# neu-vi/Superpoints_Registration

Measured on AMD Instinct MI355X. Metric: point-cloud pairs/sec (16 384 pts/cloud), higher is better.
Workload: dtype f32 (matrix products: range-scaled split-f16x2 MFMA, f32 accumulate; attention weights below 2^-5 of their row sum carried in one f16 plane); 1 GPU; synthetic 16384-pt pairs, full KPConv backbone + superpoint attn + Sinkhorn-SVD pose (3dmatch config, BASELINE configs[1]); streams_per_gpu=1, points_per_cloud=16384, generator=box, point_order=reference, upsample_indices=True, cross_step_overlap=True, streams_inside_a_forward=3: main path, pyramid searches, ResNet shortcut branches

## Files before the change

### include/spr.h

```cpp
#ifndef SPR_H_
#define SPR_H_

#include <stddef.h>
#include <stdint.h>

#ifdef __cplusplus
extern "C" {
#endif

#define SPR_VERSION 6

#define SPR_ACT_NONE 0
#define SPR_ACT_RELU 1
#define SPR_ACT_SIGMOID 2

#define SPR_ORDER_REFERENCE 0
#define SPR_ORDER_CANONICAL 1

int spr_version(void);
const char* spr_last_error(void);

size_t spr_grid_subsample_workspace_bytes(int n, int nb);
int spr_grid_subsample(const float* xyz, const int* cu, int n, int nb, float dl,
                       int max_p, int order_mode, float* out_xyz, int* out_lens,
                       int* out_total, void* ws, size_t ws_bytes, void* stream);

size_t spr_voxel_downsample_workspace_bytes(int n);
int spr_voxel_downsample(const float* xyz, int n, double voxel_size, int* out_idx,
                         int* out_count, void* ws, size_t ws_bytes, void* stream);

size_t spr_radius_neighbors_workspace_bytes(int nq, int ns, int nb);
int spr_radius_neighbors(const float* q_xyz, const int* q_cu, int nq,
                         const float* s_xyz, const int* s_cu, int ns, int nb,
                         float radius, int limit, int algo, int* out_idx,
                         int* max_count, void* ws, size_t ws_bytes, void* stream);

size_t spr_radius_table_bytes(int ns, int nb);
size_t spr_radius_table_build_workspace_bytes(int ns, int nb);
size_t spr_radius_table_query_workspace_bytes(int nq);
int spr_radius_table_slots(void);
int spr_radius_table_build(const float* s_xyz, const int* s_cu, int ns, int nb, float radius,
                           void* table, size_t table_bytes, void* ws, size_t ws_bytes, void* stream);
int spr_radius_table_query(const float* q_xyz, const int* q_cu, int nq, int self, int ns, int nb,
                           float radius, int limit, int slot, const void* table, int* out_idx,
                           int* max_count, int algo, void* ws, size_t ws_bytes, void* stream);

size_t spr_gt_overlap_workspace_bytes(int ns, int nt, int nb);
int spr_gt_overlap(const float* src_xyz, const int* src_cu, int ns, const float* tgt_xyz, const int* tgt_cu,
                   int nt, const float* pose, int nb, double radius, int* src_corr, int* tgt_corr,
                   unsigned char* src_mask, unsigned char* tgt_mask, int* corr, int* corr_count, void* ws,
                   size_t ws_bytes, void* stream);

#define SPR_AUG_NONE 0
#define SPR_AUG_SMALL 1
#define SPR_AUG_LARGE 2
int spr_philox4x32_host(const uint32_t* ctr_host, const uint32_t* key_host, uint32_t* out_host);
int spr_augment_draw(uint64_t seed, const uint64_t* pair_key_host, int nb, int mode, unsigned char* perturb_src_host,
                     unsigned char* swap_host, float* perturb_host, const uint64_t* pair_key, const int* src_cu,
                     int ns, const int* tgt_cu, int nt, float* noise, unsigned int* keys, void* stream);
size_t spr_augment_workspace_bytes(int ns, int nt, int nb, int corr_stride);
int spr_augment_pairs(const float* src_xyz, const int* src_cu, int ns, const float* tgt_xyz, const int* tgt_cu,
                      int nt, const float* pose, int nb, const unsigned char* src_mask,
                      const unsigned char* tgt_mask, const int* corr, int corr_stride, const int* corr_off,
                      const int* corr_count, const float* perturb, const unsigned char* flags, int mode, float scale,
                      int max_pts, uint64_t seed, const uint64_t* pair_key, const float* noise,
                      const unsigned int* keys, float* out_src_xyz, float* out_tgt_xyz, int* out_src_cu,
                      int* out_tgt_cu, float* out_pose, unsigned char* out_src_mask, unsigned char* out_tgt_mask,
                      int* out_src_perm, int* out_tgt_perm, int* out_corr, int* out_corr_count, int* status, void* ws,
                      size_t ws_bytes, void* stream);

size_t spr_kpconv_workspace_bytes(int nq, int ns, int cin, int cout);
size_t spr_kpconv_plan_bytes(int nq);
int spr_kpconv_plan(const int* nbr, int nq, int ns, int nbr_stride, int kmax, int rows_sorted,
                    const int* order, void* plan, size_t plan_bytes, void* stream);
size_t spr_kpconv_wplanes_bytes(int cin, int cout);
int spr_kpconv_prep_weights(const float* weights, int n_kp, int cin, int cout, const float* w_range,
                            int w_range_n, void* wplanes, size_t wplanes_bytes, void* stream);
int spr_kpconv_fwd(const float* q_xyz, int nq, const float* s_xyz, int ns, const int* nbr,
                   int nbr_stride, int kmax, int rows_sorted, const float* x, int cin,
                   const float* weights, int cout, const float* kernel_points, int n_kp,
                   float kp_extent, float* out, int impl, const float* x_range, int x_range_n,
                   const float* w_range, int w_range_n, const void* plan, const void* wplanes,
                   void* ws, size_t ws_bytes, void* stream);

size_t spr_instnorm_workspace_bytes(int max_len_host, int nb, int c);
int spr_instnorm(const float* x, const int* cu, int n, int nb, int max_len_host, int c,
                 float eps, int norm, const float* add, float slope, float* out,
                 float* out_range, int out_range_n, void* ws, size_t ws_bytes, void* stream);
int spr_instnorm_stats(const float* x, const int* cu, int n, int nb, int max_len_host, int c, float eps,
                       float* mean, float* rstd, void* ws, size_t ws_bytes, void* stream);

int spr_block_tail_tile_rows(int ka, int kb, int n_out);
size_t spr_block_tail_tiles_len(int n, int nb, int tile_rows);
int spr_block_tail_tiles(const int* cu, int n, int nb, int tile_rows, int* tiles, void* stream);
size_t spr_block_tail_workspace_bytes(int n, int nb, int kb, int n_out, int tile_rows);
int spr_block_tail(const float* xa, int ka, const float* wa, const float* xb, int kb, const float* wb,
                   const float* add, const int* cu, const int* tiles, int n, int nb, int n_out, float eps,
                   float slope, float* out, const float* xa_range, int xa_range_n, const float* wa_range,
                   int wa_range_n, const float* xb_range, int xb_range_n, const float* wb_range,
                   int wb_range_n, float* out_range, int out_range_n, const float* xa_mean,
                   const float* xa_rstd, float xa_slope, void* ws, size_t ws_bytes, void* stream);

int spr_maxpool_gather(const float* x, int ns, int c, const int* idx, int nq, int idx_stride, int k,
                       const int* order, float* out, float* out_range, int out_range_n, void* stream);
size_t spr_cell_order_workspace_bytes(int n);
int spr_cell_order(const float* xyz, const int* cu, int n, int nb, float cell, int* order, void* ws, size_t ws_bytes,
                   void* stream);

size_t spr_linear_workspace_bytes(void);
int spr_linear(const float* x, int m, int k, const float* w, int n, const float* bias,
               const float* residual, int act, float* out, const float* x_range,
               int x_range_n, const float* w_range, int w_range_n, float* out_range,
               int out_range_cap, int* out_range_n_host, void* ws, size_t ws_bytes, void* stream);
int spr_range_parts(void);
int spr_absmax(const float* x, long rows, int cols, long stride, float* parts, void* stream);
int spr_absmax_multi(const void* jobs_dev, int njobs, int parts_per_job, float* parts_out, void* stream);

int spr_set_gemm_mode(int mode);

int spr_layernorm_range_count(int m);
int spr_layernorm(const float* x, int m, int c, const float* gamma, const float* beta,
                  float eps, const float* pos, float* out_norm, float* out_pos,
                  float* range_norm, float* range_pos, void* stream);

int spr_posemb_sine(const float* xyz, int n, int d_model, float scale,
                    float temperature, float* out, void* stream);

size_t spr_attn_workspace_bytes(int t, int nseg, int nhead, int head_dim);
int spr_attn_varlen_fwd(const float* q, int q_stride, const float* k, int k_stride, const float* v,
                        int v_stride, const int* cu, const int* kv_seg, int t, int nseg, int max_len_host,
                        int nhead, int head_dim, float scale, float* out, int o_stride, float* lse,
                        int* lse_written, void* ws, size_t ws_bytes, void* stream);

size_t spr_attn_inproj_workspace_bytes(int t, int nseg, int nhead, int head_dim);
int spr_attn_inproj_prepare(const float* w_in, int d, float* out, void* stream);
int spr_attn_inproj_varlen_fwd(const float* x_qk, const float* x_v, int t, const float* w_in,
                               const float* b_in, const int* cu, const int* kv_seg, int nseg,
                               int max_len_host, int nhead, int head_dim, float scale,
                               float* out, int o_stride, const float* xqk_range,
                               int xqk_range_n, const float* xv_range, int xv_range_n,
                               float* out_range, const float* w_prep, void* ws, size_t ws_bytes, void* stream);

size_t spr_attn_probs_workspace_bytes(int t, int nhead, int head_dim);
int spr_attn_probs(const float* q, int q_stride, const float* k, int k_stride, const int* cu,
                   const int* kv_seg, int t, int nseg, int max_len_host, int nhead, int head_dim,
                   float scale, int per_head, float* out, const long long* place, int max_rows_host,
                   int max_cols_host, void* ws, size_t ws_bytes, void* stream);

#define SPR_XENC_PTRS_PER_LAYER 18
size_t spr_xenc_prepared_bytes(int n_layers, int d_ff);
size_t spr_xenc_plan_bytes(void);
int spr_xenc_prepare(const void* const* layer_ptrs_host, const float* eps_host, int n_layers,
                     int d_model, int nhead, int d_ff, const float* final_g, const float* final_b,
                     float final_eps, float pos_bound, void* prepared, size_t prepared_bytes,
                     void* plan_host, size_t plan_bytes, void* stream);
size_t spr_xenc_workspace_bytes(int t, int nseg);
int spr_xenc_forward(const void* plan_host, const float* x, const float* pos, const int* cu,
                     const int* kv_self, const int* kv_cross, int t, int nseg, int max_len_host,
                     float* out, void* ws, size_t ws_bytes, void* stream);

size_t spr_attn_bwd_workspace_bytes(int t, int nseg, int nhead);
size_t spr_attn_bwd_min_workspace_bytes(int t, int nhead);
int spr_attn_varlen_bwd(const float* q, int q_stride, const float* k, int k_stride, const float* v,
                        int v_stride, const float* out, int o_stride, const float* dout, int do_stride,
                        const float* lse, const int* cu, const int* kv_seg, const int* q_seg, int t, int nseg,
                        int max_len_host, int nhead, int head_dim, float scale, float* dq, float* dk,
                        float* dv, void* ws, size_t ws_bytes, void* stream);

int spr_set_attn_mode(int mode);

size_t spr_match_workspace_bytes(const int* cu_host, int npairs);
int spr_match_dualsoftmax(const float* feat, int d, const int* cu,
                          const int* cu_host, int npairs, float* match_val,
                          float* match_val2, int* match_ind, void* ws, size_t ws_bytes,
                          void* stream);

int spr_pose_residuals(const float* pose, const float* a, const float* b, const int* pair_cu,
                       int npairs, int total_host, float* res, void* stream);
int spr_pose_scores(const float* poses, int nh, const float* a, const float* b, int n,
                    float* score, void* stream);

int spr_weighted_procrustes(const float* a, const float* b, const float* w,
                            const int* pair_cu, int npairs, float* out_pose,
                            void* stream);

size_t spr_sinkhorn_workspace_bytes(const int* cu_host, int npairs);
int spr_sinkhorn_correspondences(const float* feat, int d, const float* xyz,
                                 const int* cu, const int* cu_host, int npairs,
                                 const float* alpha, const float* beta, int n_iters,
                                 int slack, float* out_w, float* out_that,
                                 void* ws, size_t ws_bytes, void* stream);

int spr_match_sinkhorn(const float* feat, int d, const float* xyz, const int* cu, const int* cu_host,
                       int npairs, const float* alpha, const float* beta, int n_iters, float* match_val,
                       float* match_val2, int* match_ind, float* out_w, float* out_that, void* ws,
                       size_t ws_bytes, void* stream);

int spr_gather_rows(const float* x, int n_src, int c, const int* idx, int n,
                    float* out, void* stream);

size_t spr_loss_workspace_bytes(int n_max, int m_max, int d);
int spr_overlap_pool(const float* ov_prev, int ns_prev, const int* pool,
                     int pool_stride, int w, int nq, float* out, void* stream);
int spr_bce_logits_mean(const float* x, const float* y, int n, float* out,
                        void* ws, size_t ws_bytes, void* stream);
int spr_infonce_pair(const float* anchor_feat, int n, const float* positive_feat,
                     int m, int d, const float* anchor_xyz, const float* pose_gt,
                     const float* positive_xyz, const float* W, float r_p,
                     float r_n, float* out, void* ws, size_t ws_bytes,
                     void* stream);
int spr_transform_l1_pair(const float* pose_gt, const float* pose_pred,
                          const float* xyz, int n, float* out, void* ws,
                          size_t ws_bytes, void* stream);
int spr_sum_scaled(const float* values, int n, float scale, float* out,
                   void* stream);

int spr_bgemm(const float* A, const float* B, float* C, const void* desc_dev, int nbatch,
              int max_m, int max_n, long sa_i, long sa_k, long sb_k, long sb_j, long sc_i,
              long sc_j, float alpha, float beta, void* stream);
size_t spr_tn_product_split_workspace_bytes(void);
int spr_tn_product_split(const float* L, const float* R, long rows, int nl, int nr, int chunk,
                         const float* l_range, int l_range_n, const float* r_range, int r_range_n,
                         float* parts, void* ws, size_t ws_bytes, void* stream);
size_t spr_tn_product_f64_workspace_bytes(long rows, int nl, int nr);
int spr_tn_product_f64(const float* L, const float* R, long rows, int nl, int nr, float* out,
                       void* ws, size_t ws_bytes, void* stream);
int spr_reduce_parts(const float* parts, int nparts, long n, float scale, float* out,
                     int accumulate, void* stream);
int spr_act_bwd(const float* y, const float* dy, int act, long n, float* out, void* stream);
size_t spr_colsum_workspace_bytes(int n);
int spr_colsum(const float* x, long m, int n, float* out, void* ws, size_t ws_bytes, void* stream);
size_t spr_layernorm_bwd_workspace_bytes(int c);
int spr_layernorm_bwd(const float* x, int m, int c, const float* gamma, float eps,
                      const float* dy_norm, const float* dy_pos, float* dx, float* dgamma,
                      float* dbeta, void* ws, size_t ws_bytes, void* stream);
size_t spr_instnorm_bwd_workspace_bytes(int max_len_host, int nb, int c);
int spr_instnorm_bwd(const float* x, const float* out, const float* dout, const int* cu, int n,
                     int nb, int max_len_host, int c, float eps, int norm, float slope,
                     float* dx, float* dadd, void* ws, size_t ws_bytes, void* stream);
size_t spr_scatter_workspace_bytes(long rows, int c);
int spr_maxpool_bwd(const float* x, int ns, int c, const int* idx, int nq, int idx_stride, int k,
                    const float* dy, float* dx, void* ws, size_t ws_bytes, void* stream);
int spr_scatter_rows_add(const float* dy, const int* idx, int n, int c, int n_src, float* dx,
                         void* ws, size_t ws_bytes, void* stream);
size_t spr_kpconv_weighted_features_workspace_bytes(int ns);
int spr_kpconv_weighted_features(const float* q_xyz, int nq, const float* s_xyz, int ns,
                                 const int* nbr, int nbr_stride, int kmax, const float* x, int cin,
                                 const float* kernel_points, int n_kp, float kp_extent,
                                 float* wf, float* cnt, void* ws, size_t ws_bytes, void* stream);
int spr_kpconv_bwd_dx(const float* q_xyz, int nq, const float* s_xyz, int ns, const int* nbr,
                      int nbr_stride, int kmax, int cin, const float* kernel_points, int n_kp,
                      float kp_extent, const float* dwf, const float* dwf_range, int dwf_range_n, float* dx,
                      void* ws, size_t ws_bytes, void* stream);
int spr_softmax_rows(float* mat, const void* desc_dev, int nbatch, int max_m, void* stream);
int spr_softmax_bwd_rows(const float* p, float* dp, const void* desc_dev, int nbatch, int max_m,
                         void* stream);

int spr_bce_logits_mean_bwd(const float* x, const float* y, int n, const float* gout, float* dx,
                            void* stream);
int spr_infonce_pair_dlogits(const float* anchor_feat, int n, const float* positive_feat, int m,
                             int d, const float* anchor_xyz, const float* pose_gt,
                             const float* positive_xyz, const float* W, float r_p, float r_n,
                             float* dlogits, float* row_mask, float* wsym_out, float* t_out,
                             void* ws, size_t ws_bytes, void* stream);
int spr_wsym_bwd(const float* dwsym, int d, float* dW, void* stream);
int spr_transform_l1_pair_bwd(const float* pose_gt, const float* pose_pred, const float* xyz, int n,
                              const float* gout, float* dpose_pred, void* stream);
int spr_weighted_procrustes_bwd(const float* a, const float* b, const float* w,
                                const int* pair_cu, int npairs, const float* dpose, float* da,
                                float* db, float* dw, void* stream);
size_t spr_sinkhorn_bwd_workspace_bytes(const int* cu_host, int npairs, int n_iters);
int spr_sinkhorn_bwd(const float* feat, int d, const float* xyz, const int* cu,
                     const int* cu_host, int npairs, const float* alpha, const float* beta,
                     int n_iters, const float* dw, const float* dthat, float* dfeat,
                     float* dalpha, float* dbeta, void* ws, size_t ws_bytes, void* stream);

size_t spr_circle_loss_workspace_bytes(int nbatch, int max_n, int max_m);
int spr_circle_loss(const float* src_feat, const float* tgt_feat, int d, const float* src_xyz,
                    const float* pose_gt, const float* tgt_xyz, const int* cu_src, const int* cu_tgt,
                    int nbatch, int max_n, int max_m, float r_p, float r_n, float* out, void* ws,
                    size_t ws_bytes, void* stream);
int spr_circle_loss_bwd(const float* src_feat, const float* tgt_feat, int d, const float* src_xyz,
                        const float* pose_gt, const float* tgt_xyz, const int* cu_src, const int* cu_tgt,
                        int nbatch, int max_n, int max_m, float r_p, float r_n, const float* gout, float* G,
                        float* d_src, float* d_tgt, void* ws, size_t ws_bytes, void* stream);

int spr_prof_enable(int on);
int spr_prof_read(int max_records, int* codes_host, int* nqs_host, float* ms_host);

int spr_selftest(int* status_host);

#ifdef __cplusplus
}
#endif
#endif
```

### superpoints_registration_amd/_lib.py

```python
import ctypes
import os
import subprocess

_HERE = os.path.dirname(os.path.abspath(__file__))
LIB_PATH = os.environ.get("SPR_HIP_LIB") or os.path.join(_HERE, "libspr_hip.so")

_vp = ctypes.c_void_p
_i = ctypes.c_int
_f = ctypes.c_float
_sz = ctypes.c_size_t
_l = ctypes.c_long
_u64 = ctypes.c_uint64

SIGNATURES = {
    "spr_version": (_i, []),
    "spr_last_error": (ctypes.c_char_p, []),
    "spr_grid_subsample_workspace_bytes": (_sz, [_i, _i]),
    "spr_grid_subsample": (_i, [_vp, _vp, _i, _i, _f, _i, _i, _vp, _vp, _vp, _vp, _sz, _vp]),
    "spr_voxel_downsample_workspace_bytes": (_sz, [_i]),
    "spr_voxel_downsample": (_i, [_vp, _i, ctypes.c_double, _vp, _vp, _vp, _sz, _vp]),
    "spr_radius_neighbors_workspace_bytes": (_sz, [_i, _i, _i]),
    "spr_radius_neighbors": (_i, [_vp, _vp, _i, _vp, _vp, _i, _i, _f, _i, _i, _vp, _vp, _vp, _sz, _vp]),
    "spr_radius_table_bytes": (_sz, [_i, _i]),
    "spr_radius_table_build_workspace_bytes": (_sz, [_i, _i]),
    "spr_radius_table_query_workspace_bytes": (_sz, [_i]),
    "spr_radius_table_slots": (_i, []),
    "spr_radius_table_build": (_i, [_vp, _vp, _i, _i, _f, _vp, _sz, _vp, _sz, _vp]),
    "spr_radius_table_query": (_i, [_vp, _vp, _i, _i, _i, _i, _f, _i, _i, _vp, _vp, _vp, _i, _vp, _sz, _vp]),
    "spr_gt_overlap_workspace_bytes": (_sz, [_i, _i, _i]),
    "spr_gt_overlap": (_i, [_vp, _vp, _i, _vp, _vp, _i, _vp, _i, ctypes.c_double, _vp, _vp, _vp, _vp, _vp, _vp, _vp,
                            _sz, _vp]),
    "spr_philox4x32_host": (_i, [_vp, _vp, _vp]),
    "spr_augment_draw": (_i, [_u64, _vp, _i, _i, _vp, _vp, _vp, _vp, _vp, _i, _vp, _i, _vp, _vp, _vp]),
    "spr_augment_workspace_bytes": (_sz, [_i, _i, _i, _i]),
    "spr_augment_pairs": (_i, [_vp, _vp, _i, _vp, _vp, _i, _vp, _i, _vp, _vp, _vp, _i, _vp, _vp, _vp, _vp, _i, _f, _i,
                               _u64, _vp, _vp, _vp, _vp, _vp, _vp, _vp, _vp, _vp, _vp, _vp, _vp, _vp, _vp, _vp, _vp,
                               _sz, _vp]),
    "spr_kpconv_workspace_bytes": (_sz, [_i, _i, _i, _i]),
    "spr_kpconv_fwd": (_i, [_vp, _i, _vp, _i, _vp, _i, _i, _i, _vp, _i, _vp, _i, _vp, _i, _f, _vp, _i, _vp, _i, _vp,
                            _i, _vp, _vp, _vp, _sz, _vp]),
    "spr_instnorm_workspace_bytes": (_sz, [_i, _i, _i]),
    "spr_instnorm": (_i, [_vp, _vp, _i, _i, _i, _i, _f, _i, _vp, _f, _vp, _vp, _i, _vp, _sz, _vp]),
    "spr_maxpool_gather": (_i, [_vp, _i, _i, _vp, _i, _i, _i, _vp, _vp, _vp, _i, _vp]),
    "spr_linear_workspace_bytes": (_sz, []),
    "spr_linear": (_i, [_vp, _i, _i, _vp, _i, _vp, _vp, _i, _vp, _vp, _i, _vp, _i, _vp, _i, _vp, _vp, _sz, _vp]),
    "spr_range_parts": (_i, []),
    "spr_absmax_multi": (_i, [_vp, _i, _i, _vp, _vp]),
    "spr_absmax": (_i, [_vp, _l, _i, _l, _vp, _vp]),
    "spr_kpconv_plan_bytes": (_sz, [_i]),
    "spr_kpconv_plan": (_i, [_vp, _i, _i, _i, _i, _i, _vp, _vp, _sz, _vp]),
    "spr_kpconv_wplanes_bytes": (_sz, [_i, _i]),
    "spr_kpconv_prep_weights": (_i, [_vp, _i, _i, _i, _vp, _i, _vp, _sz, _vp]),
    "spr_block_tail_tile_rows": (_i, [_i, _i, _i]),
    "spr_block_tail_tiles_len": (_sz, [_i, _i, _i]),
    "spr_block_tail_tiles": (_i, [_vp, _i, _i, _i, _vp, _vp]),
    "spr_block_tail_workspace_bytes": (_sz, [_i, _i, _i, _i, _i]),
    "spr_block_tail": (_i, [_vp, _i, _vp, _vp, _i, _vp, _vp, _vp, _vp, _i, _i, _i, _f, _f, _vp, _vp, _i, _vp, _i,
                            _vp, _i, _vp, _i, _vp, _i, _vp, _vp, _f, _vp, _sz, _vp]),
    "spr_instnorm_stats": (_i, [_vp, _vp, _i, _i, _i, _i, _f, _vp, _vp, _vp, _sz, _vp]),
    "spr_cell_order_workspace_bytes": (_sz, [_i]),
    "spr_cell_order": (_i, [_vp, _vp, _i, _i, _f, _vp, _vp, _sz, _vp]),
    "spr_layernorm_range_count": (_i, [_i]),
    "spr_attn_inproj_prepare": (_i, [_vp, _i, _vp, _vp]),
    "spr_set_gemm_mode": (_i, [_i]),
    "spr_layernorm": (_i, [_vp, _i, _i, _vp, _vp, _f, _vp, _vp, _vp, _vp, _vp, _vp]),
    "spr_posemb_sine": (_i, [_vp, _i, _i, _f, _f, _vp, _vp]),
    "spr_attn_workspace_bytes": (_sz, [_i, _i, _i, _i]),
    "spr_attn_varlen_fwd": (_i, [_vp, _i, _vp, _i, _vp, _i, _vp, _vp, _i, _i, _i, _i, _i, _f, _vp, _i, _vp, _vp, _vp,
                                 _sz, _vp]),
    "spr_attn_probs_workspace_bytes": (_sz, [_i, _i, _i]),
    "spr_attn_probs": (_i, [_vp, _i, _vp, _i, _vp, _vp, _i, _i, _i, _i, _i, _f, _i, _vp, _vp, _i, _i, _vp, _sz,
                            _vp]),
    "spr_attn_bwd_workspace_bytes": (_sz, [_i, _i, _i]),
    "spr_attn_bwd_min_workspace_bytes": (_sz, [_i, _i]),
    "spr_attn_varlen_bwd": (_i, [_vp, _i, _vp, _i, _vp, _i, _vp, _i, _vp, _i, _vp, _vp, _vp, _vp, _i, _i, _i, _i, _i,
                                 _f, _vp, _vp, _vp, _vp, _sz, _vp]),
    "spr_attn_inproj_workspace_bytes": (_sz, [_i, _i, _i, _i]),
    "spr_attn_inproj_varlen_fwd": (_i, [_vp, _vp, _i, _vp, _vp, _vp, _vp, _i, _i, _i, _i, _f, _vp, _i, _vp, _i, _vp,
                                        _i, _vp, _vp, _vp, _sz, _vp]),
    "spr_set_attn_mode": (_i, [_i]),
    "spr_xenc_prepared_bytes": (_sz, [_i, _i]),
    "spr_xenc_plan_bytes": (_sz, []),
    "spr_xenc_prepare": (_i, [_vp, _vp, _i, _i, _i, _i, _vp, _vp, _f, _f, _vp, _sz, _vp, _sz, _vp]),
    "spr_xenc_workspace_bytes": (_sz, [_i, _i]),
    "spr_xenc_forward": (_i, [_vp, _vp, _vp, _vp, _vp, _vp, _i, _i, _i, _vp, _vp, _sz, _vp]),
    "spr_match_workspace_bytes": (_sz, [_vp, _i]),
    "spr_match_dualsoftmax": (_i, [_vp, _i, _vp, _vp, _i, _vp, _vp, _vp, _vp, _sz, _vp]),
    "spr_pose_residuals": (_i, [_vp, _vp, _vp, _vp, _i, _i, _vp, _vp]),
    "spr_pose_scores": (_i, [_vp, _i, _vp, _vp, _i, _vp, _vp]),
    "spr_weighted_procrustes": (_i, [_vp, _vp, _vp, _vp, _i, _vp, _vp]),
    "spr_sinkhorn_workspace_bytes": (_sz, [_vp, _i]),
    "spr_match_sinkhorn": (_i, [_vp, _i, _vp, _vp, _vp, _i, _vp, _vp, _i, _vp, _vp, _vp, _vp, _vp, _vp, _sz, _vp]),
    "spr_sinkhorn_correspondences": (_i, [_vp, _i, _vp, _vp, _vp, _i, _vp, _vp, _i, _i, _vp, _vp, _vp,
                                          _sz, _vp]),
    "spr_loss_workspace_bytes": (_sz, [_i, _i, _i]),
    "spr_overlap_pool": (_i, [_vp, _i, _vp, _i, _i, _i, _vp, _vp]),
    "spr_bce_logits_mean": (_i, [_vp, _vp, _i, _vp, _vp, _sz, _vp]),
    "spr_infonce_pair": (_i, [_vp, _i, _vp, _i, _i, _vp, _vp, _vp, _vp, _f, _f, _vp, _vp, _sz, _vp]),
    "spr_transform_l1_pair": (_i, [_vp, _vp, _vp, _i, _vp, _vp, _sz, _vp]),
    "spr_sum_scaled": (_i, [_vp, _i, _f, _vp, _vp]),
    "spr_gather_rows": (_i, [_vp, _i, _i, _vp, _i, _vp, _vp]),
    "spr_bgemm": (_i, [_vp, _vp, _vp, _vp, _i, _i, _i, _l, _l, _l, _l, _l, _l, _f, _f, _vp]),
    "spr_tn_product_split_workspace_bytes": (_sz, []),
    "spr_tn_product_split": (_i, [_vp, _vp, _l, _i, _i, _i, _vp, _i, _vp, _i, _vp, _vp, _sz, _vp]),
    "spr_tn_product_f64_workspace_bytes": (_sz, [_l, _i, _i]),
    "spr_tn_product_f64": (_i, [_vp, _vp, _l, _i, _i, _vp, _vp, _sz, _vp]),
    "spr_reduce_parts": (_i, [_vp, _i, _l, _f, _vp, _i, _vp]),
    "spr_act_bwd": (_i, [_vp, _vp, _i, _l, _vp, _vp]),
    "spr_colsum_workspace_bytes": (_sz, [_i]),
    "spr_colsum": (_i, [_vp, _l, _i, _vp, _vp, _sz, _vp]),
    "spr_layernorm_bwd_workspace_bytes": (_sz, [_i]),
    "spr_layernorm_bwd": (_i, [_vp, _i, _i, _vp, _f, _vp, _vp, _vp, _vp, _vp, _vp, _sz, _vp]),
    "spr_instnorm_bwd_workspace_bytes": (_sz, [_i, _i, _i]),
    "spr_instnorm_bwd": (_i, [_vp, _vp, _vp, _vp, _i, _i, _i, _i, _f, _i, _f, _vp, _vp, _vp, _sz, _vp]),
    "spr_scatter_workspace_bytes": (_sz, [_l, _i]),
    "spr_maxpool_bwd": (_i, [_vp, _i, _i, _vp, _i, _i, _i, _vp, _vp, _vp, _sz, _vp]),
    "spr_scatter_rows_add": (_i, [_vp, _vp, _i, _i, _i, _vp, _vp, _sz, _vp]),
    "spr_kpconv_weighted_features_workspace_bytes": (_sz, [_i]),
    "spr_kpconv_weighted_features": (_i, [_vp, _i, _vp, _i, _vp, _i, _i, _vp, _i, _vp, _i, _f, _vp, _vp, _vp, _sz,
                                          _vp]),
    "spr_kpconv_bwd_dx": (_i, [_vp, _i, _vp, _i, _vp, _i, _i, _i, _vp, _i, _f, _vp, _vp, _i, _vp, _vp, _sz, _vp]),
    "spr_softmax_rows": (_i, [_vp, _vp, _i, _i, _vp]),
    "spr_softmax_bwd_rows": (_i, [_vp, _vp, _vp, _i, _i, _vp]),
    "spr_bce_logits_mean_bwd": (_i, [_vp, _vp, _i, _vp, _vp, _vp]),
    "spr_infonce_pair_dlogits": (_i, [_vp, _i, _vp, _i, _i, _vp, _vp, _vp, _vp, _f, _f, _vp, _vp, _vp, _vp, _vp, _sz,
                                      _vp]),
    "spr_wsym_bwd": (_i, [_vp, _i, _vp, _vp]),
    "spr_transform_l1_pair_bwd": (_i, [_vp, _vp, _vp, _i, _vp, _vp, _vp]),
    "spr_weighted_procrustes_bwd": (_i, [_vp, _vp, _vp, _vp, _i, _vp, _vp, _vp, _vp, _vp]),
    "spr_sinkhorn_bwd_workspace_bytes": (_sz, [_vp, _i, _i]),
    "spr_sinkhorn_bwd": (_i, [_vp, _i, _vp, _vp, _vp, _i, _vp, _vp, _i, _vp, _vp, _vp, _vp, _vp, _vp, _sz, _vp]),
    "spr_circle_loss_workspace_bytes": (_sz, [_i, _i, _i]),
    "spr_circle_loss": (_i, [_vp, _vp, _i, _vp, _vp, _vp, _vp, _vp, _i, _i, _i, _f, _f, _vp, _vp, _sz, _vp]),
    "spr_circle_loss_bwd": (_i, [_vp, _vp, _i, _vp, _vp, _vp, _vp, _vp, _i, _i, _i, _f, _f, _vp, _vp, _vp, _vp, _vp,
                                 _sz, _vp]),
    "spr_selftest": (_i, [_vp]),
    "spr_prof_enable": (_i, [_i]),
    "spr_prof_read": (_i, [_i, _vp, _vp, _vp]),
}

_lib = None


def build(force: bool = False) -> str:
    if force:
        subprocess.check_call(["make", "-s", "-C", os.path.join(_HERE, "csrc"), "clean"])
    subprocess.check_call(["make", "-s", "-j8", "-C", os.path.join(_HERE, "csrc")])
    return LIB_PATH


def lib():
    global _lib
    if _lib is None:
        if not os.path.exists(LIB_PATH):
            raise RuntimeError(
                f"{LIB_PATH} is missing: build it with "
                "`python -c 'import __graft_entry__ as g; g.build()'` "
                "(there is no fallback path)")
        l = ctypes.CDLL(LIB_PATH)
        for name, (res, args) in SIGNATURES.items():
            fn = getattr(l, name)
            fn.restype = res
            fn.argtypes = args
        _lib = l
    return _lib


def check(rc: int, what: str) -> None:
    if rc != 0:
        msg = lib().spr_last_error()
        raise RuntimeError(f"{what}: {msg.decode() if msg else 'error'} (status {rc})")
```

### superpoints_registration_amd/csrc/grid_subsample.hip

```cpp
#include <cstring>
#include <rocprim/device/device_radix_sort.hpp>
#include <rocprim/device/device_scan.hpp>

#include <mutex>
#include <unordered_map>
#include <vector>

#include "spr_common.h"

namespace spr {
namespace {

constexpr int kKeyBits = 40;
constexpr unsigned long long kKeyMask = (1ull << kKeyBits) - 1;
constexpr int kMaxSched = 40;

struct CloudInfo {
  float org[3];
  unsigned int nx, ny;
};

struct SchedArg {
  unsigned int v[kMaxSched];
};

struct Schedule {
  std::vector<unsigned int> buckets;
};
const Schedule& host_schedule() {
  static Schedule s;
  static std::once_flag once;
  std::call_once(once, [] {
    std::unordered_map<size_t, char> m;
    size_t bc = m.bucket_count();
    s.buckets.push_back((unsigned int)bc);
    const size_t kMax = (size_t)1 << 22;
    for (size_t i = 0; i < kMax; ++i) {
      m.emplace(i, 0);
      if (m.bucket_count() != bc) {
        bc = m.bucket_count();
        s.buckets.push_back((unsigned int)bc);
      }
    }
  });
  return s;
}

__global__ __launch_bounds__(256) void k_bbox(const float* __restrict__ xyz,
                                              const int* __restrict__ cu,
                                              float dl, CloudInfo* info) {
  const int c = blockIdx.x;
  const int beg = cu[c], end = cu[c + 1];
  __shared__ float smn[3][256], smx[3][256];
  float mn[3], mx[3];
  if (end > beg) {
    for (int d = 0; d < 3; ++d) mn[d] = mx[d] = xyz[3 * (size_t)beg + d];
  } else {
    for (int d = 0; d < 3; ++d) mn[d] = mx[d] = 0.f;
  }
  for (int i = beg + threadIdx.x; i < end; i += blockDim.x) {
    for (int d = 0; d < 3; ++d) {
      float v = xyz[3 * (size_t)i + d];
      if (v < mn[d]) mn[d] = v;
      if (v > mx[d]) mx[d] = v;
    }
  }
  for (int d = 0; d < 3; ++d) {
    smn[d][threadIdx.x] = mn[d];
    smx[d][threadIdx.x] = mx[d];
  }
  __syncthreads();
  for (int s = 128; s > 0; s >>= 1) {
    if (threadIdx.x < s) {
      for (int d = 0; d < 3; ++d) {
        float a = smn[d][threadIdx.x + s];
        if (a < smn[d][threadIdx.x]) smn[d][threadIdx.x] = a;
        float b = smx[d][threadIdx.x + s];
        if (b > smx[d][threadIdx.x]) smx[d][threadIdx.x] = b;
      }
    }
    __syncthreads();
  }
  if (threadIdx.x == 0) {
    const float inv = __fdiv_rn(1.0f, dl);
    CloudInfo ci;
    for (int d = 0; d < 3; ++d)
      ci.org[d] = __fmul_rn(floorf(__fmul_rn(smn[d][0], inv)), dl);
    ci.nx = (unsigned int)floorf(__fdiv_rn(__fsub_rn(smx[0][0], ci.org[0]), dl)) + 1u;
    ci.ny = (unsigned int)floorf(__fdiv_rn(__fsub_rn(smx[1][0], ci.org[1]), dl)) + 1u;
    info[c] = ci;
  }
}

__global__ void k_keys(const float* __restrict__ xyz, const int* __restrict__ cu,
                       int n, int nb, float dl, const CloudInfo* __restrict__ info,
                       unsigned long long* keys, int* vals, int* err) {
  const int i = blockIdx.x * blockDim.x + threadIdx.x;
  if (i >= n) return;
  const int c = find_segment(cu, nb, i);
  const CloudInfo ci = info[c];
  const unsigned long long ix =
      (unsigned long long)floorf(__fdiv_rn(__fsub_rn(xyz[3 * (size_t)i + 0], ci.org[0]), dl));
  const unsigned long long iy =
      (unsigned long long)floorf(__fdiv_rn(__fsub_rn(xyz[3 * (size_t)i + 1], ci.org[1]), dl));
  const unsigned long long iz =
      (unsigned long long)floorf(__fdiv_rn(__fsub_rn(xyz[3 * (size_t)i + 2], ci.org[2]), dl));
  const unsigned long long key =
      ix + (unsigned long long)ci.nx * iy + (unsigned long long)ci.nx * ci.ny * iz;
  if (key > kKeyMask) atomicOr(err, 1);
  keys[i] = ((unsigned long long)c << kKeyBits) | (key & kKeyMask);
  vals[i] = i;
}

__global__ void k_flags(const unsigned long long* __restrict__ keys, int n, int* flags) {
  const int i = blockIdx.x * blockDim.x + threadIdx.x;
  if (i >= n) return;
  flags[i] = (i == 0 || keys[i] != keys[i - 1]) ? 1 : 0;
}

__global__ void k_segstart(const int* __restrict__ flags, const int* __restrict__ vid,
                           int n, int* vstart, int* nvox) {
  const int i = blockIdx.x * blockDim.x + threadIdx.x;
  if (i >= n) return;
  if (flags[i]) vstart[vid[i]] = i;
  if (i == n - 1) *nvox = vid[i] + flags[i];
}

__global__ void k_bary(const float* __restrict__ xyz,
                       const unsigned long long* __restrict__ keys,
                       const int* __restrict__ vals, const int* __restrict__ vstart,
                       const int* __restrict__ nvox_p, int n, float* bary,
                       unsigned long long* vkey, int* vfirst) {
  const int v = blockIdx.x * blockDim.x + threadIdx.x;
  const int nvox = *nvox_p;
  if (v >= nvox) return;
  const int beg = vstart[v];
  const int end = (v + 1 < nvox) ? vstart[v + 1] : n;
  float sx = 0.f, sy = 0.f, sz = 0.f;
  for (int j = beg; j < end; ++j) {
    const size_t p = (size_t)vals[j];
    sx = __fadd_rn(sx, xyz[3 * p + 0]);
    sy = __fadd_rn(sy, xyz[3 * p + 1]);
    sz = __fadd_rn(sz, xyz[3 * p + 2]);
  }
  const float a = (float)(1.0 / (double)(end - beg));
  bary[3 * (size_t)v + 0] = __fmul_rn(sx, a);
  bary[3 * (size_t)v + 1] = __fmul_rn(sy, a);
  bary[3 * (size_t)v + 2] = __fmul_rn(sz, a);
  const unsigned long long k = keys[beg];
  vkey[v] = k;
  vfirst[v] = vals[beg];
}

__global__ void k_cloud_lb(const unsigned long long* __restrict__ vkey,
                           const int* __restrict__ nvox_p, int nb, int* vcu) {
  const int c = blockIdx.x * blockDim.x + threadIdx.x;
  if (c > nb) return;
  const int nvox = *nvox_p;
  int lo = 0, hi = nvox;
  while (lo < hi) {
    const int mid = (lo + hi) >> 1;
    if ((int)(vkey[mid] >> kKeyBits) < c)
      lo = mid + 1;
    else
      hi = mid;
  }
  vcu[c] = lo;
}

__global__ void k_cloud_offsets(const int* __restrict__ vcu, int nb, int max_p, int* out_cu,
                                int* out_lens, int* out_total) {
  if (threadIdx.x != 0 || blockIdx.x != 0) return;
  int b = 0;
  for (int c = 0; c < nb; ++c) {
    out_cu[c] = b;
    const int m = vcu[c + 1] - vcu[c];
    const int keep = (max_p > 0 && m > max_p) ? max_p : m;
    out_lens[c] = keep;
    b += keep;
  }
  out_cu[nb] = b;
  *out_total = b;
}

__global__ void k_emit_canonical(const float* __restrict__ bary,
                                 const unsigned long long* __restrict__ vkey,
                                 const int* __restrict__ nvox_p,
                                 const int* __restrict__ vcu,
                                 const int* __restrict__ out_cu,
                                 const int* __restrict__ out_lens, float* out) {
  const int v = blockIdx.x * blockDim.x + threadIdx.x;
  if (v >= *nvox_p) return;
  const int c = (int)(vkey[v] >> kKeyBits);
  const int r = v - vcu[c];
  if (r >= out_lens[c]) return;
  const size_t o = (size_t)(out_cu[c] + r);
  out[3 * o + 0] = bary[3 * (size_t)v + 0];
  out[3 * o + 1] = bary[3 * (size_t)v + 1];
  out[3 * o + 2] = bary[3 * (size_t)v + 2];
}

__global__ void k_mark_first(const int* __restrict__ vfirst, const int* __restrict__ nvox_p, int* __restrict__ mark,
                             int* __restrict__ who) {
  const int v = blockIdx.x * blockDim.x + threadIdx.x;
  if (v >= *nvox_p) return;
  const int f = vfirst[v];
  mark[f] = 1;
  who[f] = v;
}
__global__ void k_compact_first(const int* __restrict__ mark, const int* __restrict__ pos, const int* __restrict__ who,
                                int n, int* __restrict__ ins) {
  const int i = blockIdx.x * blockDim.x + threadIdx.x;
  if (i >= n || !mark[i]) return;
  ins[pos[i]] = who[i];
}

__device__ void block_inclusive_scan(int* data, int m, int* lds ) {
  const int t = threadIdx.x, T = blockDim.x;
  const int per = (m + T - 1) / T;
  const int beg = min(t * per, m), end = min(beg + per, m);
  int s = 0;
  for (int i = beg; i < end; ++i) s += data[i];
  lds[t] = s;
  __syncthreads();
  for (int o = 1; o < T; o <<= 1) {
    int v = (t >= o) ? lds[t - o] : 0;
    __syncthreads();
    lds[t] += v;
    __syncthreads();
  }
  int run = lds[t] - s;
  for (int i = beg; i < end; ++i) {
    run += data[i];
    data[i] = run;
  }
  __syncthreads();
}

__device__ __forceinline__ int fast_mod(unsigned long long k, unsigned int nbk, double inv) {
  const unsigned long long q = (unsigned long long)((double)k * inv);
  long long r = (long long)k - (long long)(q * (unsigned long long)nbk);
  if (r < 0) r += nbk;
  else if (r >= (long long)nbk) r -= nbk;
  return (int)r;
}

constexpr int kUmapLdsInts = 31744;

__global__ __launch_bounds__(1024) void k_umap_order(
    const unsigned long long* __restrict__ vkey, const int* __restrict__ ins,
    const int* __restrict__ vcu, const int* __restrict__ cu, int nsched, SchedArg sched,
    int* listA, int* listB, int* tfirst, int* tcnt, int* thead, int* nxt,
    int* scan, int* bucket, const float* __restrict__ bary, const int* __restrict__ out_cu,
    const int* __restrict__ out_lens, float* out) {
  __shared__ int lds[1024];
  extern __shared__ int lds_tab[];
  const int c = blockIdx.x;
  const int base = vcu[c];
  const int m = vcu[c + 1] - base;
  if (m <= 0) return;
  int* la = listA + base;
  int* lb = listB + base;
  int* nx = nxt + base;
  int* sc = scan + base;
  int* bk = bucket + base;
  const size_t toff = 3 * (size_t)cu[c] + 16 * (size_t)c;
  const int t = threadIdx.x, T = blockDim.x;

  int done = 0;
  int e = 0;
  int* cur = la;
  int* nxtl = lb;
  while (done < m) {
    e += 1;
    if (e >= nsched) break;
    const int nbk = (int)sched.v[e];
    const int upto = min(m, nbk);
    const int len = upto;
    const double inv = 1.0 / (double)nbk;
    auto epoch = [&](int* tf, int* tc, int* th) {
      for (int b = t; b < nbk; b += T) {
        tf[b] = 0x7fffffff;
        tc[b] = 0;
        th[b] = -1;
      }
      for (int p = done + t; p < upto; p += T) cur[p] = p;
      __syncthreads();
      for (int p = t; p < len; p += T) {
        const int el = cur[p];
        const int b = fast_mod(vkey[ins[base + el]] & kKeyMask, (unsigned int)nbk, inv);
        bk[p] = b;
        atomicMin(&tf[b], p);
        atomicAdd(&tc[b], 1);
        nx[p] = atomicExch(&th[b], p);
      }
      __syncthreads();
      for (int p = t; p < len; p += T) {
        const int b = bk[p];
        sc[p] = (tf[b] == p) ? tc[b] : 0;
      }
      __syncthreads();
      block_inclusive_scan(sc, len, lds);
      const int total = len;
      for (int p = t; p < len; p += T) {
        const int b = bk[p];
        int greater = 0;
        for (int q = th[b]; q != -1; q = nx[q]) greater += (q > p) ? 1 : 0;
        const int pos = (total - sc[tf[b]]) + greater;
        nxtl[pos] = cur[p];
      }
      __syncthreads();
    };
    if (3 * nbk <= kUmapLdsInts) epoch(lds_tab, lds_tab + nbk, lds_tab + 2 * nbk);
    else epoch(tfirst + toff, tcnt + toff, thead + toff);
    int* tmp = cur;
    cur = nxtl;
    nxtl = tmp;
    done = upto;
  }
  const int keep = out_lens[c];
  const size_t ob = (size_t)out_cu[c];
  for (int p = t; p < keep; p += T) {
    const size_t v = (size_t)ins[base + cur[p]];
    out[3 * (ob + p) + 0] = bary[3 * v + 0];
    out[3 * (ob + p) + 1] = bary[3 * v + 1];
    out[3 * (ob + p) + 2] = bary[3 * v + 2];
  }
}

__global__ void k_check_err(const int* err, int* out_total) {
  if (*err) *out_total = -1;
}

size_t sort_temp_bytes(int n) {
  size_t bytes = 0;
  rocprim::radix_sort_pairs(nullptr, bytes, (unsigned long long*)nullptr,
                            (unsigned long long*)nullptr, (int*)nullptr, (int*)nullptr,
                            (unsigned int)(n > 0 ? n : 1));
  size_t sb = 0;
  rocprim::exclusive_scan(nullptr, sb, (int*)nullptr, (int*)nullptr, 0, (size_t)(n > 0 ? n : 1),
                          rocprim::plus<int>());
  return align_up(bytes > sb ? bytes : sb, 256) + 256;
}

}
}

using namespace spr;

extern "C" size_t spr_grid_subsample_workspace_bytes(int n, int nb) {
  const size_t N = (size_t)(n > 0 ? n : 1), B = (size_t)(nb > 0 ? nb : 1);
  size_t b = 0;
  b += align_up(sizeof(CloudInfo) * B, 256);
  b += 3 * align_up(8 * N, 256);
  b += 10 * align_up(4 * N, 256);
  b += 2 * align_up(4 * N, 256);
  b += align_up(12 * N, 256);
  b += 3 * align_up(4 * (3 * N + 16 * B + 64), 256);
  b += 4 * align_up(4 * (B + 1), 256);
  b += 1024;
  b += sort_temp_bytes(n);
  return b;
}

extern "C" int spr_grid_subsample(const float* xyz, const int* cu, int n, int nb,
                                  float dl, int max_p, int order_mode,
                                  float* out_xyz, int* out_lens, int* out_total,
                                  void* ws, size_t ws_bytes, void* stream_) {
  hipStream_t stream = (hipStream_t)stream_;
  SPR_REQUIRE(n >= 0 && nb >= 1, "grid_subsample: bad sizes n=%d nb=%d", n, nb);
  SPR_REQUIRE(dl > 0.f, "grid_subsample: sampleDl must be > 0");
  SPR_REQUIRE(nb < (1 << 23), "grid_subsample: too many clouds");
  SPR_REQUIRE(n > 0, "grid_subsample: empty input");
  SPR_REQUIRE(ws_bytes >= spr_grid_subsample_workspace_bytes(n, nb),
              "grid_subsample: workspace too small");
  Workspace w(ws, ws_bytes);
  const size_t N = (size_t)n;
  CloudInfo* info = w.take<CloudInfo>(nb);
  unsigned long long* keys = w.take<unsigned long long>(N);
  unsigned long long* keys2 = w.take<unsigned long long>(N);
  unsigned long long* vkey = w.take<unsigned long long>(N);
  int* vals = w.take<int>(N);
  int* vals2 = w.take<int>(N);
  int* flags = w.take<int>(N);
  int* vid = w.take<int>(N);
  int* vstart = w.take<int>(N);
  int* vfirst = w.take<int>(N);
  int* sval = w.take<int>(N);
  int* sval2 = w.take<int>(N);
  int* listA = w.take<int>(N);
  int* listB = w.take<int>(N);
  int* nxt = w.take<int>(N);
  int* scan = w.take<int>(N);
  float* bary = w.take<float>(3 * N);
  const size_t tsz = 3 * N + 16 * (size_t)nb + 64;
  int* tfirst = w.take<int>(tsz);
  int* tcnt = w.take<int>(tsz);
  int* thead = w.take<int>(tsz);
  int* cloud_cnt = w.take<int>(nb + 1);
  int* vcu = w.take<int>(nb + 1);
  int* out_cu = w.take<int>(nb + 1);
  int* scalars = w.take<int>(64);
  size_t temp_bytes = sort_temp_bytes(n);
  void* temp = w.take<char>(temp_bytes);
  SPR_REQUIRE(temp != nullptr, "grid_subsample: workspace carve failed");
  int* nvox = scalars;
  int* err = scalars + 1;

  SPR_HIP_CHECK(hipMemsetAsync(scalars, 0, 64 * sizeof(int), stream));
  SPR_HIP_CHECK(hipMemsetAsync(cloud_cnt, 0, (nb + 1) * sizeof(int), stream));

  const int TB = 256;
  hipLaunchKernelGGL(k_bbox, dim3(nb), dim3(256), 0, stream, xyz, cu, dl, info);
  hipLaunchKernelGGL(k_keys, dim3(cdiv(n, TB)), dim3(TB), 0, stream, xyz, cu, n, nb, dl,
                     info, keys, vals, err);
  SPR_LAUNCH_CHECK();
  size_t tb = temp_bytes;
  int key_bits = kKeyBits + 1;
  while (key_bits < 64 && (1ull << (key_bits - kKeyBits)) < (unsigned long long)nb) ++key_bits;
  SPR_HIP_CHECK(rocprim::radix_sort_pairs(temp, tb, keys, keys2, vals, vals2,
                                          (unsigned int)n, 0, key_bits, stream));
  hipLaunchKernelGGL(k_flags, dim3(cdiv(n, TB)), dim3(TB), 0, stream, keys2, n, flags);
  tb = temp_bytes;
  SPR_HIP_CHECK(rocprim::exclusive_scan(temp, tb, flags, vid, 0, (size_t)n,
                                        rocprim::plus<int>(), stream));
  hipLaunchKernelGGL(k_segstart, dim3(cdiv(n, TB)), dim3(TB), 0, stream, flags, vid, n,
                     vstart, nvox);
  hipLaunchKernelGGL(k_bary, dim3(cdiv(n, TB)), dim3(TB), 0, stream, xyz, keys2, vals2,
                     vstart, nvox, n, bary, vkey, vfirst);
  hipLaunchKernelGGL(k_cloud_lb, dim3(cdiv(nb + 1, 256)), dim3(256), 0, stream, vkey, nvox, nb, vcu);
  hipLaunchKernelGGL(k_cloud_offsets, dim3(1), dim3(64), 0, stream, vcu, nb, max_p, out_cu,
                     out_lens, out_total);
  SPR_LAUNCH_CHECK();
  if (order_mode == SPR_ORDER_CANONICAL) {
    hipLaunchKernelGGL(k_emit_canonical, dim3(cdiv(n, TB)), dim3(TB), 0, stream, bary,
                       vkey, nvox, vcu, out_cu, out_lens, out_xyz);
  } else {
    const Schedule& s = host_schedule();
    SchedArg sched;
    for (int i = 0; i < kMaxSched; ++i)
      sched.v[i] = i < (int)s.buckets.size() ? s.buckets[i] : 0xffffffffu;
    const int nsched = (int)(s.buckets.size() < (size_t)kMaxSched ? s.buckets.size() : kMaxSched);
    SPR_HIP_CHECK(hipMemsetAsync(flags, 0, N * sizeof(int), stream));
    hipLaunchKernelGGL(k_mark_first, dim3(cdiv(n, TB)), dim3(TB), 0, stream, vfirst, nvox, flags, vid);
    tb = temp_bytes;
    SPR_HIP_CHECK(rocprim::exclusive_scan(temp, tb, flags, vstart, 0, (size_t)n, rocprim::plus<int>(), stream));
    hipLaunchKernelGGL(k_compact_first, dim3(cdiv(n, TB)), dim3(TB), 0, stream, flags, vstart, vid, n, sval2);
    const int umap_lds = kUmapLdsInts * (int)sizeof(int);
    if (int rc = ensure_dyn_lds((const void*)k_umap_order, umap_lds)) return rc;
    hipLaunchKernelGGL(k_umap_order, dim3(nb), dim3(1024), umap_lds, stream, vkey, sval2, vcu, cu,
                       nsched, sched, listA, listB, tfirst, tcnt, thead, nxt, scan, sval, bary, out_cu,
                       out_lens, out_xyz);
  }
  hipLaunchKernelGGL(k_check_err, dim3(1), dim3(1), 0, stream, err, out_total);
  SPR_LAUNCH_CHECK();
  return 0;
}

namespace spr {
namespace {
__device__ __forceinline__ unsigned int spread10(unsigned int v) {
  v &= 0x3ffu;
  v = (v | (v << 16)) & 0x030000ffu;
  v = (v | (v << 8)) & 0x0300f00fu;
  v = (v | (v << 4)) & 0x030c30c3u;
  v = (v | (v << 2)) & 0x09249249u;
  return v;
}
__global__ void k_order_keys(const float* __restrict__ xyz, const int* __restrict__ cu, int n, int nb, float inv_cell,
                             unsigned long long* __restrict__ keys, int* __restrict__ vals) {
  const int i = blockIdx.x * blockDim.x + threadIdx.x;
  if (i >= n) return;
  int lo = 0, hi = nb;
  while (hi - lo > 1) {
    const int mid = (lo + hi) >> 1;
    if (cu[mid] <= i) lo = mid; else hi = mid;
  }
  const int o = cu[lo];
  unsigned int c[3];
#pragma unroll
  for (int a = 0; a < 3; ++a) {
    const float d = (xyz[3 * (size_t)i + a] - xyz[3 * (size_t)o + a]) * inv_cell;
    const int q = (int)floorf(fminf(fmaxf(d, -512.f), 511.f)) + 512;
    c[a] = (unsigned int)q;
  }
  const unsigned int m = spread10(c[0]) | (spread10(c[1]) << 1) | (spread10(c[2]) << 2);
  keys[i] = ((unsigned long long)lo << 30) | m;
  vals[i] = i;
}
}
}

extern "C" size_t spr_cell_order_workspace_bytes(int n) {
  const size_t N = (size_t)(n > 0 ? n : 1);
  return 2 * align_up(8 * N, 256) + align_up(4 * N, 256) + sort_temp_bytes(n) + 256;
}

extern "C" int spr_cell_order(const float* xyz, const int* cu, int n, int nb, float cell, int* order, void* ws,
                              size_t ws_bytes, void* stream_) {
  hipStream_t stream = (hipStream_t)stream_;
  SPR_REQUIRE(n >= 1 && nb >= 1 && nb < (1 << 30) && cell > 0.f, "cell_order: bad arguments");
  SPR_REQUIRE(ws_bytes >= spr_cell_order_workspace_bytes(n), "cell_order: workspace too small");
  Workspace w(ws, ws_bytes);
  unsigned long long* keys = w.take<unsigned long long>(n);
  unsigned long long* keys2 = w.take<unsigned long long>(n);
  int* vals = w.take<int>(n);
  size_t tb = sort_temp_bytes(n);
  void* temp = w.take<char>(tb);
  SPR_REQUIRE(temp != nullptr, "cell_order: workspace carve failed");
  hipLaunchKernelGGL(k_order_keys, dim3(cdiv(n, 256)), dim3(256), 0, stream, xyz, cu, n, nb, 1.0f / cell, keys, vals);
  SPR_LAUNCH_CHECK();
  int bits = 31;
  while (bits < 60 && (1ull << (bits - 30)) < (unsigned long long)nb) ++bits;
  SPR_HIP_CHECK(rocprim::radix_sort_pairs(temp, tb, keys, keys2, vals, order, (unsigned int)n, 0, bits, stream));
  return 0;
}

namespace spr {
namespace {
__global__ void k_vox_keys(const float* __restrict__ xyz, int n, double voxel, unsigned long long* keys,
                           int* vals, int* err) {
  const int i = blockIdx.x * blockDim.x + threadIdx.x;
  if (i >= n) return;
  unsigned long long k = 0;
#pragma unroll
  for (int d = 0; d < 3; ++d) {
    const double q = (double)xyz[3 * (size_t)i + d] / voxel;
    const long long c = (long long)q;
    if (c < -(1ll << 20) || c >= (1ll << 20)) atomicExch(err, 1);
    k = (k << 21) | (unsigned long long)((c + (1ll << 20)) & 0x1fffff);
  }
  keys[i] = k;
  vals[i] = i;
}
__global__ void k_vox_heads(const unsigned long long* __restrict__ keys, const int* __restrict__ vals, int n,
                            unsigned int* out) {
  const int i = blockIdx.x * blockDim.x + threadIdx.x;
  if (i >= n) return;
  const bool head = i == 0 || keys[i] != keys[i - 1];
  out[i] = head ? (unsigned int)vals[i] : 0xffffffffu;
}
__global__ void k_vox_count(const unsigned int* __restrict__ sorted, int n, int* out_idx, int* count,
                            const int* err) {
  const int i = blockIdx.x * blockDim.x + threadIdx.x;
  if (i >= n) return;
  const bool ok = sorted[i] != 0xffffffffu;
  out_idx[i] = ok ? (int)sorted[i] : -1;
  if (ok && (i + 1 == n || sorted[i + 1] == 0xffffffffu)) count[0] = err[0] ? -1 : i + 1;
}
size_t vox_temp_bytes(int n) {
  size_t a = 0, b = 0;
  rocprim::radix_sort_pairs(nullptr, a, (unsigned long long*)nullptr, (unsigned long long*)nullptr, (int*)nullptr,
                            (int*)nullptr, (unsigned int)(n > 0 ? n : 1), 0, 63);
  rocprim::radix_sort_keys(nullptr, b, (unsigned int*)nullptr, (unsigned int*)nullptr, (unsigned int)(n > 0 ? n : 1), 0,
                           32);
  return align_up(a > b ? a : b, 256);
}
}
}

extern "C" size_t spr_voxel_downsample_workspace_bytes(int n) {
  const size_t N = (size_t)(n > 0 ? n : 1);
  return 2 * align_up(8 * N, 256) + 4 * align_up(4 * N, 256) + 256 + spr::vox_temp_bytes(n);
}

extern "C" int spr_voxel_downsample(const float* xyz, int n, double voxel_size, int* out_idx, int* out_count, void* ws,
                                    size_t ws_bytes, void* stream_) {
  hipStream_t stream = (hipStream_t)stream_;
  SPR_REQUIRE(n >= 1 && voxel_size > 0.0 && xyz && out_idx && out_count, "voxel_downsample: bad arguments");
  SPR_REQUIRE(ws && ws_bytes >= spr_voxel_downsample_workspace_bytes(n), "voxel_downsample: workspace too small");
  Workspace w(ws, ws_bytes);
  unsigned long long* keys = w.take<unsigned long long>(n);
  unsigned long long* keys2 = w.take<unsigned long long>(n);
  int* vals = w.take<int>(n);
  int* vals2 = w.take<int>(n);
  unsigned int* sel = w.take<unsigned int>(n);
  unsigned int* sel2 = w.take<unsigned int>(n);
  int* err = w.take<int>(1);
  const size_t temp_bytes = vox_temp_bytes(n);
  void* temp = w.take<char>(temp_bytes);
  SPR_REQUIRE(temp != nullptr, "voxel_downsample: workspace carve failed");
  SPR_HIP_CHECK(hipMemsetAsync(err, 0, sizeof(int), stream));
  SPR_HIP_CHECK(hipMemsetAsync(out_count, 0, sizeof(int), stream));
  const int TBk = 256;
  hipLaunchKernelGGL(k_vox_keys, dim3(cdiv(n, TBk)), dim3(TBk), 0, stream, xyz, n, voxel_size, keys, vals, err);
  size_t tb = temp_bytes;
  SPR_HIP_CHECK(rocprim::radix_sort_pairs(temp, tb, keys, keys2, vals, vals2, (unsigned int)n, 0, 63, stream));
  hipLaunchKernelGGL(k_vox_heads, dim3(cdiv(n, TBk)), dim3(TBk), 0, stream, keys2, vals2, n, sel);
  tb = temp_bytes;
  SPR_HIP_CHECK(rocprim::radix_sort_keys(temp, tb, sel, sel2, (unsigned int)n, 0, 32, stream));
  hipLaunchKernelGGL(k_vox_count, dim3(cdiv(n, TBk)), dim3(TBk), 0, stream, sel2, n, out_idx, out_count, err);
  SPR_LAUNCH_CHECK();
  return 0;
}
```

### superpoints_registration_amd/csrc/radius_neighbors.hip

```cpp
#include <cstring>
#include <rocprim/device/device_radix_sort.hpp>
#include <rocprim/device/device_scan.hpp>

#include "spr_common.h"
#include <type_traits>

namespace spr {
namespace {

struct NbrCloud {
  float mn[3];
  int pad;
};

constexpr int kMaxCell = 8191;

__global__ __launch_bounds__(256) void k_min(const float* __restrict__ xyz,
                                             const int* __restrict__ cu, NbrCloud* info) {
  const int c = blockIdx.x;
  const int beg = cu[c], end = cu[c + 1];
  __shared__ float smn[3][256];
  float mn[3] = {3.0e38f, 3.0e38f, 3.0e38f};
  for (int i = beg + threadIdx.x; i < end; i += blockDim.x)
    for (int d = 0; d < 3; ++d) mn[d] = fminf(mn[d], xyz[3 * (size_t)i + d]);
  for (int d = 0; d < 3; ++d) smn[d][threadIdx.x] = mn[d];
  __syncthreads();
  for (int s = 128; s > 0; s >>= 1) {
    if (threadIdx.x < s)
      for (int d = 0; d < 3; ++d)
        smn[d][threadIdx.x] = fminf(smn[d][threadIdx.x], smn[d][threadIdx.x + s]);
    __syncthreads();
  }
  if (threadIdx.x == 0) {
    NbrCloud ci;
    for (int d = 0; d < 3; ++d) ci.mn[d] = (end > beg) ? smn[d][0] : 0.f;
    ci.pad = 0;
    info[c] = ci;
  }
}

__device__ __forceinline__ int cell_coord(float p, float mn, float inv_cell) {
  float v = (p - mn) * inv_cell;
  v = fminf(fmaxf(v, -4.0f), 20000.0f);
  return (int)floorf(v);
}

__device__ __forceinline__ unsigned long long pack_key(int c, int cz, int cy, int cx) {
  return ((unsigned long long)c << 48) | ((unsigned long long)cz << 32) |
         ((unsigned long long)cy << 16) | (unsigned long long)cx;
}

__global__ void k_cellkeys(const float* __restrict__ xyz, const int* __restrict__ cu, int n,
                           int nb, float inv_cell, const NbrCloud* __restrict__ info,
                           unsigned long long* keys, int* vals, int* err) {
  const int i = blockIdx.x * blockDim.x + threadIdx.x;
  if (i >= n) return;
  const int c = find_segment(cu, nb, i);
  const NbrCloud ci = info[c];
  const int cx = cell_coord(xyz[3 * (size_t)i + 0], ci.mn[0], inv_cell);
  const int cy = cell_coord(xyz[3 * (size_t)i + 1], ci.mn[1], inv_cell);
  const int cz = cell_coord(xyz[3 * (size_t)i + 2], ci.mn[2], inv_cell);
  if (cx > kMaxCell || cy > kMaxCell || cz > kMaxCell || cx < 0 || cy < 0 || cz < 0)
    atomicOr(err, 1);
  keys[i] = pack_key(c, cz & 0xffff, cy & 0xffff, cx & 0xffff);
  vals[i] = i;
}

__global__ void k_gather_sorted(const float* __restrict__ xyz, const int* __restrict__ vals,
                                int n, float4* rec) {
  const int i = blockIdx.x * blockDim.x + threadIdx.x;
  if (i >= n) return;
  const int j = vals[i];
  rec[i] = make_float4(xyz[3 * (size_t)j + 0], xyz[3 * (size_t)j + 1], xyz[3 * (size_t)j + 2],
                       __int_as_float(j));
}

__device__ __forceinline__ bool nbr_less(float d2a, int ia, float d2b, int ib) {
  return (d2a < d2b) || (d2a == d2b && ia < ib);
}

template <int BLOCK>
__global__ __launch_bounds__(BLOCK) void k_query(
    const float* __restrict__ q_xyz, const int* __restrict__ q_cu, int nq,
    const int* __restrict__ s_cu, int ns, int nb, const NbrCloud* __restrict__ info,
    const unsigned long long* __restrict__ skeys, const float4* __restrict__ rec, float r2,
    float inv_cell, int limit, int* __restrict__ out, int* max_count) {
  extern __shared__ __align__(16) unsigned char smem[];
  float* l_d2 = (float*)smem;
  int* l_id = (int*)(smem + sizeof(float) * (size_t)limit * BLOCK);
  const int t = threadIdx.x;
  const int i = blockIdx.x * BLOCK + t;
  int total = 0;
  if (i < nq) {
    const int c = find_segment(q_cu, nb, i);
    const NbrCloud ci = info[c];
    const float qx = q_xyz[3 * (size_t)i + 0], qy = q_xyz[3 * (size_t)i + 1],
                qz = q_xyz[3 * (size_t)i + 2];
    const int cx = cell_coord(qx, ci.mn[0], inv_cell);
    const int cy = cell_coord(qy, ci.mn[1], inv_cell);
    const int cz = cell_coord(qz, ci.mn[2], inv_cell);
    const int sbeg = s_cu[c], send = s_cu[c + 1];
    int kept = 0;
    const int xlo = max(cx - 1, 0), xhi = min(cx + 1, kMaxCell);
    if (xhi >= 0 && xlo <= kMaxCell && send > sbeg) {
      for (int dz = -1; dz <= 1; ++dz) {
        const int z = cz + dz;
        if (z < 0 || z > kMaxCell) continue;
        for (int dy = -1; dy <= 1; ++dy) {
          const int y = cy + dy;
          if (y < 0 || y > kMaxCell) continue;
          const unsigned long long klo = pack_key(c, z, y, xlo);
          const unsigned long long khi = pack_key(c, z, y, xhi);
          int lo = sbeg, hi = send;
          while (lo < hi) {
            const int mid = (lo + hi) >> 1;
            if (skeys[mid] < klo)
              lo = mid + 1;
            else
              hi = mid;
          }
          for (int j = lo; j < send; ++j) {
            if (skeys[j] > khi) break;
            const float4 s = rec[j];
            const float dx = __fsub_rn(qx, s.x), dy2 = __fsub_rn(qy, s.y),
                        dzz = __fsub_rn(qz, s.z);
            float d2 = __fmul_rn(dx, dx);
            d2 = __fadd_rn(d2, __fmul_rn(dy2, dy2));
            d2 = __fadd_rn(d2, __fmul_rn(dzz, dzz));
            if (d2 < r2) {
              total++;
              const int sid = __float_as_int(s.w);
              int pos;
              if (kept < limit) {
                pos = kept++;
              } else {
                const int last = limit - 1;
                if (!nbr_less(d2, sid, l_d2[last * BLOCK + t], l_id[last * BLOCK + t]))
                  continue;
                pos = last;
              }
              while (pos > 0 &&
                     nbr_less(d2, sid, l_d2[(pos - 1) * BLOCK + t], l_id[(pos - 1) * BLOCK + t])) {
                l_d2[pos * BLOCK + t] = l_d2[(pos - 1) * BLOCK + t];
                l_id[pos * BLOCK + t] = l_id[(pos - 1) * BLOCK + t];
                --pos;
              }
              l_d2[pos * BLOCK + t] = d2;
              l_id[pos * BLOCK + t] = sid;
            }
          }
        }
      }
    }
    int* row = out + (size_t)i * limit;
    for (int k = 0; k < limit; ++k) row[k] = (k < kept) ? l_id[k * BLOCK + t] : ns;
  }
  int m = total;
#pragma unroll
  for (int o = 32; o > 0; o >>= 1) m = max(m, __shfl_xor(m, o, 64));
  if ((t & 63) == 0 && m > 0) atomicMax(max_count, m);
}


struct GridCloud {
  float mn[3];
  int dim[3];
  long long off;
};

__global__ __launch_bounds__(256) void k_grid_dims(const float* __restrict__ xyz,
                                                   const int* __restrict__ cu, float inv_cell,
                                                   GridCloud* info, int* err) {
  const int c = blockIdx.x;
  const int beg = cu[c], end = cu[c + 1];
  __shared__ float smn[3][256], smx[3][256];
  float mn[3] = {3.0e38f, 3.0e38f, 3.0e38f}, mx[3] = {-3.0e38f, -3.0e38f, -3.0e38f};
  for (int i = beg + threadIdx.x; i < end; i += blockDim.x)
    for (int d = 0; d < 3; ++d) {
      const float v = xyz[3 * (size_t)i + d];
      mn[d] = fminf(mn[d], v);
      mx[d] = fmaxf(mx[d], v);
    }
  for (int d = 0; d < 3; ++d) {
    smn[d][threadIdx.x] = mn[d];
    smx[d][threadIdx.x] = mx[d];
  }
  __syncthreads();
  for (int s = 128; s > 0; s >>= 1) {
    if (threadIdx.x < s)
      for (int d = 0; d < 3; ++d) {
        smn[d][threadIdx.x] = fminf(smn[d][threadIdx.x], smn[d][threadIdx.x + s]);
        smx[d][threadIdx.x] = fmaxf(smx[d][threadIdx.x], smx[d][threadIdx.x + s]);
      }
    __syncthreads();
  }
  if (threadIdx.x == 0) {
    GridCloud g;
    for (int d = 0; d < 3; ++d) {
      g.mn[d] = (end > beg) ? smn[d][0] : 0.f;
      int n = 1;
      if (end > beg) {
        n = cell_coord(smx[d][0], g.mn[d], inv_cell) + 1;
        if (n < 1) n = 1;
        if (n > kMaxCell + 1) {
          atomicOr(err, 1);
          n = 1;
        }
      }
      g.dim[d] = n;
    }
    g.off = 0;
    info[c] = g;
  }
}

constexpr int kTableSlots = 8;
constexpr int kHdrErr = 0, kHdrCells = 1, kHdrSlot0 = 8;
__global__ void k_grid_offsets(GridCloud* info, int nb, long long cap, int* hdr) {
  if (threadIdx.x != 0 || blockIdx.x != 0) return;
  int* err = hdr + kHdrErr;
  for (int k = 0; k < kTableSlots; ++k) hdr[kHdrSlot0 + k] = 0;
  long long off = 0;
  for (int c = 0; c < nb; ++c) {
    info[c].off = off;
    off += (long long)info[c].dim[0] * info[c].dim[1] * info[c].dim[2];
    if (off > cap) {
      atomicOr(err, 2);
      off = 0;
    }
  }
  hdr[kHdrCells] = (int)off;
}

constexpr int kScanBlock = 4096;
__global__ __launch_bounds__(256) void k_table_zero(const int* __restrict__ hdr, int* __restrict__ count) {
  const long base = (long)blockIdx.x * kScanBlock;
  if (base > (long)hdr[kHdrCells]) return;
  int4* p = reinterpret_cast<int4*>(count + base) + threadIdx.x;
#pragma unroll
  for (int u = 0; u < 4; ++u) p[u * 256] = make_int4(0, 0, 0, 0);
}

__device__ __forceinline__ int block_sum_256(int v, int* sh ) {
#pragma unroll
  for (int o = 32; o > 0; o >>= 1) v += __shfl_xor(v, o, 64);
  if ((threadIdx.x & 63) == 0) sh[threadIdx.x >> 6] = v;
  __syncthreads();
  const int r = sh[0] + sh[1] + sh[2] + sh[3];
  __syncthreads();
  return r;
}

__global__ __launch_bounds__(256) void k_table_bsum(const int* __restrict__ hdr, const int* __restrict__ count,
                                                    int* __restrict__ bsum) {
  __shared__ int sh[4];
  const long base = (long)blockIdx.x * kScanBlock;
  if (base > (long)hdr[kHdrCells]) return;
  const int4* p = reinterpret_cast<const int4*>(count + base) + threadIdx.x;
  int v = 0;
#pragma unroll
  for (int u = 0; u < 4; ++u) {
    const int4 q = p[u * 256];
    v += q.x + q.y + q.z + q.w;
  }
  v = block_sum_256(v, sh);
  if (threadIdx.x == 0) bsum[blockIdx.x] = v;
}

__global__ __launch_bounds__(256) void k_table_scan(const int* __restrict__ hdr, int* __restrict__ count,
                                                    const int* __restrict__ bsum) {
  __shared__ int sh[4];
  __shared__ int wsum[4];
  const long base = (long)blockIdx.x * kScanBlock;
  if (base > (long)hdr[kHdrCells]) return;
  int off = 0;
  for (int b = threadIdx.x; b < (int)blockIdx.x; b += 256) off += bsum[b];
  off = block_sum_256(off, sh);
  int4* p = reinterpret_cast<int4*>(count + base) + 4 * threadIdx.x;
  int4 q[4];
#pragma unroll
  for (int u = 0; u < 4; ++u) q[u] = p[u];
  int mine = 0;
#pragma unroll
  for (int u = 0; u < 4; ++u) mine += q[u].x + q[u].y + q[u].z + q[u].w;
  int incl = mine;
  const int lane = threadIdx.x & 63;
#pragma unroll
  for (int o = 1; o < 64; o <<= 1) {
    const int v = __shfl_up(incl, o, 64);
    if (lane >= o) incl += v;
  }
  if (lane == 63) wsum[threadIdx.x >> 6] = incl;
  __syncthreads();
  int run = off + incl - mine;
  for (int w = 0; w < (int)(threadIdx.x >> 6); ++w) run += wsum[w];
#pragma unroll
  for (int u = 0; u < 4; ++u) {
    int4 o4;
    o4.x = run; run += q[u].x;
    o4.y = run; run += q[u].y;
    o4.z = run; run += q[u].z;
    o4.w = run; run += q[u].w;
    p[u] = o4;
  }
}

__device__ __forceinline__ long long grid_cell(const GridCloud& g, int cx, int cy, int cz) {
  return g.off + ((long long)cz * g.dim[1] + cy) * g.dim[0] + cx;
}

__global__ void k_cell_count(const float* __restrict__ xyz, const int* __restrict__ cu, int n, int nb,
                             float inv_cell, const GridCloud* __restrict__ info,
                             const int* __restrict__ err, int* count, int* cell_of, int* rank) {
  const int i = blockIdx.x * blockDim.x + threadIdx.x;
  if (i >= n || *err) return;
  const int c = find_segment(cu, nb, i);
  const GridCloud g = info[c];
  int cx = cell_coord(xyz[3 * (size_t)i + 0], g.mn[0], inv_cell);
  int cy = cell_coord(xyz[3 * (size_t)i + 1], g.mn[1], inv_cell);
  int cz = cell_coord(xyz[3 * (size_t)i + 2], g.mn[2], inv_cell);
  cx = min(max(cx, 0), g.dim[0] - 1);
  cy = min(max(cy, 0), g.dim[1] - 1);
  cz = min(max(cz, 0), g.dim[2] - 1);
  const long long L = grid_cell(g, cx, cy, cz);
  cell_of[i] = (int)L;
  rank[i] = atomicAdd(&count[L], 1);
}

__global__ void k_cell_scatter(const float* __restrict__ xyz, int n, const int* __restrict__ err,
                               const int* __restrict__ cell_of, const int* __restrict__ start,
                               const int* __restrict__ rank, float4* rec) {
  const int i = blockIdx.x * blockDim.x + threadIdx.x;
  if (i >= n || *err) return;
  const int L = cell_of[i];
  const int pos = start[L] + rank[i];
  rec[pos] = make_float4(xyz[3 * (size_t)i + 0], xyz[3 * (size_t)i + 1], xyz[3 * (size_t)i + 2],
                         __int_as_float(i));
}

struct Runs9 {
  int2 r0, r1, r2, r3, r4, r5, r6, r7, r8;
};
__device__ __forceinline__ int2 pick9(int k, const Runs9& a) {
  int2 v = a.r0;
  v = (k == 1) ? a.r1 : v;
  v = (k == 2) ? a.r2 : v;
  v = (k == 3) ? a.r3 : v;
  v = (k == 4) ? a.r4 : v;
  v = (k == 5) ? a.r5 : v;
  v = (k == 6) ? a.r6 : v;
  v = (k == 7) ? a.r7 : v;
  v = (k == 8) ? a.r8 : v;
  return v;
}

__device__ __forceinline__ unsigned long long nbr_key(float d2, int id) {
  return ((unsigned long long)__float_as_uint(d2) << 32) | (unsigned)id;
}

static inline int nbr_row_cap(int limit) { return limit * 2 < 128 ? limit * 2 : 128; }

__global__ __launch_bounds__(256) void k_scan_table(
    const float* __restrict__ q_xyz, const int* __restrict__ q_cu, int nq, int nb,
    const GridCloud* __restrict__ info, const int* __restrict__ start,
    const float4* __restrict__ rec, const int* __restrict__ err, float r2, float inv_cell,
    int cap, int limit, int self, unsigned long long* __restrict__ tmp_key, int* __restrict__ kept_out,
    int* __restrict__ qid_out, int* max_count) {
  constexpr int kBins = 16;
  __shared__ unsigned short l_hist[kBins * 256];
  const int t = blockIdx.x * blockDim.x + threadIdx.x;
  if (*err) return;
  int total = 0;
  if (t < nq) {
    const int c = find_segment(q_cu, nb, t);
    const GridCloud g = info[c];
    int i = t;
    float qx, qy, qz;
    if (self) {
      const float4 me = rec[t];
      i = __float_as_int(me.w);
      qx = me.x, qy = me.y, qz = me.z;
    } else {
      qx = q_xyz[3 * (size_t)t + 0], qy = q_xyz[3 * (size_t)t + 1], qz = q_xyz[3 * (size_t)t + 2];
    }
    const int cx = cell_coord(qx, g.mn[0], inv_cell);
    const int cy = cell_coord(qy, g.mn[1], inv_cell);
    const int cz = cell_coord(qz, g.mn[2], inv_cell);
    const int xlo = max(cx - 1, 0), xhi = min(cx + 1, g.dim[0] - 1);
    auto run_of = [&](int k) -> int2 {
      const int z = cz + k / 3 - 1, y = cy + k % 3 - 1;
      const bool in = xlo <= xhi && z >= 0 && z < g.dim[2] && y >= 0 && y < g.dim[1];
      const long long L0 = in ? grid_cell(g, xlo, y, z) : 0;
      const long long L1 = in ? grid_cell(g, xhi, y, z) + 1 : 0;
      const int b = start[L0];
      return make_int2(b, in ? start[L1] : b);
    };
    Runs9 runs;
    runs.r0 = run_of(0); runs.r1 = run_of(1); runs.r2 = run_of(2);
    runs.r3 = run_of(3); runs.r4 = run_of(4); runs.r5 = run_of(5);
    runs.r6 = run_of(6); runs.r7 = run_of(7); runs.r8 = run_of(8);
    unsigned long long* const row = tmp_key + t;
    const size_t rs = (size_t)nq;
    int kept = 0;
    unsigned long long worst = 0;
    int w_pos = 0;
    const float bin_scale = (float)kBins / r2;
    unsigned short* my_hist = l_hist + threadIdx.x;
#pragma unroll
    for (int b = 0; b < kBins; ++b) my_hist[b * 256] = 0;
    int cut_bin = kBins;
    bool second = false;
    auto consider = [&](const float4 s) {
      const float dx = __fsub_rn(qx, s.x), dy = __fsub_rn(qy, s.y), dz = __fsub_rn(qz, s.z);
      float d2 = __fmul_rn(dx, dx);
      d2 = __fadd_rn(d2, __fmul_rn(dy, dy));
      d2 = __fadd_rn(d2, __fmul_rn(dz, dz));
      if (!(d2 < r2)) return;
      const int bin = min((int)(d2 * bin_scale), kBins - 1);
      if (!second) {
        total++;
        const unsigned short h = my_hist[bin * 256];
        my_hist[bin * 256] = h == 65535 ? h : (unsigned short)(h + 1);
        if (kept < cap) row[rs * kept++] = nbr_key(d2, __float_as_int(s.w));
        return;
      }
      if (bin > cut_bin) return;
      const unsigned long long key = nbr_key(d2, __float_as_int(s.w));
      if (kept < cap) {
        row[rs * kept] = key;
        if (kept == 0 || key > worst) {
          worst = key;
          w_pos = kept;
        }
        ++kept;
        return;
      }
      if (!(key < worst)) return;
      row[rs * w_pos] = key;
      __threadfence_block();
      worst = key;
      for (int k = 0; k < cap; ++k) {
        const unsigned long long rk = row[rs * k];
        if (rk > worst) {
          worst = rk;
          w_pos = k;
        }
      }
    };
    auto scan = [&]() {
      int k = 0, j = runs.r0.x, e = runs.r0.y;
      while (k < 9) {
        float4 s8[8];
        bool v8[8];
#pragma unroll
        for (int u = 0; u < 8; ++u) {
          while (k < 9 && j >= e) {
            ++k;
            const int2 r = pick9(k, runs);
            j = r.x;
            e = r.y;
          }
          v8[u] = k < 9;
          s8[u] = rec[v8[u] ? j : 0];
          j += v8[u] ? 1 : 0;
        }
#pragma unroll
        for (int u = 0; u < 8; ++u)
          if (v8[u]) consider(s8[u]);
      }
    };
    scan();
    if (total > cap) {
      int cum = 0;
      cut_bin = kBins - 1;
      for (int b = 0; b < kBins; ++b) {
        cum += my_hist[b * 256];
        if (cum >= limit) {
          cut_bin = b;
          break;
        }
      }
      second = true;
      kept = 0;
      scan();
    }
    kept_out[t] = kept;
    qid_out[t] = i;
  }
  int m = total;
#pragma unroll
  for (int o = 32; o > 0; o >>= 1) m = max(m, __shfl_xor(m, o, 64));
  if ((threadIdx.x & 63) == 0 && m > 0) atomicMax(max_count, m);
}

template <int BLOCK>
__global__ __launch_bounds__(BLOCK) void k_sort_rows(const unsigned long long* __restrict__ tmp_key,
                                                     const int* __restrict__ kept_in,
                                                     const int* __restrict__ qid_in,
                                                     const int* __restrict__ err, int nq, int ns,
                                                     int limit, int lslots, int* __restrict__ out) {
  extern __shared__ __align__(16) unsigned char smem[];
  unsigned long long* l_key = (unsigned long long*)smem;
  const int t = threadIdx.x;
  const int i = blockIdx.x * BLOCK + t;
  if (*err || i >= nq) return;
  const int kept = kept_in[i];
  const unsigned long long* src = tmp_key + i;
  const size_t rs = (size_t)nq;
  const int staged = min(kept, lslots);
  for (int k = 0; k < staged; ++k) l_key[k * BLOCK + t] = src[rs * k];
  auto key_at = [&](int k) { return k < lslots ? l_key[k * BLOCK + t] : src[rs * k]; };
  int* row = out + (size_t)qid_in[i] * limit;
  constexpr unsigned long long kInf = ~0ull;
  for (int a = 0; a < kept; a += 4) {
    const unsigned long long k0 = key_at(a);
    const unsigned long long k1 = a + 1 < kept ? key_at(a + 1) : kInf;
    const unsigned long long k2 = a + 2 < kept ? key_at(a + 2) : kInf;
    const unsigned long long k3 = a + 3 < kept ? key_at(a + 3) : kInf;
    int r0 = 0, r1 = 0, r2 = 0, r3 = 0;
    for (int b = 0; b < staged; ++b) {
      const unsigned long long kb = l_key[b * BLOCK + t];
      r0 += kb < k0 ? 1 : 0;
      r1 += kb < k1 ? 1 : 0;
      r2 += kb < k2 ? 1 : 0;
      r3 += kb < k3 ? 1 : 0;
    }
    for (int b = staged; b < kept; ++b) {
      const unsigned long long kb = src[rs * b];
      r0 += kb < k0 ? 1 : 0;
      r1 += kb < k1 ? 1 : 0;
      r2 += kb < k2 ? 1 : 0;
      r3 += kb < k3 ? 1 : 0;
    }
    if (r0 < limit) row[r0] = (int)(unsigned)k0;
    if (a + 1 < kept && r1 < limit) row[r1] = (int)(unsigned)k1;
    if (a + 2 < kept && r2 < limit) row[r2] = (int)(unsigned)k2;
    if (a + 3 < kept && r3 < limit) row[r3] = (int)(unsigned)k3;
  }
  for (int k = kept; k < limit; ++k) row[k] = ns;
}

constexpr int kKnnChunk = 16;

__device__ __forceinline__ unsigned long long readlane_u64(unsigned long long v, int l) {
  const unsigned lo = __builtin_amdgcn_readlane((int)(unsigned)v, l);
  const unsigned hi = __builtin_amdgcn_readlane((int)(unsigned)(v >> 32), l);
  return ((unsigned long long)hi << 32) | lo;
}

template <bool BIG>
__global__ __launch_bounds__(256) void k_knn_wave(
    const float* __restrict__ q_xyz, const int* __restrict__ q_cu, int nq, int nb,
    const GridCloud* __restrict__ info, const int* __restrict__ start, const float4* __restrict__ rec,
    const int* __restrict__ err, float r2, float inv_cell, int limit, int self, int ns, int* __restrict__ out,
    int* max_count, int* q_ctr) {
  __shared__ unsigned long long s_key[4][128];
  const int lane = threadIdx.x & 63, wave = threadIdx.x >> 6;
  if (*err) return;
  unsigned long long* sk = s_key[wave];
  constexpr unsigned long long kNone = ~0ull;
  int cl_lo = 0, cl_hi = 0;
  GridCloud g = info[0];
  int wave_max = 0;
  for (;;) {
    int c0 = 0;
    if (lane == 0) c0 = atomicAdd(q_ctr, kKnnChunk);
    c0 = __builtin_amdgcn_readfirstlane(c0);
    if (c0 >= nq) break;
    const int c1 = min(c0 + kKnnChunk, nq);
    for (int t = c0; t < c1; ++t) {
      if (t < cl_lo || t >= cl_hi) {
        const int c = find_segment(q_cu, nb, t);
        cl_lo = q_cu[c];
        cl_hi = q_cu[c + 1];
        g = info[c];
      }
      int qi = t;
      float qx, qy, qz;
      if (self) {
        const float4 me = rec[t];
        qi = __float_as_int(me.w);
        qx = me.x, qy = me.y, qz = me.z;
      } else {
        qx = q_xyz[3 * (size_t)t + 0], qy = q_xyz[3 * (size_t)t + 1], qz = q_xyz[3 * (size_t)t + 2];
      }
      const int cx = cell_coord(qx, g.mn[0], inv_cell);
      const int cy = cell_coord(qy, g.mn[1], inv_cell);
      const int cz = cell_coord(qz, g.mn[2], inv_cell);
      const int xlo = max(cx - 1, 0), xhi = min(cx + 1, g.dim[0] - 1);
      int rb = 0, re = 0;
      if (lane < 9) {
        const int z = cz + lane / 3 - 1, y = cy + lane % 3 - 1;
        const bool in = xlo <= xhi && z >= 0 && z < g.dim[2] && y >= 0 && y < g.dim[1];
        if (in) {
          rb = start[grid_cell(g, xlo, y, z)];
          re = start[grid_cell(g, xhi, y, z) + 1];
        }
      }
      const int len = re - rb;
      int pre = len;
#pragma unroll
      for (int o = 1; o < 16; o <<= 1) {
        const int v = __shfl_up(pre, o, 64);
        if (lane >= o) pre += v;
      }
      const int n_c = __builtin_amdgcn_readlane(pre, 8);
      const int ex = pre - len;
      int roff[9], rdel[9];
#pragma unroll
      for (int k = 0; k < 9; ++k) {
        roff[k] = __builtin_amdgcn_readlane(ex, k);
        rdel[k] = __builtin_amdgcn_readlane(rb, k) - roff[k];
      }
      unsigned long long lk0 = kNone, lk1 = kNone;
      int cnt = 0, total = 0;
      auto fetch = [&](int base) __attribute__((always_inline)) -> float4 {
        const int ci = base + lane;
        int d = rdel[0];
#pragma unroll
        for (int k = 1; k < 9; ++k) d = ci >= roff[k] ? rdel[k] : d;
        return rec[ci < n_c ? ci + d : 0];
      };
      float4 sp_next = make_float4(0.f, 0.f, 0.f, 0.f);
      if (n_c > 0) sp_next = fetch(0);
      for (int base = 0; base < n_c; base += 64) {
        const int ci = base + lane;
        const bool valid = ci < n_c;
        const float4 sp = sp_next;
        if (base + 64 < n_c) sp_next = fetch(base + 64);
        const float dx = __fsub_rn(qx, sp.x), dy = __fsub_rn(qy, sp.y), dz = __fsub_rn(qz, sp.z);
        float d2 = __fmul_rn(dx, dx);
        d2 = __fadd_rn(d2, __fmul_rn(dy, dy));
        d2 = __fadd_rn(d2, __fmul_rn(dz, dz));
        bool in = valid && d2 < r2;
        const unsigned long long key = nbr_key(d2, __float_as_int(sp.w));
        unsigned long long m = __builtin_amdgcn_ballot_w64(in);
        total += __popcll(m);
        if (cnt == limit) {
          const unsigned long long worst = (!BIG || limit <= 64) ? readlane_u64(lk0, limit - 1) : readlane_u64(lk1, limit - 65);
          in = in && key < worst;
          m = __builtin_amdgcn_ballot_w64(in);
        }
        if (m == 0) continue;
        int sh0 = 0, sh1 = 0, myrank = 0;
        for (unsigned long long mm = m; mm != 0; mm &= mm - 1) {
          const int jl = __builtin_ctzll(mm);
          const unsigned long long kj = readlane_u64(key, jl);
          int nl = __popcll(__builtin_amdgcn_ballot_w64(lk0 < kj));
          sh0 += kj < lk0 ? 1 : 0;
          if (BIG) {
            nl += __popcll(__builtin_amdgcn_ballot_w64(lk1 < kj));
            sh1 += kj < lk1 ? 1 : 0;
          }
          nl += __popcll(__builtin_amdgcn_ballot_w64(in && key < kj));
          if (lane == jl) myrank = nl;
        }
        if (lk0 != kNone && lane + sh0 < limit) sk[lane + sh0] = lk0;
        if (BIG && lk1 != kNone && 64 + lane + sh1 < limit) sk[64 + lane + sh1] = lk1;
        if (in && myrank < limit) sk[myrank] = key;
        cnt = min(cnt + (int)__popcll(m), limit);
        asm volatile("s_waitcnt lgkmcnt(0)" ::: "memory");
        lk0 = lane < cnt ? sk[lane] : kNone;
        if (BIG) lk1 = 64 + lane < cnt ? sk[64 + lane] : kNone;
        asm volatile("s_waitcnt lgkmcnt(0)" ::: "memory");
      }
      int* row = out + (size_t)qi * limit;
      if (lane < limit) row[lane] = lane < cnt ? (int)(unsigned)lk0 : ns;
      if (BIG && 64 + lane < limit) row[64 + lane] = 64 + lane < cnt ? (int)(unsigned)lk1 : ns;
      wave_max = max(wave_max, total);
    }
  }
  if (lane == 0 && wave_max > 0 && wave_max > *reinterpret_cast<volatile int*>(max_count)) atomicMax(max_count, wave_max);
}

template <int B, int E, class F>
__device__ __forceinline__ void static_for(F&& f) {
  if constexpr (B < E) {
    f(std::integral_constant<int, B>{});
    static_for<B + 1, E>(f);
  }
}

template <int N>
__global__ __launch_bounds__(256) void k_sort_rows_reg(const unsigned long long* __restrict__ tmp_key,
                                                       const int* __restrict__ kept_in, const int* __restrict__ qid_in,
                                                       const int* __restrict__ err, int nq, int ns, int limit,
                                                       int* __restrict__ out) {
  static_assert(N % 8 == 0, "rows in chunks of eight");
  const int i = blockIdx.x * 256 + threadIdx.x;
  if (*err) return;
  const bool act = i < nq;
  const int kept = act ? min(kept_in[i], N) : 0;
  int kmax = kept;
#pragma unroll
  for (int o = 32; o > 0; o >>= 1) kmax = max(kmax, __shfl_xor(kmax, o, 64));
  kmax = __builtin_amdgcn_readfirstlane(kmax);
  const unsigned long long* src = tmp_key + (act ? i : 0);
  const size_t rs = (size_t)nq;
  unsigned long long key[N];
  static_for<0, N>([&](auto kc) { key[decltype(kc)::value] = ~0ull; });
  static_for<0, N / 8>([&](auto cc) {
    constexpr int k0 = 8 * decltype(cc)::value;
    if (k0 < kmax) {
      static_for<k0, k0 + 8>([&](auto kc) {
        constexpr int k = decltype(kc)::value;
        if (k < kept) key[k] = src[rs * k];
      });
    }
  });
  int* row = out + (size_t)(act ? qid_in[i] : 0) * limit;
  static_for<0, N>([&](auto ac) {
    constexpr int a = decltype(ac)::value;
    if (a < kmax) {
      int r = 0;
      static_for<0, N / 8>([&](auto cc) {
        constexpr int b0 = 8 * decltype(cc)::value;
        if (b0 < kmax) {
          static_for<b0, b0 + 8>([&](auto bc) { r += key[decltype(bc)::value] < key[a] ? 1 : 0; });
        }
      });
      if (a < kept && r < limit) row[r] = (int)(unsigned)key[a];
    }
  });
  if (act)
    for (int k = kept; k < limit; ++k) row[k] = ns;
}

__global__ void k_nbr_err2(const int* hdr, int slot, int* max_count) {
  const int err = hdr[kHdrErr];
  if (err & 1) *max_count = -1;
  else if (err & 2) *max_count = -2;
  else *max_count = hdr[kHdrSlot0 + slot];
}

size_t table_cap_cells(int ns) { return (size_t)64 * (size_t)(ns > 0 ? ns : 1) + ((size_t)1 << 20); }

size_t table_cells_alloc(int ns) { return align_up(table_cap_cells(ns) + 1, kScanBlock); }
struct TableView {
  int* hdr;
  GridCloud* ginfo;
  int* start;
  float4* rec;
};
size_t table_bytes(int ns, int nb) {
  return align_up(64 * sizeof(int), 256) + align_up(sizeof(GridCloud) * (size_t)(nb > 0 ? nb : 1), 256) +
         align_up(4 * table_cells_alloc(ns), 256) + align_up(16 * (size_t)(ns > 0 ? ns : 1), 256);
}
TableView table_view(void* blob, int ns, int nb) {
  Workspace w(blob, table_bytes(ns, nb));
  TableView t;
  t.hdr = w.take<int>(64);
  t.ginfo = w.take<GridCloud>(nb > 0 ? nb : 1);
  t.start = w.take<int>(table_cells_alloc(ns));
  t.rec = w.take<float4>(ns > 0 ? ns : 1);
  return t;
}
size_t table_build_ws_bytes(int ns) {
  return 2 * align_up(4 * (size_t)(ns > 0 ? ns : 1), 256) + align_up(4 * (table_cells_alloc(ns) / kScanBlock), 256);
}
size_t table_query_ws_bytes(int nq) {
  const size_t Q = (size_t)(nq > 0 ? nq : 1);
  return align_up(8 * Q * 128, 256) + 2 * align_up(4 * Q, 256);
}

int table_build(const float* s_xyz, const int* s_cu, int ns, int nb, float radius, void* blob, void* ws,
                size_t ws_bytes, hipStream_t stream) {
  const TableView t = table_view(blob, ns, nb);
  Workspace w(ws, ws_bytes);
  int* cell_of = w.take<int>((size_t)ns);
  int* rank = w.take<int>((size_t)ns);
  const int nblk = (int)(table_cells_alloc(ns) / kScanBlock);
  int* bsum = w.take<int>((size_t)nblk);
  SPR_REQUIRE(bsum != nullptr, "radius table: workspace carve failed");
  const float inv_cell = 1.0f / (radius * (1.0f + 1.0f / 256.0f));
  const int TB = 256;
  SPR_HIP_CHECK(hipMemsetAsync(t.hdr, 0, 8 * sizeof(int), stream));
  hipLaunchKernelGGL(k_grid_dims, dim3(nb), dim3(256), 0, stream, s_xyz, s_cu, inv_cell, t.ginfo, t.hdr + kHdrErr);
  hipLaunchKernelGGL(k_grid_offsets, dim3(1), dim3(64), 0, stream, t.ginfo, nb, (long long)table_cap_cells(ns), t.hdr);
  hipLaunchKernelGGL(k_table_zero, dim3(nblk), dim3(256), 0, stream, t.hdr, t.start);
  hipLaunchKernelGGL(k_cell_count, dim3(cdiv(ns, TB)), dim3(TB), 0, stream, s_xyz, s_cu, ns, nb, inv_cell, t.ginfo,
                     t.hdr + kHdrErr, t.start, cell_of, rank);
  hipLaunchKernelGGL(k_table_bsum, dim3(nblk), dim3(256), 0, stream, t.hdr, t.start, bsum);
  hipLaunchKernelGGL(k_table_scan, dim3(nblk), dim3(256), 0, stream, t.hdr, t.start, bsum);
  hipLaunchKernelGGL(k_cell_scatter, dim3(cdiv(ns, TB)), dim3(TB), 0, stream, s_xyz, ns, t.hdr + kHdrErr, cell_of,
                     t.start, rank, t.rec);
  SPR_LAUNCH_CHECK();
  return 0;
}

int table_query(const float* q_xyz, const int* q_cu, int nq, int self, int ns, int nb, float radius, int limit,
                int slot, const void* blob, int* out_idx, int* max_count, void* ws, size_t ws_bytes,
                hipStream_t stream, int algo = -1) {
  const TableView t = table_view(const_cast<void*>(blob), ns, nb);
  Workspace w(ws, ws_bytes);
  constexpr int kRegRows = 64;
  const bool use_reg = limit <= kRegRows;
  const int rcap = use_reg ? min(nbr_row_cap(limit), kRegRows) : nbr_row_cap(limit);
  unsigned long long* tmp_key = w.take<unsigned long long>((size_t)nq * rcap);
  int* kept = w.take<int>((size_t)nq);
  int* qid = w.take<int>((size_t)nq);
  SPR_REQUIRE(qid != nullptr, "radius query: workspace carve failed");
  const float r2 = radius * radius;
  const float inv_cell = 1.0f / (radius * (1.0f + 1.0f / 256.0f));
  if (algo == 1) {
    SPR_HIP_CHECK(hipMemsetAsync(qid, 0, sizeof(int), stream));
    const int nblk = min(cdiv(nq, 4 * kKnnChunk), 8 * device_cu_count());
    if (limit <= 64)
      hipLaunchKernelGGL(k_knn_wave<false>, dim3(nblk), dim3(256), 0, stream, q_xyz, q_cu, nq, nb, t.ginfo, t.start, t.rec,
                         t.hdr + kHdrErr, r2, inv_cell, limit, self, ns, out_idx, t.hdr + kHdrSlot0 + slot, qid);
    else
      hipLaunchKernelGGL(k_knn_wave<true>, dim3(nblk), dim3(256), 0, stream, q_xyz, q_cu, nq, nb, t.ginfo, t.start, t.rec,
                         t.hdr + kHdrErr, r2, inv_cell, limit, self, ns, out_idx, t.hdr + kHdrSlot0 + slot, qid);
    hipLaunchKernelGGL(k_nbr_err2, dim3(1), dim3(1), 0, stream, t.hdr, slot, max_count);
    SPR_LAUNCH_CHECK();
    return 0;
  }
  hipLaunchKernelGGL(k_scan_table, dim3(cdiv(nq, 256)), dim3(256), 0, stream, q_xyz, q_cu, nq, nb, t.ginfo, t.start,
                     t.rec, t.hdr + kHdrErr, r2, inv_cell, rcap, limit, self, tmp_key, kept, qid, t.hdr + kHdrSlot0 + slot);
  if (use_reg) {
    hipLaunchKernelGGL(k_sort_rows_reg<kRegRows>, dim3(cdiv(nq, 256)), dim3(256), 0, stream, tmp_key, kept, qid,
                       t.hdr + kHdrErr, nq, ns, limit, out_idx);
    hipLaunchKernelGGL(k_nbr_err2, dim3(1), dim3(1), 0, stream, t.hdr, slot, max_count);
    SPR_LAUNCH_CHECK();
    return 0;
  }
  constexpr int BLOCK = 64;
  hipLaunchKernelGGL(k_sort_rows<BLOCK>, dim3(cdiv(nq, BLOCK)), dim3(BLOCK), (size_t)rcap * 8 * BLOCK, stream, tmp_key,
                     kept, qid, t.hdr + kHdrErr, nq, ns, limit, rcap, out_idx);
  hipLaunchKernelGGL(k_nbr_err2, dim3(1), dim3(1), 0, stream, t.hdr, slot, max_count);
  SPR_LAUNCH_CHECK();
  return 0;
}

__global__ void k_nbr_err(const int* err, int* max_count) {
  if (*err) *max_count = -1;
}

size_t nbr_sort_temp_bytes(int n) {
  size_t bytes = 0;
  rocprim::radix_sort_pairs(nullptr, bytes, (unsigned long long*)nullptr,
                            (unsigned long long*)nullptr, (int*)nullptr, (int*)nullptr,
                            (unsigned int)(n > 0 ? n : 1));
  return align_up(bytes, 256) + 256;
}

}
}

using namespace spr;

extern "C" size_t spr_radius_neighbors_workspace_bytes(int nq, int ns, int nb) {
  const size_t N = (size_t)(ns > 0 ? ns : 1), B = (size_t)(nb > 0 ? nb : 1);
  size_t b = 0;
  b += align_up(sizeof(NbrCloud) * B, 256);
  b += 2 * align_up(8 * N, 256);
  b += 2 * align_up(4 * N, 256);
  b += align_up(16 * N, 256);
  b += 256;
  b += nbr_sort_temp_bytes(ns);
  b += table_bytes(ns, nb) + table_build_ws_bytes(ns) + table_query_ws_bytes(nq);
  return b;
}

extern "C" int spr_radius_neighbors(const float* q_xyz, const int* q_cu, int nq,
                                    const float* s_xyz, const int* s_cu, int ns, int nb,
                                    float radius, int limit, int algo, int* out_idx,
                                    int* max_count, void* ws, size_t ws_bytes, void* stream_) {
  hipStream_t stream = (hipStream_t)stream_;
  SPR_REQUIRE(nq > 0 && ns > 0 && nb >= 1, "radius_neighbors: empty input (nq=%d ns=%d)", nq, ns);
  SPR_REQUIRE(nb < 65536, "radius_neighbors: at most 65535 clouds per call");
  SPR_REQUIRE(radius > 0.f, "radius_neighbors: radius must be > 0");
  SPR_REQUIRE(limit >= 1 && limit <= 128, "radius_neighbors: limit must be in [1,128], got %d", limit);
  SPR_REQUIRE(ws_bytes >= spr_radius_neighbors_workspace_bytes(nq, ns, nb),
              "radius_neighbors: workspace too small");
  Workspace w(ws, ws_bytes);
  const size_t N = (size_t)ns;
  NbrCloud* info = w.take<NbrCloud>(nb);
  unsigned long long* keys = w.take<unsigned long long>(N);
  unsigned long long* keys2 = w.take<unsigned long long>(N);
  int* vals = w.take<int>(N);
  int* vals2 = w.take<int>(N);
  float4* rec = w.take<float4>(N);
  int* err = w.take<int>(16);
  size_t temp_bytes = nbr_sort_temp_bytes(ns);
  void* temp = w.take<char>(temp_bytes);
  SPR_REQUIRE(temp != nullptr, "radius_neighbors: workspace carve failed");

  const int TB = 256;
  if (algo == 0) {
    void* blob = w.take<char>(table_bytes(ns, nb));
    const size_t bws = table_build_ws_bytes(ns), qws = table_query_ws_bytes(nq);
    void* build_ws = w.take<char>(bws);
    void* query_ws = w.take<char>(qws);
    SPR_REQUIRE(query_ws != nullptr, "radius_neighbors: workspace carve failed (table)");
    if (int rc = table_build(s_xyz, s_cu, ns, nb, radius, blob, build_ws, bws, stream)) return rc;
    return table_query(q_xyz, q_cu, nq, (q_xyz == s_xyz && q_cu == s_cu && nq == ns) ? 1 : 0, ns, nb, radius, limit, 0,
                       blob, out_idx, max_count, query_ws, qws, stream);
  }
  const float r2 = radius * radius;
  const float inv_cell = 1.0f / (radius * (1.0f + 1.0f / 256.0f));
  SPR_HIP_CHECK(hipMemsetAsync(err, 0, 16 * sizeof(int), stream));
  SPR_HIP_CHECK(hipMemsetAsync(max_count, 0, sizeof(int), stream));
  hipLaunchKernelGGL(k_min, dim3(nb), dim3(256), 0, stream, s_xyz, s_cu, info);
  hipLaunchKernelGGL(k_cellkeys, dim3(cdiv(ns, TB)), dim3(TB), 0, stream, s_xyz, s_cu, ns, nb,
                     inv_cell, info, keys, vals, err);
  SPR_LAUNCH_CHECK();
  size_t tb = temp_bytes;
  SPR_HIP_CHECK(rocprim::radix_sort_pairs(temp, tb, keys, keys2, vals, vals2,
                                          (unsigned int)ns, 0, 64, stream));
  hipLaunchKernelGGL(k_gather_sorted, dim3(cdiv(ns, TB)), dim3(TB), 0, stream, s_xyz, vals2, ns,
                     rec);
  if (limit <= 64) {
    constexpr int BLOCK = 128;
    const size_t lds = (size_t)limit * BLOCK * 8;
    hipLaunchKernelGGL(k_query<BLOCK>, dim3(cdiv(nq, BLOCK)), dim3(BLOCK), lds, stream, q_xyz,
                       q_cu, nq, s_cu, ns, nb, info, keys2, rec, r2, inv_cell, limit, out_idx,
                       max_count);
  } else {
    constexpr int BLOCK = 64;
    const size_t lds = (size_t)limit * BLOCK * 8;
    hipLaunchKernelGGL(k_query<BLOCK>, dim3(cdiv(nq, BLOCK)), dim3(BLOCK), lds, stream, q_xyz,
                       q_cu, nq, s_cu, ns, nb, info, keys2, rec, r2, inv_cell, limit, out_idx,
                       max_count);
  }
  hipLaunchKernelGGL(k_nbr_err, dim3(1), dim3(1), 0, stream, err, max_count);
  SPR_LAUNCH_CHECK();
  return 0;
}

extern "C" size_t spr_radius_table_bytes(int ns, int nb) { return table_bytes(ns, nb); }
extern "C" size_t spr_radius_table_build_workspace_bytes(int ns, int nb) { (void)nb; return table_build_ws_bytes(ns); }
extern "C" size_t spr_radius_table_query_workspace_bytes(int nq) { return table_query_ws_bytes(nq); }
extern "C" int spr_radius_table_slots(void) { return kTableSlots; }

extern "C" int spr_radius_table_build(const float* s_xyz, const int* s_cu, int ns, int nb, float radius, void* table,
                                      size_t table_bytes_, void* ws, size_t ws_bytes, void* stream_) {
  SPR_REQUIRE(s_xyz && s_cu && table && ns > 0 && nb >= 1 && nb < 65536, "radius_table_build: bad arguments");
  SPR_REQUIRE(radius > 0.f, "radius_table_build: radius must be > 0");
  SPR_REQUIRE(table_bytes_ >= table_bytes(ns, nb) && ((uintptr_t)table & 255) == 0, "radius_table_build: table too small or misaligned");
  SPR_REQUIRE(ws != nullptr && ws_bytes >= table_build_ws_bytes(ns), "radius_table_build: workspace too small");
  return table_build(s_xyz, s_cu, ns, nb, radius, table, ws, ws_bytes, (hipStream_t)stream_);
}

extern "C" int spr_radius_table_query(const float* q_xyz, const int* q_cu, int nq, int self, int ns, int nb,
                                      float radius, int limit, int slot, const void* table, int* out_idx,
                                      int* max_count, int algo, void* ws, size_t ws_bytes, void* stream_) {
  SPR_REQUIRE(q_xyz && q_cu && table && out_idx && max_count && nq > 0 && ns > 0 && nb >= 1, "radius_table_query: bad arguments");
  SPR_REQUIRE(limit >= 1 && limit <= 128, "radius_table_query: limit must be in [1,128], got %d", limit);
  SPR_REQUIRE(slot >= 0 && slot < kTableSlots, "radius_table_query: slot out of range");
  SPR_REQUIRE(!self || nq == ns, "radius_table_query: a self search has nq == ns");
  SPR_REQUIRE(algo >= -1 && algo <= 1,
              "radius_table_query: algo must be 0 (thread per query), 1 (wave per query) or -1 (the library's choice)");
  SPR_REQUIRE(ws != nullptr && ws_bytes >= table_query_ws_bytes(nq), "radius_table_query: workspace too small");
  return table_query(q_xyz, q_cu, nq, self ? 1 : 0, ns, nb, radius, limit, slot, table, out_idx, max_count, ws, ws_bytes,
                     (hipStream_t)stream_, algo);
}
```

### superpoints_registration_amd/csrc/spr_common.h

```cpp
#pragma once
#include <hip/hip_runtime.h>

#include <cstdarg>
#include <cstdio>
#include <cstdint>
#include <cstring>

#include "../../include/spr.h"

namespace spr {

constexpr int kWave = 64;

void set_error(const char* fmt, ...);

#define SPR_HIP_CHECK(expr)                                                   \
  do {                                                                        \
    hipError_t _e = (expr);                                                   \
    if (_e != hipSuccess) {                                                   \
      ::spr::set_error("%s failed: %s (%s:%d)", #expr, hipGetErrorString(_e), \
                       __FILE__, __LINE__);                                   \
      return 1;                                                               \
    }                                                                         \
  } while (0)

#define SPR_LAUNCH_CHECK()                                                  \
  do {                                                                      \
    hipError_t _e = hipGetLastError();                                      \
    if (_e != hipSuccess) {                                                 \
      ::spr::set_error("kernel launch failed: %s (%s:%d)",                  \
                       hipGetErrorString(_e), __FILE__, __LINE__);          \
      return 1;                                                             \
    }                                                                       \
  } while (0)

#define SPR_REQUIRE(cond, ...)        \
  do {                                \
    if (!(cond)) {                    \
      ::spr::set_error(__VA_ARGS__);  \
      return 2;                       \
    }                                 \
  } while (0)

static inline size_t align_up(size_t x, size_t a) { return (x + a - 1) / a * a; }
static inline int cdiv(long a, long b) { return (int)((a + b - 1) / b); }

struct Workspace {
  char* base;
  size_t size;
  size_t off;
  Workspace(void* p, size_t n) : base((char*)p), size(n), off(0) {}
  template <typename T>
  T* take(size_t count) {
    size_t bytes = align_up(count * sizeof(T), 256);
    if (off + bytes > size) return nullptr;
    T* r = (T*)(base + off);
    off += bytes;
    return r;
  }
};

bool prof_enabled();
void prof_push(hipEvent_t beg, hipEvent_t end, int code, int n);
struct ProfScope {
  hipStream_t stream;
  bool on;
  hipEvent_t beg, end;
  int code, n;
  ProfScope(hipStream_t s, int code_, int n_) : stream(s), on(prof_enabled()), code(code_), n(n_) {
    if (!on) return;
    if (hipEventCreate(&beg) != hipSuccess || hipEventCreate(&end) != hipSuccess) {
      on = false;
      return;
    }
    (void)hipEventRecord(beg, stream);
  }
  ~ProfScope() {
    if (!on) return;
    (void)hipEventRecord(end, stream);
    prof_push(beg, end, code, n);
  }
};

int ensure_dyn_lds(const void* kernel, int bytes);
int device_cu_count();

int launch_absmax(const float* x, long rows, int cols, long stride, float* parts, hipStream_t stream);
int launch_absmax2(const float* x0, long rows0, int cols0, long stride0, float* parts0, const float* x1,
                   long rows1, int cols1, long stride1, float* parts1, hipStream_t stream);

#ifdef __HIPCC__
typedef float f32x4 __attribute__((ext_vector_type(4)));
typedef float f32x16 __attribute__((ext_vector_type(16)));

__device__ __forceinline__ int find_segment(const int* __restrict__ cu, int nseg,
                                            int i) {
  int lo = 0, hi = nseg;
  while (hi - lo > 1) {
    int mid = (lo + hi) >> 1;
    if (cu[mid] <= i)
      lo = mid;
    else
      hi = mid;
  }
  return lo;
}

__device__ __forceinline__ int xcd_swizzle(int b, int nwg) {
  const int q = nwg >> 3, r = nwg & 7;
  const int xcd = b & 7, idx = b >> 3;
  const int base = (xcd < r) ? xcd * (q + 1) : r * (q + 1) + (xcd - r) * q;
  return base + idx;
}

typedef _Float16 spr_h16x2 __attribute__((ext_vector_type(2)));
__device__ __forceinline__ void split_pk(float a, float b, unsigned int& hi_u, unsigned int& lo_u) {
  const spr_h16x2 hi = {(_Float16)a, (_Float16)b};
  hi_u = __builtin_bit_cast(unsigned int, hi);
  asm("v_fma_mixlo_f16 %0, %1, -1.0, %2 op_sel_hi:[1,0,0]\n\t"
      "v_fma_mixhi_f16 %0, %1, -1.0, %3 op_sel:[1,0,0] op_sel_hi:[1,0,0]"
      : "=&v"(lo_u)
      : "v"(hi_u), "v"(a), "v"(b));
}

__device__ __forceinline__ void split_pk_s(float a, float b, float s, unsigned int& hi_u,
                                           unsigned int& lo_u) {
  asm("v_fma_mixlo_f16 %0, %1, %3, 0 op_sel_hi:[0,0,0]\n\t"
      "v_fma_mixhi_f16 %0, %2, %3, 0 op_sel_hi:[0,0,0]"
      : "=&v"(hi_u)
      : "v"(a), "v"(b), "v"(s));
  asm("v_fma_mixlo_f16 %0, %2, %4, -%1 op_sel_hi:[0,0,1]\n\t"
      "v_fma_mixhi_f16 %0, %3, %4, -%1 op_sel:[0,0,1] op_sel_hi:[0,0,1]"
      : "=&v"(lo_u)
      : "v"(hi_u), "v"(a), "v"(b), "v"(s));
}

__device__ __forceinline__ void split_pk_s_hi(float a, float b, float s, unsigned int& hi_u) {
  asm("v_fma_mixlo_f16 %0, %1, %3, 0 op_sel_hi:[0,0,0]\n\t"
      "v_fma_mixhi_f16 %0, %2, %3, 0 op_sel_hi:[0,0,0]"
      : "=&v"(hi_u)
      : "v"(a), "v"(b), "v"(s));
}
__device__ __forceinline__ void split_pk_s_lo(float a, float b, float s, unsigned int hi_u, unsigned int& lo_u) {
  asm("v_fma_mixlo_f16 %0, %2, %4, -%1 op_sel_hi:[0,0,1]\n\t"
      "v_fma_mixhi_f16 %0, %3, %4, -%1 op_sel:[0,0,1] op_sel_hi:[0,0,1]"
      : "=&v"(lo_u)
      : "v"(hi_u), "v"(a), "v"(b), "v"(s));
}

__host__ __device__ __forceinline__ int pow2_exp_for(float amax) {
  if (!(amax > 0.f) || !(amax < 3.0e38f)) return 0;
  unsigned int u;
#ifdef __HIP_DEVICE_COMPILE__
  u = __float_as_uint(amax);
#else
  memcpy(&u, &amax, 4);
#endif
  const int e = (int)((u >> 23) & 0xff) - 127;
  int k = 14 - e;
  if (k > 60) k = 60;
  if (k < -60) k = -60;
  return k;
}
__host__ __device__ __forceinline__ float pow2f(int k) {
  const unsigned int u = (unsigned int)(127 + k) << 23;
  float f;
#ifdef __HIP_DEVICE_COMPILE__
  f = __uint_as_float(u);
#else
  memcpy(&f, &u, 4);
#endif
  return f;
}

constexpr int kAmaxParts = 512;
constexpr int kRangeSlots = 64;
__device__ __forceinline__ float block_absmax(const float* __restrict__ parts, float* sh, int n = kAmaxParts) {
  float m = 0.f;
  for (int i = threadIdx.x; i < n; i += blockDim.x) m = fmaxf(m, parts[i]);
#pragma unroll
  for (int o = 32; o > 0; o >>= 1) m = fmaxf(m, __shfl_xor(m, o, 64));
  if ((threadIdx.x & 63) == 0) sh[threadIdx.x >> 6] = m;
  __syncthreads();
  if (threadIdx.x == 0) {
    float t = sh[0];
    for (int w = 1; w < (int)(blockDim.x >> 6); ++w) t = fmaxf(t, sh[w]);
    sh[16] = t;
  }
  __syncthreads();
  return sh[16];
}

__device__ __forceinline__ float wave_sum(float v) {
#pragma unroll
  for (int o = 32; o > 0; o >>= 1) v += __shfl_xor(v, o, 64);
  return v;
}
__device__ __forceinline__ double wave_sum_d(double v) {
#pragma unroll
  for (int o = 32; o > 0; o >>= 1) v += __shfl_xor(v, o, 64);
  return v;
}
__device__ __forceinline__ float wave_max(float v) {
#pragma unroll
  for (int o = 32; o > 0; o >>= 1) v = fmaxf(v, __shfl_xor(v, o, 64));
  return v;
}
#endif

}
```

### superpoints_registration_amd/hip_shim.py

```python
import ctypes
import os

import numpy as np
import torch

_LIB = os.environ.get("SPR_HIP_LIB") or os.path.join(os.path.dirname(os.path.abspath(__file__)), "libspr_hip.so")
_L = None


def _lib():
    global _L
    if _L is None:
        L = ctypes.CDLL(_LIB)
        L.spr_grid_subsample_workspace_bytes.restype = ctypes.c_size_t
        L.spr_radius_neighbors_workspace_bytes.restype = ctypes.c_size_t
        L.spr_last_error.restype = ctypes.c_char_p
        _L = L
    return _L


def _p(t):
    return ctypes.c_void_p(t.data_ptr())


def _cu(lens, dev):
    cu = np.zeros(len(lens) + 1, np.int32)
    cu[1:] = np.cumsum(np.asarray(lens, dtype=np.int64))
    return torch.from_numpy(cu).to(dev)


def _stream(dev):
    return ctypes.c_void_p(torch.cuda.current_stream(dev).cuda_stream)


def _raise(L):
    msg = L.spr_last_error()
    raise RuntimeError(msg.decode() if msg else "Error")


class cpp_subsampling:

    @staticmethod
    def subsample_batch(points, batches, sampleDl=0.1, max_p=0, verbose=0):
        L = _lib()
        dev = torch.device("cuda")
        x = torch.as_tensor(np.ascontiguousarray(points, dtype=np.float32)).to(dev)
        n, nb = int(x.shape[0]), len(batches)
        if n < 1 or nb < 1 or int(np.sum(batches)) != n:
            raise RuntimeError("Error converting input to numpy arrays of the right type")
        ws = torch.empty(L.spr_grid_subsample_workspace_bytes(n, nb), dtype=torch.uint8, device=dev)
        out = torch.empty((n, 3), dtype=torch.float32, device=dev)
        lens = torch.empty(nb, dtype=torch.int32, device=dev)
        tot = torch.empty(1, dtype=torch.int32, device=dev)
        cu = _cu(batches, dev)
        rc = L.spr_grid_subsample(_p(x), _p(cu), n, nb, ctypes.c_float(sampleDl), int(max_p), 0,
                                  _p(out), _p(lens), _p(tot), _p(ws), ctypes.c_size_t(ws.numel()), _stream(dev))
        if rc:
            _raise(L)
        m = int(tot.item())
        if m < 0:
            raise RuntimeError("voxel grid too large for 40-bit keys")
        return out[:m].cpu().numpy(), lens.cpu().numpy()


class cpp_neighbors:

    @staticmethod
    def batch_query(queries, supports, q_batches, s_batches, radius=0.1, limit=128):
        L = _lib()
        dev = torch.device("cuda")
        q = torch.as_tensor(np.ascontiguousarray(queries, dtype=np.float32)).to(dev)
        s = torch.as_tensor(np.ascontiguousarray(supports, dtype=np.float32)).to(dev)
        nq, ns, nb = int(q.shape[0]), int(s.shape[0]), len(q_batches)
        if nq < 1 or ns < 1 or nb < 1 or len(s_batches) != nb:
            raise RuntimeError("Error")
        ws = torch.empty(L.spr_radius_neighbors_workspace_bytes(nq, ns, nb), dtype=torch.uint8, device=dev)
        out = torch.empty((nq, limit), dtype=torch.int32, device=dev)
        mc = torch.empty(1, dtype=torch.int32, device=dev)
        m = -2
        q_cu, s_cu = _cu(q_batches, dev), _cu(s_batches, dev)
        for algo in (0, 1):
            rc = L.spr_radius_neighbors(_p(q), _p(q_cu), nq, _p(s), _p(s_cu), ns, nb,
                                        ctypes.c_float(radius), int(limit), algo, _p(out), _p(mc), _p(ws),
                                        ctypes.c_size_t(ws.numel()), _stream(dev))
            if rc:
                _raise(L)
            m = int(mc.item())
            if m != -2:
                break
        if m < 1:
            raise RuntimeError("Error")
        return out[:, :min(m, limit)].cpu().numpy()
```

### superpoints_registration_amd/kpconv.py

```python
from dataclasses import dataclass
from typing import List

import torch
import torch.nn as nn

from . import ops
from .kpconv_blocks import block_decider

_DOWN = ('pool', 'strided')
_STOP = ('global', 'upsample')


@dataclass
class BlockPlan:
    name: str
    level: int
    radius: float
    in_dim: int
    out_dim: int
    down: bool


@dataclass
class LevelPlan:
    radius: float
    has_conv: bool
    down: bool
    limit: int


def plan_pyramid(cfg):
    r = cfg.first_subsampling_dl * cfg.conv_radius
    in_dim, out_dim, level = cfg.in_feats_dim, cfg.first_feats_dim, 0
    blocks: List[BlockPlan] = []
    members: List[List[BlockPlan]] = [[]]
    for name in cfg.architecture:
        if any(s in name for s in _STOP):
            break
        down = any(s in name for s in _DOWN)
        bp = BlockPlan(name, level, r, in_dim, out_dim, down)
        blocks.append(bp)
        members[-1].append(bp)
        in_dim = out_dim // 2 if 'simple' in name else out_dim
        if down:
            level += 1
            r *= 2
            out_dim *= 2
            members.append([])
    if not members[-1]:
        members.pop()
    levels = []
    for l, mem in enumerate(members):
        levels.append(LevelPlan(radius=mem[0].radius,
                                has_conv=any(not b.down for b in mem),
                                down=mem[-1].down,
                                limit=int(cfg.neighborhood_limits[l])))
    return blocks, levels, in_dim


class KPFEncoder(nn.Module):

    def __init__(self, config, d_bottle, increase_channel_when_downsample=True):
        super().__init__()
        if not increase_channel_when_downsample:
            raise NotImplementedError("constant-width pyramids are not used by RegTR")
        blocks, _, final_dim = plan_pyramid(config)
        self._plans = blocks
        self.encoder_blocks = nn.ModuleList(
            block_decider(b.name, b.radius, b.in_dim, b.out_dim, b.level, config) for b in blocks)
        self.encoder_skips = [i for i, b in enumerate(blocks) if b.down]
        self.encoder_skip_dims = [b.in_dim for b in blocks if b.down]
        self.encoder_skips.append(len(blocks) - 1)
        self.encoder_skip_dims.append(final_dim)

    def forward(self, x, batch):
        skip_x = []
        for i, block in enumerate(self.encoder_blocks):
            if i in self.encoder_skips:
                skip_x.append(x)
            x = block(x, batch)
        return x, skip_x

    def forward_streamed(self, x, stream):
        plans = self._plans
        skip_x, i, meta = [], 0, None
        for meta, kind, level in stream:
            while i < len(self.encoder_blocks):
                bp = plans[i]
                ready = bp.level < level or (bp.level == level and (kind == 'down' or not bp.down))
                if not ready:
                    break
                if i in self.encoder_skips:
                    skip_x.append(x)
                x = self.encoder_blocks[i](x, meta)
                i += 1
        assert i == len(self.encoder_blocks), "pyramid ended before the encoder"
        return x, skip_x, meta


def batch_grid_subsampling_kpconv(points, batches_len, features=None, labels=None, sampleDl=0.1,
                                  max_p=0, verbose=0, random_grid_orient=True,
                                  order=ops.ORDER_REFERENCE):
    if features is not None or labels is not None:
        raise NotImplementedError('subsampling with features / labels is not on the RegTR path')
    return ops.grid_subsample(points, ops.lengths_to_cu(batches_len, points.device), sampleDl,
                              max_p=max_p, order=order)


def batch_neighbors_kpconv(queries, supports, q_batches, s_batches, radius, max_neighbors):
    limit = int(max_neighbors) if max_neighbors > 0 else 128
    idx, _ = ops.radius_neighbors(queries, supports,
                                  ops.lengths_to_cu(q_batches, queries.device),
                                  ops.lengths_to_cu(s_batches, queries.device),
                                  radius, limit, exact_width=True)
    return idx


batch_grid_subsampling_kpconv_gpu = batch_grid_subsampling_kpconv
batch_neighbors_kpconv_gpu = batch_neighbors_kpconv


class _IndexList(list):

    def __init__(self, dtype):
        super().__init__()
        self._dtype = dtype

    def _conv(self, i):
        t = list.__getitem__(self, i)
        if t.dtype != self._dtype:
            t = t.to(self._dtype)
            list.__setitem__(self, i, t)
        return t

    def __getitem__(self, i):
        if isinstance(i, slice):
            return [self._conv(j) for j in range(*i.indices(len(self)))]
        return self._conv(i if i >= 0 else len(self) + i)

    def __iter__(self):
        return (self._conv(i) for i in range(len(self)))


class Preprocessor(nn.Module):

    def __init__(self, cfg, compute_upsamples=True, order=ops.ORDER_REFERENCE,
                 index_dtype=torch.int64):
        super().__init__()
        self.cfg = cfg
        self.compute_upsamples = compute_upsamples
        self.order = order
        self.index_dtype = index_dtype
        self._row_counts = {}

    def forward(self, pts: List[torch.Tensor]):
        meta = None
        for meta, _, _ in self.stream(pts):
            pass
        return meta

    def stream(self, pts: List[torch.Tensor]):
        cfg = self.cfg
        _, levels, _ = plan_pyramid(cfg)
        device = pts[0].device
        points = torch.cat(pts, dim=0).to(torch.float32).contiguous()
        lens_host = [int(p.shape[0]) for p in pts]

        meta = {k: [] for k in ('points', 'stack_lengths')}
        meta.update({k: _IndexList(self.index_dtype) for k in ('neighbors', 'pools', 'upsamples')})
        meta.update(_cu={}, _i32={}, _lens_host=[], _rows_sorted=True, pool_order=[])
        placeholder = torch.zeros((0, 1), dtype=self.index_dtype, device=device)

        def publish(key, level, idx):
            if idx is None:
                meta[key].append(placeholder)
                return
            meta['_i32'][(key, level)] = idx
            meta[key].append(idx)
            if key != 'upsamples':
                ops.kpconv_plan_prefetch(idx, plan_ns[0])

        plan_ns = [0]

        def open_level(l, points, lens_host, cu):
            meta['points'].append(points)
            meta['stack_lengths'].append(torch.tensor(lens_host, dtype=torch.int32, device=device))
            meta['_cu'][l] = cu
            meta['_lens_host'].append(lens_host)

        table = [None]

        def search(key, queries, q_cu, supports, s_cu, radius, limit):
            if table[0] is None or not table[0].matches(supports, s_cu, radius):
                table[0] = ops.RadiusTable(supports, s_cu, radius)
            prev = self._row_counts.get(key)
            idx, m = table[0].query(queries, q_cu, limit, dense=None if prev is None else prev > 1.5 * limit)
            self._row_counts[key] = m
            return idx

        cu = ops.lengths_to_cu(lens_host, device)
        open_level(0, points, lens_host, cu)
        for l, lv in enumerate(levels):
            conv = pool = up = None
            plan_ns[0] = points.shape[0]
            if lv.has_conv:
                conv = search((l, 'conv'), points, cu, points, cu, lv.radius, lv.limit)
            publish('neighbors', l, conv)
            yield meta, 'conv', l
            if lv.down:
                dl = 2 * lv.radius / cfg.conv_radius
                sub_points, sub_lens = ops.grid_subsample(points, cu, dl, order=self.order)
                sub_lens_host = sub_lens.tolist()
                sub_cu = ops.lengths_to_cu(sub_lens_host, device)
                pool = search((l, 'pool'), sub_points, sub_cu, points, cu, lv.radius, lv.limit)
                meta['pool_order'].append(ops.cell_order(sub_points, sub_cu, dl))
                if self.compute_upsamples:
                    up = search((l, 'up'), points, cu, sub_points, sub_cu, 2 * lv.radius, lv.limit)
            if not lv.down:
                meta['pool_order'].append(None)
            publish('pools', l, pool)
            publish('upsamples', l, up)
            if lv.down:
                points, lens_host, cu = sub_points, sub_lens_host, sub_cu
                open_level(l + 1, points, lens_host, cu)
            yield meta, 'down', l


PreprocessorGPU = Preprocessor
```

### superpoints_registration_amd/ops.py

```python
import ctypes
import math
import threading
from typing import Optional, Sequence, Tuple

import numpy as np
import torch

from . import _lib

ACT_NONE, ACT_RELU, ACT_SIGMOID = 0, 1, 2
ORDER_REFERENCE, ORDER_CANONICAL = 0, 1


def _stream(t: torch.Tensor):
    return ctypes.c_void_p(torch.cuda.current_stream(t.device).cuda_stream)


def _ptr(t: Optional[torch.Tensor]):
    return None if t is None else ctypes.c_void_p(t.data_ptr())


def _dev(t: torch.Tensor, name: str, dtype=None) -> torch.Tensor:
    if not isinstance(t, torch.Tensor) or not t.is_cuda:
        raise RuntimeError(f"{name} must be a tensor on the MI355X device (got "
                           f"{t.device if isinstance(t, torch.Tensor) else type(t)}); "
                           "the HIP path has no CPU fallback")
    if dtype is not None and t.dtype != dtype:
        t = t.to(dtype)
    return t.contiguous()


_ws_cache = {}


_range_epoch = [0]


def invalidate_ranges() -> None:
    _range_epoch[0] += 1


def _set_range(t: torch.Tensor, parts: torch.Tensor, n: int, guard=None) -> None:
    if n > 0:
        t._spr_range = (parts, int(n), t._version, t.data_ptr(), _range_epoch[0], guard)


def _get_range(t):
    r = getattr(t, '_spr_range', None)
    if r is None or r[2] != t._version or r[3] != t.data_ptr() or r[4] != _range_epoch[0]:
        return None, 0
    if r[5] is not None:
        r[5].acquire()
    return r[0], r[1]

_RANGE_CAP = 4096
_STREAM_SLOTS = 512
_zero_pool = {}


def _zero_slots(n: int, device) -> torch.Tensor:
    key = (device, torch.cuda.current_stream(device).cuda_stream)
    pool = _zero_pool.get(key)
    if pool is None or pool[1] + n > pool[0].numel():
        pool = [torch.zeros(1 << 18, dtype=torch.float32, device=device), 0]
        _zero_pool[key] = pool
    out = pool[0][pool[1]:pool[1] + n]
    pool[1] += n
    return out


class _StreamGuard:

    def __init__(self, buf: torch.Tensor):
        self.stream = torch.cuda.current_stream(buf.device)
        self.event = torch.cuda.Event()
        self.event.record(self.stream)
        self.buf = buf
        self.seen = {self.stream.cuda_stream}

    def acquire(self):
        cur = torch.cuda.current_stream(self.buf.device)
        if cur.cuda_stream not in self.seen:
            cur.wait_event(self.event)
            self.buf.record_stream(cur)
            self.seen.add(cur.cuda_stream)


def _static_range(w: torch.Tensor):
    r, n = _get_range(w)
    if r is not None:
        return r, n
    L = _lib.lib()
    n = L.spr_range_parts()
    flat = w.reshape(-1, w.shape[-1])
    parts = torch.empty((n,), dtype=torch.float32, device=w.device)
    _lib.check(L.spr_absmax(_ptr(flat), flat.shape[0], flat.shape[1], flat.shape[1], _ptr(parts), _stream(w)),
               "spr_absmax")
    _set_range(w, parts, n, _StreamGuard(parts))
    return parts, n


_PRIME_PARTS = 16


def prime_weight_ranges(params) -> int:
    todo = [p for p in params if isinstance(p, torch.Tensor) and p.is_cuda and p.dtype == torch.float32
            and p.dim() >= 2 and p.is_contiguous() and p.numel() > 0 and _get_range(p)[0] is None]
    if not todo:
        return 0
    dev = todo[0].device
    todo = [p for p in todo if p.device == dev]
    rec = np.zeros((len(todo), 2), dtype=np.int64)
    for i, p in enumerate(todo):
        rec[i, 0] = p.data_ptr()
        rec[i, 1] = p.numel()
    jobs = torch.from_numpy(rec).to(dev)
    parts = torch.empty((len(todo), _PRIME_PARTS), dtype=torch.float32, device=dev)
    _lib.check(_lib.lib().spr_absmax_multi(_ptr(jobs), len(todo), _PRIME_PARTS, _ptr(parts), _stream(parts)),
               "spr_absmax_multi")
    guard = _StreamGuard(parts)
    for i, p in enumerate(todo):
        _set_range(p, parts[i], _PRIME_PARTS, guard)
    return len(todo)


def weight_transposed(w: torch.Tensor) -> torch.Tensor:
    c = getattr(w, '_spr_wt', None)
    if c is not None and c[1] == w._version and c[2] == w.data_ptr() and c[3] == _range_epoch[0]:
        c[4].acquire()
        return c[0]
    wt = w.detach().t().contiguous()
    r, n = _static_range(w)
    if r is not None:
        rw = getattr(w, '_spr_range', None)
        _set_range(wt, r, n, rw[5] if rw is not None else None)
    w._spr_wt = (wt, w._version, w.data_ptr(), _range_epoch[0], _StreamGuard(wt))
    return wt


def ensure_range(t: torch.Tensor) -> torch.Tensor:
    if t.dim() != 2 or not t.is_contiguous() or _get_range(t)[0] is not None:
        return t
    L = _lib.lib()
    n = L.spr_range_parts()
    parts = torch.empty((n,), dtype=torch.float32, device=t.device)
    _lib.check(L.spr_absmax(_ptr(t), t.shape[0], t.shape[1], t.shape[1], _ptr(parts), _stream(t)), "spr_absmax")
    _set_range(t, parts, n)
    return t


def _workspace(nbytes: int, device) -> torch.Tensor:
    key = (device, torch.cuda.current_stream(device).cuda_stream)
    buf = _ws_cache.get(key)
    if buf is None or buf.numel() < nbytes:
        buf = torch.empty(max(int(nbytes), 1 << 20), dtype=torch.uint8, device=device)
        _ws_cache[key] = buf
    return buf


def lengths_to_cu(lengths, device) -> torch.Tensor:
    if isinstance(lengths, torch.Tensor):
        l = lengths.to(device=device, dtype=torch.int32)
        cu = torch.zeros(l.numel() + 1, dtype=torch.int32, device=device)
        cu[1:] = torch.cumsum(l, 0)
        return cu
    arr = np.zeros(len(lengths) + 1, dtype=np.int32)
    arr[1:] = np.cumsum(np.asarray(lengths, dtype=np.int64))
    return torch.from_numpy(arr).to(device)


def selftest() -> None:
    st = ctypes.c_int(-1)
    _lib.check(_lib.lib().spr_selftest(ctypes.byref(st)), "spr_selftest")


def grid_subsample(points: torch.Tensor, cu: torch.Tensor, dl: float, max_p: int = 0,
                   order: int = ORDER_REFERENCE) -> Tuple[torch.Tensor, torch.Tensor]:
    points = _dev(points, "points", torch.float32)
    cu = _dev(cu, "cu", torch.int32)
    n, nb = points.shape[0], cu.numel() - 1
    L = _lib.lib()
    ws = _workspace(L.spr_grid_subsample_workspace_bytes(n, nb), points.device)
    out = torch.empty((max(n, 1), 3), dtype=torch.float32, device=points.device)
    out_lens = torch.empty((nb,), dtype=torch.int32, device=points.device)
    total = torch.empty((1,), dtype=torch.int32, device=points.device)
    _lib.check(L.spr_grid_subsample(_ptr(points), _ptr(cu), n, nb, float(dl), int(max_p), int(order),
                                    _ptr(out), _ptr(out_lens), _ptr(total), _ptr(ws), ws.numel(),
                                    _stream(points)), "spr_grid_subsample")
    m = int(total.item())
    if m < 0:
        raise RuntimeError("spr_grid_subsample: voxel grid too large for 40-bit keys")
    return out[:m], out_lens


def voxel_downsample(points: torch.Tensor, voxel_size: float) -> torch.Tensor:
    points = _dev(points, "points", torch.float32)
    n = points.shape[0]
    L = _lib.lib()
    ws = _workspace(L.spr_voxel_downsample_workspace_bytes(n), points.device)
    idx = torch.empty((n,), dtype=torch.int32, device=points.device)
    cnt = torch.empty((1,), dtype=torch.int32, device=points.device)
    _lib.check(L.spr_voxel_downsample(_ptr(points), n, float(voxel_size), _ptr(idx), _ptr(cnt), _ptr(ws), ws.numel(),
                                      _stream(points)), "spr_voxel_downsample")
    m = int(cnt.item())
    if m < 0:
        raise RuntimeError("spr_voxel_downsample: coordinates exceed 2^20 voxels")
    return points[idx[:m].long()]


def radius_neighbors(queries: torch.Tensor, supports: torch.Tensor, q_cu: torch.Tensor,
                     s_cu: torch.Tensor, radius: float, limit: int,
                     exact_width: bool = True, algo: int = 0) -> Tuple[torch.Tensor, int]:
    queries = _dev(queries, "queries", torch.float32)
    supports = _dev(supports, "supports", torch.float32)
    q_cu = _dev(q_cu, "q_cu", torch.int32)
    s_cu = _dev(s_cu, "s_cu", torch.int32)
    nq, ns, nb = queries.shape[0], supports.shape[0], q_cu.numel() - 1
    L = _lib.lib()
    ws = _workspace(L.spr_radius_neighbors_workspace_bytes(nq, ns, nb), queries.device)
    out = torch.empty((nq, limit), dtype=torch.int32, device=queries.device)
    mc = torch.empty((1,), dtype=torch.int32, device=queries.device)
    _lib.check(L.spr_radius_neighbors(_ptr(queries), _ptr(q_cu), nq, _ptr(supports), _ptr(s_cu), ns,
                                      nb, float(radius), int(limit), int(algo), _ptr(out), _ptr(mc),
                                      _ptr(ws), ws.numel(), _stream(queries)), "spr_radius_neighbors")
    if not exact_width:
        return out, -1
    m = int(mc.item())
    if m == -2 and algo == 0:
        return radius_neighbors(queries, supports, q_cu, s_cu, radius, limit, exact_width, algo=1)
    if m < 0:
        raise RuntimeError("spr_radius_neighbors: cloud extent / radius exceeds 8191 cells per axis")
    if m < 1:
        raise RuntimeError("Error")
    return out[:, :min(m, limit)], m


def gt_overlap(src_xyz: torch.Tensor, src_cu: torch.Tensor, tgt_xyz: torch.Tensor, tgt_cu: torch.Tensor,
               pose: torch.Tensor, radius: float):
    src_xyz = _dev(src_xyz, "src_xyz", torch.float32)
    tgt_xyz = _dev(tgt_xyz, "tgt_xyz", torch.float32)
    src_cu = _dev(src_cu, "src_cu", torch.int32)
    tgt_cu = _dev(tgt_cu, "tgt_cu", torch.int32)
    pose = _dev(pose, "pose", torch.float32)
    ns, nt, nb = src_xyz.shape[0], tgt_xyz.shape[0], src_cu.numel() - 1
    if tgt_cu.numel() - 1 != nb or tuple(pose.shape) != (nb, 3, 4):
        raise ValueError(f"gt_overlap: {nb} source clouds, {tgt_cu.numel() - 1} target clouds, pose {tuple(pose.shape)}")
    dev = src_xyz.device
    L = _lib.lib()
    ws = _workspace(L.spr_gt_overlap_workspace_bytes(ns, nt, nb), dev)
    src_corr = torch.empty((ns,), dtype=torch.int32, device=dev)
    tgt_corr = torch.empty((nt,), dtype=torch.int32, device=dev)
    src_mask = torch.empty((ns,), dtype=torch.uint8, device=dev)
    tgt_mask = torch.empty((nt,), dtype=torch.uint8, device=dev)
    corr = torch.empty((2, ns), dtype=torch.int32, device=dev)
    count = torch.zeros((max(nb, 1),), dtype=torch.int32, device=dev)
    _lib.check(L.spr_gt_overlap(_ptr(src_xyz), _ptr(src_cu), ns, _ptr(tgt_xyz), _ptr(tgt_cu), nt, _ptr(pose), nb,
                                float(radius), _ptr(src_corr), _ptr(tgt_corr), _ptr(src_mask), _ptr(tgt_mask),
                                _ptr(corr), _ptr(count), _ptr(ws), ws.numel(), _stream(src_xyz)), "spr_gt_overlap")
    counts = count[:nb].tolist()
    if any(c < 0 for c in counts):
        raise RuntimeError("spr_gt_overlap: non-finite coordinates or pose")
    return src_corr, tgt_corr, src_mask.view(torch.bool), tgt_mask.view(torch.bool), corr, counts


AUG_MODES = {'none': 0, 'small': 1, 'large': 2}


def philox4x32(counter, key) -> np.ndarray:
    c = np.ascontiguousarray(counter, dtype=np.uint32).reshape(4)
    k = np.ascontiguousarray(key, dtype=np.uint32).reshape(2)
    out = np.zeros(4, dtype=np.uint32)
    _lib.check(_lib.lib().spr_philox4x32_host(c.ctypes.data, k.ctypes.data, out.ctypes.data), "spr_philox4x32_host")
    return out


def augment_draw(seed: int, pair_keys, mode: str, src_cu: Optional[torch.Tensor] = None,
                 tgt_cu: Optional[torch.Tensor] = None, ns: int = 0, nt: int = 0):
    pk = np.ascontiguousarray(pair_keys, dtype=np.uint64).reshape(-1)
    nb = pk.size
    psrc = np.zeros(nb, dtype=np.uint8)
    swap = np.zeros(nb, dtype=np.uint8)
    perturb = np.zeros((nb, 3, 4), dtype=np.float32)
    L = _lib.lib()
    if src_cu is None:
        _lib.check(L.spr_augment_draw(int(seed), pk.ctypes.data, nb, AUG_MODES[mode], psrc.ctypes.data, swap.ctypes.data,
                                      perturb.ctypes.data, None, None, 0, None, 0, None, None, None), "spr_augment_draw")
        return psrc.astype(bool), swap.astype(bool), perturb
    src_cu = _dev(src_cu, "src_cu", torch.int32)
    tgt_cu = _dev(tgt_cu, "tgt_cu", torch.int32)
    if src_cu.numel() - 1 != nb or tgt_cu.numel() - 1 != nb:
        raise ValueError(f"augment_draw: {nb} pair keys, cu arrays of {src_cu.numel() - 1} / {tgt_cu.numel() - 1} clouds")
    dev = src_cu.device
    pk_dev = torch.from_numpy(pk.view(np.int64)).to(dev)
    noise = torch.empty((ns + nt, 3), dtype=torch.float32, device=dev)
    keys = torch.empty((ns + nt,), dtype=torch.int32, device=dev)
    _lib.check(L.spr_augment_draw(int(seed), pk.ctypes.data, nb, AUG_MODES[mode], psrc.ctypes.data, swap.ctypes.data,
                                  perturb.ctypes.data, _ptr(pk_dev), _ptr(src_cu), int(ns), _ptr(tgt_cu), int(nt),
                                  _ptr(noise), _ptr(keys), _stream(src_cu)), "spr_augment_draw")
    return psrc.astype(bool), swap.astype(bool), perturb, noise, keys


def augment_pairs(src_xyz: torch.Tensor, src_cu: torch.Tensor, tgt_xyz: torch.Tensor, tgt_cu: torch.Tensor,
                  pose: torch.Tensor, perturb_src, swap, perturb, mode: str, scale: float, max_pts: int = 30000,
                  seed: int = 0, pair_keys=None, src_mask: Optional[torch.Tensor] = None,
                  tgt_mask: Optional[torch.Tensor] = None, corr: Optional[torch.Tensor] = None, corr_off=None,
                  corr_count=None, noise: Optional[torch.Tensor] = None, keys: Optional[torch.Tensor] = None,
                  out_lens=None) -> dict:
    src_xyz = _dev(src_xyz, "src_xyz", torch.float32)
    tgt_xyz = _dev(tgt_xyz, "tgt_xyz", torch.float32)
    src_cu = _dev(src_cu, "src_cu", torch.int32)
    tgt_cu = _dev(tgt_cu, "tgt_cu", torch.int32)
    pose = _dev(pose, "pose", torch.float32)
    dev = src_xyz.device
    ns, nt, nb = src_xyz.shape[0], tgt_xyz.shape[0], src_cu.numel() - 1
    if tgt_cu.numel() - 1 != nb or tuple(pose.shape) != (nb, 3, 4):
        raise ValueError(f"augment_pairs: {nb} source clouds, {tgt_cu.numel() - 1} target clouds, pose {tuple(pose.shape)}")
    flags_h = (np.asarray(perturb_src, dtype=bool).reshape(-1).astype(np.uint8)
               | (np.asarray(swap, dtype=bool).reshape(-1).astype(np.uint8) << 1))
    if flags_h.size != nb:
        raise ValueError(f"augment_pairs: {flags_h.size} decisions for {nb} pairs")
    flags = torch.from_numpy(flags_h).to(dev)
    if isinstance(perturb, torch.Tensor):
        perturb_d = perturb.to(device=dev, dtype=torch.float32).contiguous()
    else:
        perturb_d = torch.from_numpy(np.ascontiguousarray(perturb, dtype=np.float32)).to(dev)
    if tuple(perturb_d.shape) != (nb, 3, 4):
        raise ValueError(f"augment_pairs: perturb {tuple(perturb_d.shape)} for {nb} pairs")
    pk_dev = None
    if pair_keys is not None:
        pk = np.ascontiguousarray(pair_keys, dtype=np.uint64).reshape(-1)
        if pk.size != nb:
            raise ValueError(f"augment_pairs: {pk.size} pair keys for {nb} pairs")
        pk_dev = torch.from_numpy(pk.view(np.int64)).to(dev)
    elif noise is None or keys is None:
        raise ValueError("augment_pairs: pair_keys are needed when noise or keys are generated inline")
    if (src_mask is None) != (tgt_mask is None):
        raise ValueError("augment_pairs: masks come for both clouds or for neither")
    if src_mask is not None:
        src_mask = _dev(src_mask, "src_mask").to(torch.uint8).contiguous()
        tgt_mask = _dev(tgt_mask, "tgt_mask").to(torch.uint8).contiguous()
        if src_mask.numel() != ns or tgt_mask.numel() != nt:
            raise ValueError("augment_pairs: mask length differs from the cloud's")
    if noise is not None:
        noise = _dev(noise, "noise", torch.float32)
        if tuple(noise.shape) != (ns + nt, 3):
            raise ValueError(f"augment_pairs: noise {tuple(noise.shape)}, expected {(ns + nt, 3)}")
    if keys is not None:
        keys = _dev(keys, "keys", torch.int32)
        if keys.numel() != ns + nt:
            raise ValueError(f"augment_pairs: {keys.numel()} keys for {ns + nt} points")
    stride = 0
    off_d = cnt_d = out_corr = out_cnt = None
    if corr is not None:
        corr = _dev(corr, "corr", torch.int32)
        stride = int(corr.shape[1])
        off_d = torch.from_numpy(np.ascontiguousarray(corr_off, dtype=np.int32).reshape(-1)).to(dev) \
            if not isinstance(corr_off, torch.Tensor) else _dev(corr_off, "corr_off", torch.int32)
        cnt_d = torch.from_numpy(np.ascontiguousarray(corr_count, dtype=np.int32).reshape(-1)).to(dev) \
            if not isinstance(corr_count, torch.Tensor) else _dev(corr_count, "corr_count", torch.int32)
        if off_d.numel() != nb or cnt_d.numel() != nb:
            raise ValueError("augment_pairs: corr_off / corr_count need one entry per pair")
        out_corr = torch.empty((2, stride), dtype=torch.int32, device=dev)
        out_cnt = torch.zeros((nb,), dtype=torch.int32, device=dev)
    if out_lens is not None:
        n_os, n_ot = int(sum(out_lens[0])), int(sum(out_lens[1]))
    else:
        n_os = n_ot = ns + nt
    L = _lib.lib()
    ws = _workspace(L.spr_augment_workspace_bytes(ns, nt, nb, stride), dev)
    o_src = torch.empty((n_os, 3), dtype=torch.float32, device=dev)
    o_tgt = torch.empty((n_ot, 3), dtype=torch.float32, device=dev)
    o_scu = torch.empty((nb + 1,), dtype=torch.int32, device=dev)
    o_tcu = torch.empty((nb + 1,), dtype=torch.int32, device=dev)
    o_pose = torch.empty((nb, 3, 4), dtype=torch.float32, device=dev)
    o_sperm = torch.empty((n_os,), dtype=torch.int32, device=dev)
    o_tperm = torch.empty((n_ot,), dtype=torch.int32, device=dev)
    o_smask = torch.empty((n_os,), dtype=torch.uint8, device=dev) if src_mask is not None else None
    o_tmask = torch.empty((n_ot,), dtype=torch.uint8, device=dev) if src_mask is not None else None
    status = torch.zeros((max(nb, 1),), dtype=torch.int32, device=dev)
    _lib.check(L.spr_augment_pairs(
        _ptr(src_xyz), _ptr(src_cu), ns, _ptr(tgt_xyz), _ptr(tgt_cu), nt, _ptr(pose), nb, _ptr(src_mask), _ptr(tgt_mask),
        _ptr(corr), stride, _ptr(off_d), _ptr(cnt_d), _ptr(perturb_d), _ptr(flags), AUG_MODES[mode], float(scale),
        int(max_pts), int(seed), _ptr(pk_dev), _ptr(noise), _ptr(keys), _ptr(o_src), _ptr(o_tgt), _ptr(o_scu),
        _ptr(o_tcu), _ptr(o_pose), _ptr(o_smask), _ptr(o_tmask), _ptr(o_sperm), _ptr(o_tperm), _ptr(out_corr),
        _ptr(out_cnt), _ptr(status), _ptr(ws), ws.numel(), _stream(src_xyz)), "spr_augment_pairs")
    out = {'src_xyz': o_src, 'tgt_xyz': o_tgt, 'src_cu': o_scu, 'tgt_cu': o_tcu, 'pose': o_pose, 'src_perm': o_sperm,
           'tgt_perm': o_tperm, 'status': status[:nb]}
    if src_mask is not None:
        out['src_mask'], out['tgt_mask'] = o_smask.view(torch.bool), o_tmask.view(torch.bool)
    if corr is not None:
        out['corr'], out['corr_count'] = out_corr, out_cnt
    return out


class RadiusTable:

    def __init__(self, supports: torch.Tensor, s_cu: torch.Tensor, radius: float):
        self.supports = _dev(supports, "supports", torch.float32)
        self.s_cu = _dev(s_cu, "s_cu", torch.int32)
        self.radius = float(radius)
        self.ns, self.nb = self.supports.shape[0], self.s_cu.numel() - 1
        L = _lib.lib()
        self.blob = torch.empty((L.spr_radius_table_bytes(self.ns, self.nb),), dtype=torch.uint8, device=supports.device)
        ws = _workspace(L.spr_radius_table_build_workspace_bytes(self.ns, self.nb), supports.device)
        _lib.check(L.spr_radius_table_build(_ptr(self.supports), _ptr(self.s_cu), self.ns, self.nb, self.radius,
                                            _ptr(self.blob), self.blob.numel(), _ptr(ws), ws.numel(),
                                            _stream(self.supports)), "spr_radius_table_build")
        self._slot = 0
        self._slots = L.spr_radius_table_slots()
        self._versions = (self.supports._version, self.s_cu._version)

    def matches(self, supports: torch.Tensor, s_cu: torch.Tensor, radius: float) -> bool:
        return (supports.data_ptr() == self.supports.data_ptr() and supports.shape[0] == self.ns
                and s_cu.data_ptr() == self.s_cu.data_ptr() and float(radius) == self.radius
                and (self.supports._version, self.s_cu._version) == self._versions
                and supports._version == self.supports._version and s_cu._version == self.s_cu._version
                and self._slot < self._slots)

    def query(self, queries: torch.Tensor, q_cu: torch.Tensor, limit: int,
              dense: Optional[bool] = None) -> Tuple[torch.Tensor, int]:
        queries = _dev(queries, "queries", torch.float32)
        q_cu = _dev(q_cu, "q_cu", torch.int32)
        nq = queries.shape[0]
        self_search = int(queries.data_ptr() == self.supports.data_ptr() and nq == self.ns
                          and q_cu.data_ptr() == self.s_cu.data_ptr())
        L = _lib.lib()
        ws = _workspace(L.spr_radius_table_query_workspace_bytes(nq), queries.device)
        out = torch.empty((nq, limit), dtype=torch.int32, device=queries.device)
        mc = torch.empty((1,), dtype=torch.int32, device=queries.device)
        slot, self._slot = self._slot, self._slot + 1
        _lib.check(L.spr_radius_table_query(_ptr(queries), _ptr(q_cu), nq, self_search, self.ns, self.nb, self.radius,
                                            int(limit), slot, _ptr(self.blob), _ptr(out), _ptr(mc),
                                            -1 if dense is None else int(bool(dense)), _ptr(ws), ws.numel(),
                                            _stream(queries)), "spr_radius_table_query")
        m = int(mc.item())
        if m == -2:
            return radius_neighbors(queries, self.supports, q_cu, self.s_cu, self.radius, limit, True, algo=1)
        if m < 0:
            raise RuntimeError("spr_radius_neighbors: cloud extent / radius exceeds 8191 cells per axis")
        if m < 1:
            raise RuntimeError("Error")
        return out[:, :min(m, limit)], m


def _wants_grad(*tensors) -> bool:
    return torch.is_grad_enabled() and any(isinstance(t, torch.Tensor) and t.requires_grad for t in tensors)


def kpconv(q_pts, s_pts, nbr, x, weights, kernel_points, kp_extent: float, rows_sorted: bool = False,
           impl: int = 0) -> torch.Tensor:
    if _wants_grad(x, weights):
        from .autograd import KPConvFn
        return KPConvFn.apply(_dev(q_pts, "q_pts", torch.float32), _dev(s_pts, "s_pts", torch.float32), nbr,
                              _dev(x, "x", torch.float32), weights, kernel_points, float(kp_extent),
                              bool(rows_sorted), int(impl))
    return kpconv_raw(q_pts, s_pts, nbr, x, weights, kernel_points, kp_extent, rows_sorted, impl)


def kpconv_raw(q_pts, s_pts, nbr, x, weights, kernel_points, kp_extent: float, rows_sorted: bool = False,
               impl: int = 0, order: Optional[torch.Tensor] = None) -> torch.Tensor:
    q_pts = _dev(q_pts, "q_pts", torch.float32)
    s_pts = _dev(s_pts, "s_pts", torch.float32)
    x = _dev(x, "x", torch.float32)
    weights = _dev(weights, "weights", torch.float32)
    kernel_points = _dev(kernel_points, "kernel_points", torch.float32)
    if not nbr.is_cuda:
        raise RuntimeError("neighb_inds must be on the device")
    if nbr.dtype != torch.int32:
        nbr = nbr.to(torch.int32)
    stride = nbr.stride(0) if nbr.stride(1) == 1 and nbr.shape[1] > 0 else None
    if stride is None:
        nbr = nbr.contiguous()
        stride = nbr.shape[1]
    nq, ns, kmax = q_pts.shape[0], s_pts.shape[0], nbr.shape[1]
    n_kp, cin, cout = weights.shape
    assert x.shape == (ns, cin), (x.shape, ns, cin)
    L = _lib.lib()
    ws = _workspace(L.spr_kpconv_workspace_bytes(nq, ns, cin, cout), x.device)
    out = torch.empty((nq, cout), dtype=torch.float32, device=x.device)
    xr, xr_n = _get_range(x)
    wr, wr_n = _static_range(weights)
    plan = wplanes = None
    if impl == 0 and n_kp == 15 and cin % 32 == 0 and cout % 32 == 0 and cout <= 256:
        if cin in (32, 64) and cin * cout <= 4096 and kmax <= 128:
            plan = _kpconv_plan(nbr, nq, ns, int(stride), kmax, bool(rows_sorted), order)
        if wr is not None:
            wplanes = _kpconv_wplanes(weights, wr, wr_n)
    _lib.check(L.spr_kpconv_fwd(_ptr(q_pts), nq, _ptr(s_pts), ns, _ptr(nbr), int(stride), kmax,
                                int(bool(rows_sorted)), _ptr(x), cin, _ptr(weights), cout,
                                _ptr(kernel_points), n_kp, float(kp_extent), _ptr(out), int(impl),
                                _ptr(xr), int(xr_n), _ptr(wr), int(wr_n), _ptr(plan), _ptr(wplanes),
                                _ptr(ws), ws.numel(), _stream(x)), "spr_kpconv_fwd")
    return out


def _kpconv_plan(nbr: torch.Tensor, nq: int, ns: int, stride: int, kmax: int, rows_sorted: bool,
                 order: Optional[torch.Tensor] = None) -> torch.Tensor:
    if order is not None:
        order = _dev(order, "order", torch.int32)
        assert order.shape == (nq,)
    key = (nbr.data_ptr(), nbr._version, nq, ns, stride, kmax, rows_sorted, _range_epoch[0],
           None if order is None else (order.data_ptr(), order._version))
    c = getattr(nbr, '_spr_kp_plan', None)
    if c is not None and c[0] == key:
        c[2].acquire()
        return c[1]
    L = _lib.lib()
    nbytes = L.spr_kpconv_plan_bytes(nq)
    plan = torch.empty((nbytes,), dtype=torch.uint8, device=nbr.device)
    _lib.check(L.spr_kpconv_plan(_ptr(nbr), nq, ns, stride, kmax, int(rows_sorted), _ptr(order), _ptr(plan), nbytes,
                                 _stream(nbr)), "spr_kpconv_plan")
    nbr._spr_kp_plan = (key, plan, _StreamGuard(plan))
    return plan


def kpconv_plan_prefetch(nbr: torch.Tensor, ns: int, rows_sorted: bool = True) -> None:
    if nbr is None or not nbr.is_cuda or nbr.dtype != torch.int32 or nbr.dim() != 2 or nbr.shape[1] < 1:
        return
    if nbr.stride(1) != 1 or nbr.shape[1] > 128 or nbr.shape[0] < 1:
        return
    _kpconv_plan(nbr, nbr.shape[0], int(ns), int(nbr.stride(0)), nbr.shape[1], bool(rows_sorted))


def _kpconv_wplanes(weights: torch.Tensor, wr: torch.Tensor, wr_n: int) -> torch.Tensor:
    key = (weights.data_ptr(), weights._version, wr.data_ptr(), _range_epoch[0])
    c = getattr(weights, '_spr_kp_wplanes', None)
    if c is not None and c[0] == key:
        c[2].acquire()
        return c[1]
    L = _lib.lib()
    n_kp, cin, cout = weights.shape
    nbytes = L.spr_kpconv_wplanes_bytes(cin, cout)
    planes = torch.empty((nbytes,), dtype=torch.uint8, device=weights.device)
    _lib.check(L.spr_kpconv_prep_weights(_ptr(weights), n_kp, cin, cout, _ptr(wr), int(wr_n), _ptr(planes), nbytes,
                                         _stream(weights)), "spr_kpconv_prep_weights")
    weights._spr_kp_wplanes = (key, planes, _StreamGuard(planes))
    return planes


def instnorm(x, cu, eps: float = 1e-5, norm: bool = True, add=None, slope: float = 1.0,
             out=None, max_len: Optional[int] = None) -> torch.Tensor:
    if _wants_grad(x, add):
        from .autograd import InstNormFn
        return InstNormFn.apply(_dev(x, "x", torch.float32), _dev(cu, "cu", torch.int32), float(eps), bool(norm),
                                None if add is None else _dev(add, "add", torch.float32), float(slope), max_len)
    return instnorm_raw(x, cu, eps, norm, add, slope, out, max_len)


def instnorm_raw(x, cu, eps: float = 1e-5, norm: bool = True, add=None, slope: float = 1.0,
                 out=None, max_len: Optional[int] = None) -> torch.Tensor:
    x = _dev(x, "x", torch.float32)
    cu = _dev(cu, "cu", torch.int32)
    n, c = x.shape
    nb = cu.numel() - 1
    if add is not None:
        add = _dev(add, "add", torch.float32)
        assert add.shape == x.shape
    if out is None:
        out = torch.empty_like(x)
    L = _lib.lib()
    max_len = n if max_len is None else max(1, min(int(max_len), n))
    ws = _workspace(L.spr_instnorm_workspace_bytes(max_len, nb, c), x.device)
    cnt = _STREAM_SLOTS
    rng = _zero_slots(cnt, x.device)
    _lib.check(L.spr_instnorm(_ptr(x), _ptr(cu), n, nb, max_len, c, float(eps), int(bool(norm)), _ptr(add),
                              float(slope), _ptr(out), _ptr(rng), cnt, _ptr(ws), ws.numel(), _stream(x)),
               "spr_instnorm")
    _set_range(out, rng, cnt)
    return out


def block_tail_tile_rows(ka: int, kb: int, n_out: int) -> int:
    if _modes["gemm"] != 1:
        return 0
    return int(_lib.lib().spr_block_tail_tile_rows(int(ka), int(kb), int(n_out)))


def _tail_tiles(cu: torch.Tensor, n: int, tr: int) -> torch.Tensor:
    key = (cu.data_ptr(), cu._version, n, tr, _range_epoch[0])
    cache = getattr(cu, '_spr_tail_tiles', None)
    if cache is None:
        cache = {}
        cu._spr_tail_tiles = cache
    c = cache.get(tr)
    if c is not None and c[0] == key:
        c[2].acquire()
        return c[1]
    L = _lib.lib()
    t = torch.empty((L.spr_block_tail_tiles_len(n, cu.numel() - 1, tr),), dtype=torch.int32, device=cu.device)
    _lib.check(L.spr_block_tail_tiles(_ptr(cu), n, cu.numel() - 1, tr, _ptr(t), _stream(cu)), "spr_block_tail_tiles")
    cache[tr] = (key, t, _StreamGuard(t))
    return t


def instnorm_stats(x, cu, eps: float = 1e-5, max_len: Optional[int] = None):
    x = _dev(x, "x", torch.float32)
    cu = _dev(cu, "cu", torch.int32)
    n, c = x.shape
    nb = cu.numel() - 1
    L = _lib.lib()
    max_len = n if max_len is None else max(1, min(int(max_len), n))
    ws = _workspace(L.spr_instnorm_workspace_bytes(max_len, nb, c), x.device)
    st = torch.empty((2, nb, c), dtype=torch.float32, device=x.device)
    _lib.check(L.spr_instnorm_stats(_ptr(x), _ptr(cu), n, nb, max_len, c, float(eps), _ptr(st[0]), _ptr(st[1]),
                                    _ptr(ws), ws.numel(), _stream(x)), "spr_instnorm_stats")
    return st[0], st[1]


_NORM_BOUNDS = {}


def _norm_bound(max_len: int, device) -> torch.Tensor:
    key = (int(max_len), str(device))
    t = _NORM_BOUNDS.get(key)
    if t is None:
        t = torch.full((1,), float(max(1, int(max_len))) ** 0.5, dtype=torch.float32, device=device)
        _NORM_BOUNDS[key] = t
    return t


def block_tail(xa, wa, cu, xb=None, wb=None, add=None, eps: float = 1e-5, slope: float = 0.1,
               xa_stats=None, xa_slope: float = 0.1, xa_max_len: Optional[int] = None) -> torch.Tensor:
    xa = _dev(xa, "xa", torch.float32)
    wa = _dev(wa, "wa", torch.float32)
    cu = _dev(cu, "cu", torch.int32)
    n, ka = xa.shape
    n_out = wa.shape[0]
    assert wa.shape[1] == ka
    kb = 0
    if xb is not None:
        xb = _dev(xb, "xb", torch.float32)
        wb = _dev(wb, "wb", torch.float32)
        kb = xb.shape[1]
        assert xb.shape[0] == n and wb.shape == (n_out, kb) and add is None
    if add is not None:
        add = _dev(add, "add", torch.float32)
        assert add.shape == (n, n_out)
    nb = cu.numel() - 1
    L = _lib.lib()
    tr = L.spr_block_tail_tile_rows(ka, kb, n_out)
    if tr <= 0:
        raise RuntimeError(f"block_tail: no kernel for ka={ka} kb={kb} n_out={n_out}")
    tiles = _tail_tiles(cu, n, tr)
    out = torch.empty((n, n_out), dtype=torch.float32, device=xa.device)
    ws = _workspace(L.spr_block_tail_workspace_bytes(n, nb, kb, n_out, tr), xa.device)
    if xa_stats is not None:
        xar, xar_n = _norm_bound(n if xa_max_len is None else xa_max_len, xa.device), 1
    else:
        xar, xar_n = _get_range(xa)
    war, war_n = _static_range(wa)
    xbr, xbr_n, wbr, wbr_n = None, 0, None, 0
    if kb > 0:
        xbr, xbr_n = _get_range(xb)
        wbr, wbr_n = _static_range(wb)
    cnt = _STREAM_SLOTS
    rng = _zero_slots(cnt, xa.device)
    mean = rstd = None
    if xa_stats is not None:
        mean, rstd = xa_stats
        assert mean.shape == (nb, ka) and rstd.shape == (nb, ka) and mean.is_contiguous() and rstd.is_contiguous()
    _lib.check(L.spr_block_tail(_ptr(xa), ka, _ptr(wa), _ptr(xb), kb, _ptr(wb), _ptr(add), _ptr(cu), _ptr(tiles),
                                n, nb, n_out, float(eps), float(slope), _ptr(out), _ptr(xar), int(xar_n),
                                _ptr(war), int(war_n), _ptr(xbr), int(xbr_n), _ptr(wbr), int(wbr_n),
                                _ptr(rng), cnt, _ptr(mean), _ptr(rstd), float(xa_slope), _ptr(ws), ws.numel(),
                                _stream(xa)), "spr_block_tail")
    _set_range(out, rng, cnt)
    return out


def cell_order(points: torch.Tensor, cu: torch.Tensor, cell: float) -> torch.Tensor:
    points = _dev(points, "points", torch.float32)
    cu = _dev(cu, "cu", torch.int32)
    n, nb = points.shape[0], cu.numel() - 1
    L = _lib.lib()
    out = torch.empty((n,), dtype=torch.int32, device=points.device)
    ws = _workspace(L.spr_cell_order_workspace_bytes(n), points.device)
    _lib.check(L.spr_cell_order(_ptr(points), _ptr(cu), n, nb, float(cell), _ptr(out), _ptr(ws), ws.numel(),
                                _stream(points)), "spr_cell_order")
    return out


def maxpool(x, idx, order=None) -> torch.Tensor:
    if _wants_grad(x):
        from .autograd import MaxPoolFn
        return MaxPoolFn.apply(_dev(x, "x", torch.float32), idx)
    return maxpool_raw(x, idx, order)


def maxpool_raw(x, idx, order=None) -> torch.Tensor:
    x = _dev(x, "x", torch.float32)
    if idx.dtype != torch.int32:
        idx = idx.to(torch.int32)
    stride = idx.stride(0) if idx.stride(1) == 1 else None
    if stride is None:
        idx = idx.contiguous()
        stride = idx.shape[1]
    ns, c = x.shape
    nq, k = idx.shape
    out = torch.empty((nq, c), dtype=torch.float32, device=x.device)
    L = _lib.lib()
    cnt = _STREAM_SLOTS
    rng = _zero_slots(cnt, x.device)
    if order is not None and (order.dtype != torch.int32 or order.numel() != nq or not order.is_contiguous()):
        raise ValueError("maxpool: order must be a contiguous int32 permutation of the query rows")
    _lib.check(L.spr_maxpool_gather(_ptr(x), ns, c, _ptr(idx), nq, int(stride), k, _ptr(order), _ptr(out),
                                    _ptr(rng), cnt, _stream(x)), "spr_maxpool_gather")
    _set_range(out, rng, cnt)
    return out


def linear(x, weight, bias=None, residual=None, act: int = ACT_NONE) -> torch.Tensor:
    if _wants_grad(x, weight, bias, residual):
        from .autograd import LinearFn
        return LinearFn.apply(_dev(x, "x", torch.float32), weight, bias, residual, int(act))
    return linear_raw(x, weight, bias, residual, act)


def linear_raw(x, weight, bias=None, residual=None, act: int = ACT_NONE) -> torch.Tensor:
    x = _dev(x, "x", torch.float32)
    weight = _dev(weight, "weight", torch.float32)
    m, k = x.shape
    n = weight.shape[0]
    assert weight.shape[1] == k
    if bias is not None:
        bias = _dev(bias, "bias", torch.float32)
    if residual is not None:
        residual = _dev(residual, "residual", torch.float32)
        assert residual.shape == (m, n)
    out = torch.empty((m, n), dtype=torch.float32, device=x.device)
    L = _lib.lib()
    ws = _workspace(L.spr_linear_workspace_bytes(), x.device)
    xr, xr_n = _get_range(x)
    wr, wr_n = _static_range(weight)
    orng = torch.empty((_RANGE_CAP,), dtype=torch.float32, device=x.device) if residual is None else None
    on = ctypes.c_int(0)
    _lib.check(L.spr_linear(_ptr(x), m, k, _ptr(weight), n, _ptr(bias), _ptr(residual), int(act), _ptr(out),
                            _ptr(xr), int(xr_n), _ptr(wr), int(wr_n), _ptr(orng),
                            _RANGE_CAP if orng is not None else 0, ctypes.byref(on),
                            _ptr(ws), ws.numel(), _stream(x)), "spr_linear")
    if orng is not None:
        _set_range(out, orng, on.value)
    return out


DEFAULT_ATTN_MODE = 4

_modes = {"gemm": 1, "attn": DEFAULT_ATTN_MODE}


def set_gemm_mode(mode: int) -> None:
    _lib.check(_lib.lib().spr_set_gemm_mode(int(mode)), "spr_set_gemm_mode")
    _modes["gemm"] = int(mode)


def layernorm(x, gamma, beta, eps: float = 1e-5, pos=None, want_norm: bool = True):
    if _wants_grad(x, gamma, beta):
        from .autograd import LayerNormFn
        n, p = LayerNormFn.apply(_dev(x, "x", torch.float32), gamma, beta, float(eps), pos, bool(want_norm))
        return (n if (want_norm or pos is None) else None), (p if pos is not None else None)
    return layernorm_raw(x, gamma, beta, eps, pos, want_norm)


def layernorm_raw(x, gamma, beta, eps: float = 1e-5, pos=None, want_norm: bool = True):
    x = _dev(x, "x", torch.float32)
    m, c = x.shape
    out_norm = torch.empty_like(x) if want_norm else None
    out_pos = None
    if pos is not None:
        pos = _dev(pos, "pos", torch.float32)
        out_pos = torch.empty_like(x)
    L = _lib.lib()
    cnt = L.spr_layernorm_range_count(m)
    rn = _zero_slots(cnt, x.device) if out_norm is not None else None
    rp = _zero_slots(cnt, x.device) if out_pos is not None else None
    _lib.check(L.spr_layernorm(_ptr(x), m, c, _ptr(_dev(gamma, "gamma", torch.float32)),
                               _ptr(_dev(beta, "beta", torch.float32)), float(eps), _ptr(pos),
                               _ptr(out_norm), _ptr(out_pos), _ptr(rn), _ptr(rp), _stream(x)), "spr_layernorm")
    if out_norm is not None:
        _set_range(out_norm, rn, cnt)
    if out_pos is not None:
        _set_range(out_pos, rp, cnt)
    return out_norm, out_pos


def posemb_sine(xyz, d_model: int, scale: float = 1.0, temperature: float = 10000.0) -> torch.Tensor:
    xyz = _dev(xyz, "xyz", torch.float32)
    n = xyz.shape[0]
    out = torch.empty((n, d_model), dtype=torch.float32, device=xyz.device)
    _lib.check(_lib.lib().spr_posemb_sine(_ptr(xyz), n, d_model, float(scale * 2 * math.pi),
                                          float(temperature), _ptr(out), _stream(xyz)),
               "spr_posemb_sine")
    return out


def attention(q, k, v, cu, kv_seg, max_len: int, nhead: int, out=None, lens_host=None,
              kv_seg_host=None) -> torch.Tensor:
    if _wants_grad(q, k, v):
        from .autograd import AttentionFn
        if lens_host is None:
            c = cu.cpu().tolist()
            lens_host = [c[i + 1] - c[i] for i in range(len(c) - 1)]
        if kv_seg_host is None:
            kv_seg_host = kv_seg.cpu().tolist()
        return AttentionFn.apply(q, k, v, _dev(cu, "cu", torch.int32), _dev(kv_seg, "kv_seg", torch.int32),
                                 int(max_len), int(nhead), list(lens_host), list(kv_seg_host))
    return attention_raw(q, k, v, cu, kv_seg, max_len, nhead, out)


def attention_raw(q, k, v, cu, kv_seg, max_len: int, nhead: int, out=None, want_lse: bool = False):
    for t, nm in ((q, "q"), (k, "k"), (v, "v")):
        if not t.is_cuda or t.dtype != torch.float32 or t.stride(1) != 1:
            raise RuntimeError(f"attention: {nm} must be a float32 device tensor with unit inner stride")
    T, d = q.shape
    hd = d // nhead
    cu = _dev(cu, "cu", torch.int32)
    kv_seg = _dev(kv_seg, "kv_seg", torch.int32)
    nseg = cu.numel() - 1
    if out is None:
        out = torch.empty((T, d), dtype=torch.float32, device=q.device)
    L = _lib.lib()
    ws = _workspace(L.spr_attn_workspace_bytes(T, nseg, nhead, hd), q.device)
    lse = torch.empty((T, nhead), dtype=torch.float32, device=q.device) if want_lse else None
    written = ctypes.c_int(0)
    _lib.check(L.spr_attn_varlen_fwd(_ptr(q), q.stride(0), _ptr(k), k.stride(0), _ptr(v), v.stride(0),
                                     _ptr(cu), _ptr(kv_seg), T, nseg, int(max_len), nhead, hd,
                                     1.0 / math.sqrt(hd), _ptr(out), out.stride(0), _ptr(lse),
                                     ctypes.byref(written), _ptr(ws), ws.numel(), _stream(q)),
               "spr_attn_varlen_fwd")
    if want_lse:
        return out, (lse if written.value else None)
    return out


def attention_probs(q, k, cu, kv_seg, max_len: int, nhead: int, average: bool = True, out=None, place=None,
                    max_rows: Optional[int] = None, max_cols: Optional[int] = None) -> torch.Tensor:
    for t, nm in ((q, "q"), (k, "k")):
        if not isinstance(t, torch.Tensor) or not t.is_cuda:
            raise RuntimeError(f"attention_probs: {nm} must be a tensor on the MI355X device; the HIP path has no "
                               "CPU fallback")
        if t.dtype != torch.float32 or t.stride(1) != 1:
            raise RuntimeError(f"attention_probs: {nm} must be float32 with unit inner stride")
    q, k = q.detach(), k.detach()
    T, d = q.shape
    hd = d // nhead
    cu = _dev(cu, "cu", torch.int32)
    kv_seg = _dev(kv_seg, "kv_seg", torch.int32)
    nseg = cu.numel() - 1
    L = int(max_len)
    if out is None:
        if place is not None:
            raise RuntimeError("attention_probs: `place` needs `out`")
        shape = (nseg, L, L) if average else (nseg, nhead, L, L)
        out = torch.empty(shape, dtype=torch.float32, device=q.device)
        per = L * L * (1 if average else nhead)
        pl = np.zeros((nseg, 5), dtype=np.int64)
        pl[:, 0] = np.arange(nseg, dtype=np.int64) * per
        pl[:, 1], pl[:, 2], pl[:, 3], pl[:, 4] = L, L * L, L, L
        place, max_rows, max_cols = pl, L, L
    else:
        if not out.is_cuda or out.dtype != torch.float32 or not out.is_contiguous():
            raise RuntimeError("attention_probs: out must be a contiguous float32 device tensor")
        if place is None:
            raise RuntimeError("attention_probs: `out` needs `place`")
    if isinstance(place, np.ndarray) or (isinstance(place, torch.Tensor) and not place.is_cuda):
        pl = np.asarray(place.cpu().numpy() if isinstance(place, torch.Tensor) else place, dtype=np.int64)
        if pl.shape != (nseg, 5):
            raise RuntimeError(f"attention_probs: place must be [nseg={nseg}, 5] (got {pl.shape})")
        nh = 1 if average else nhead
        last = pl[:, 0] + (nh - 1) * pl[:, 2] + (pl[:, 3] - 1) * pl[:, 1] + pl[:, 4]
        if (pl[:, 0] < 0).any() or (pl[:, 3] < 1).any() or (pl[:, 4] < 1).any() or (pl[:, 4] > pl[:, 1]).any() \
                or int(last.max()) > out.numel():
            raise RuntimeError("attention_probs: place describes entries outside `out`")
        max_rows, max_cols = int(pl[:, 3].max()), int(pl[:, 4].max())
        place = torch.from_numpy(pl).to(q.device)
    elif max_rows is None or max_cols is None:
        raise RuntimeError("attention_probs: a device `place` needs max_rows and max_cols")
    Lb = _lib.lib()
    ws = _workspace(Lb.spr_attn_probs_workspace_bytes(T, nhead, hd), q.device)
    _lib.check(Lb.spr_attn_probs(_ptr(q), q.stride(0), _ptr(k), k.stride(0), _ptr(cu), _ptr(kv_seg), T, nseg, L,
                                 nhead, hd, 1.0 / math.sqrt(hd), 0 if average else 1, _ptr(out), _ptr(place),
                                 int(max_rows), int(max_cols), _ptr(ws), ws.numel(), _stream(q)), "spr_attn_probs")
    return out


_seg_perm_cache = {}


def _segment_perms(kv_seg_host, device):
    key = (tuple(int(x) for x in kv_seg_host), str(device))
    c = _seg_perm_cache.get(key)
    if c is None:
        kv = np.asarray(key[0], dtype=np.int32)
        inv = np.empty_like(kv)
        inv[kv] = np.arange(kv.size, dtype=np.int32)
        c = (torch.from_numpy(kv).to(device), torch.from_numpy(inv).to(device))
        _seg_perm_cache[key] = c
    return c


def attention_bwd(q, k, v, out, dout, cu, kv_seg_host, max_len: int, nhead: int, lse=None):
    for t, nm in ((q, "q"), (k, "k"), (v, "v"), (out, "out"), (dout, "dout")):
        if not t.is_cuda or t.dtype != torch.float32 or t.stride(1) != 1:
            raise RuntimeError(f"attention_bwd: {nm} must be a float32 device tensor with unit inner stride")
    T, d = q.shape
    hd = d // nhead
    cu = _dev(cu, "cu", torch.int32)
    nseg = cu.numel() - 1
    kv, inv = _segment_perms(kv_seg_host, q.device)
    dq = torch.empty((T, d), dtype=torch.float32, device=q.device)
    dk = torch.empty_like(dq)
    dv = torch.empty_like(dq)
    L = _lib.lib()
    ws = _workspace(L.spr_attn_bwd_workspace_bytes(T, nseg, nhead), q.device)
    _lib.check(L.spr_attn_varlen_bwd(_ptr(q), q.stride(0), _ptr(k), k.stride(0), _ptr(v), v.stride(0), _ptr(out),
                                     out.stride(0), _ptr(dout), dout.stride(0), _ptr(lse), _ptr(cu), _ptr(kv),
                                     _ptr(inv), T, nseg, int(max_len), nhead, hd, 1.0 / math.sqrt(hd), _ptr(dq),
                                     _ptr(dk), _ptr(dv), _ptr(ws), ws.numel(), _stream(q)), "spr_attn_varlen_bwd")
    return dq, dk, dv


def inproj_prepare(w_in: torch.Tensor):
    r = getattr(w_in, '_spr_inproj', None)
    if r is not None and r[1] == w_in._version and r[2] == w_in.data_ptr() and r[3] == _range_epoch[0]:
        r[4].acquire()
        return r[0]
    L = _lib.lib()
    d = w_in.shape[1]
    buf = torch.empty((L.spr_range_parts() + 3 * d,), dtype=torch.float32, device=w_in.device)
    _lib.check(L.spr_attn_inproj_prepare(_ptr(w_in), d, _ptr(buf), _stream(w_in)), "spr_attn_inproj_prepare")
    w_in._spr_inproj = (buf, w_in._version, w_in.data_ptr(), _range_epoch[0], _StreamGuard(buf))
    return buf


def attention_inproj(x_qk, x_v, w_in, b_in, cu, kv_seg, max_len: int, nhead: int, w_prep=None) -> torch.Tensor:
    x_qk = _dev(x_qk, "x_qk", torch.float32)
    x_v = x_qk if x_v is x_qk else _dev(x_v, "x_v", torch.float32)
    w_in = _dev(w_in, "w_in", torch.float32)
    b_in = _dev(b_in, "b_in", torch.float32)
    T, d = x_qk.shape
    assert x_v.shape == (T, d) and w_in.shape == (3 * d, d) and b_in.shape == (3 * d,)
    hd = d // nhead
    cu = _dev(cu, "cu", torch.int32)
    kv_seg = _dev(kv_seg, "kv_seg", torch.int32)
    nseg = cu.numel() - 1
    out = torch.empty((T, d), dtype=torch.float32, device=x_qk.device)
    L = _lib.lib()
    ws = _workspace(L.spr_attn_inproj_workspace_bytes(T, nseg, nhead, hd), x_qk.device)
    fused = _modes["attn"] != 0 and _modes["gemm"] == 1 and T >= 256
    qr, qn = _get_range(x_qk) if fused else (None, 0)
    vr, vn = (qr, qn) if x_v is x_qk else (_get_range(x_v) if fused else (None, 0))
    orng = torch.empty((1,), dtype=torch.float32, device=x_qk.device) if fused else None
    _lib.check(L.spr_attn_inproj_varlen_fwd(_ptr(x_qk), _ptr(x_v), T, _ptr(w_in), _ptr(b_in), _ptr(cu),
                                            _ptr(kv_seg), nseg, int(max_len), nhead, hd, 1.0 / math.sqrt(hd),
                                            _ptr(out), out.stride(0), _ptr(qr), int(qn), _ptr(vr), int(vn),
                                            _ptr(orng), _ptr(w_prep if fused else None), _ptr(ws), ws.numel(),
                                            _stream(x_qk)),
               "spr_attn_inproj_varlen_fwd")
    if orng is not None:
        _set_range(out, orng, 1)
    return out


_xenc_lock = threading.Lock()
XENC_PTRS_PER_LAYER = 18


class XencPlan:

    def __init__(self, key, prepared, plan, keep):
        self.key, self.prepared, self.plan, self.keep = key, prepared, plan, keep

    def __deepcopy__(self, memo):
        return None

    def __reduce__(self):
        return (_no_plan, ())


def _no_plan():
    return None
# ... 358 lines not shown
```

Measured before the change: 1209 pairs/s.

## Replace global radix sort with per-cloud LDS segmented sort in subsampling

```diff
diff --git a/include/spr.h b/include/spr.h
--- a/include/spr.h
+++ b/include/spr.h
@@ -21,7 +21,10 @@
 const char* spr_last_error(void);
 
 size_t spr_grid_subsample_workspace_bytes(int n, int nb);
-int spr_grid_subsample(const float* xyz, const int* cu, int n, int nb, float dl,
+size_t spr_segmented_sort_workspace_bytes(int n);
+int spr_segmented_sort(const unsigned long long* keys, const int* cu, int n, int nb, int max_len, int key_shift,
+                       unsigned long long* keys_out, int* vals_out, void* ws, size_t ws_bytes, void* stream);
+int spr_grid_subsample(const float* xyz, const int* cu, int n, int nb, int max_len, float dl,
                        int max_p, int order_mode, float* out_xyz, int* out_lens,
                        int* out_total, void* ws, size_t ws_bytes, void* stream);
 
@@ -31,7 +34,7 @@
 
 size_t spr_radius_neighbors_workspace_bytes(int nq, int ns, int nb);
 int spr_radius_neighbors(const float* q_xyz, const int* q_cu, int nq,
-                         const float* s_xyz, const int* s_cu, int ns, int nb,
+                         const float* s_xyz, const int* s_cu, int ns, int nb, int s_max_len,
                          float radius, int limit, int algo, int* out_idx,
                          int* max_count, void* ws, size_t ws_bytes, void* stream);
 
@@ -104,8 +107,8 @@
 int spr_maxpool_gather(const float* x, int ns, int c, const int* idx, int nq, int idx_stride, int k,
                        const int* order, float* out, float* out_range, int out_range_n, void* stream);
 size_t spr_cell_order_workspace_bytes(int n);
-int spr_cell_order(const float* xyz, const int* cu, int n, int nb, float cell, int* order, void* ws, size_t ws_bytes,
-                   void* stream);
+int spr_cell_order(const float* xyz, const int* cu, int n, int nb, int max_len, float cell, int* order, void* ws,
+                   size_t ws_bytes, void* stream);
 
 size_t spr_linear_workspace_bytes(void);
 int spr_linear(const float* x, int m, int k, const float* w, int n, const float* bias,
diff --git a/superpoints_registration_amd/_lib.py b/superpoints_registration_amd/_lib.py
--- a/superpoints_registration_amd/_lib.py
+++ b/superpoints_registration_amd/_lib.py
@@ -16,11 +16,13 @@
     "spr_version": (_i, []),
     "spr_last_error": (ctypes.c_char_p, []),
     "spr_grid_subsample_workspace_bytes": (_sz, [_i, _i]),
-    "spr_grid_subsample": (_i, [_vp, _vp, _i, _i, _f, _i, _i, _vp, _vp, _vp, _vp, _sz, _vp]),
+    "spr_grid_subsample": (_i, [_vp, _vp, _i, _i, _i, _f, _i, _i, _vp, _vp, _vp, _vp, _sz, _vp]),
+    "spr_segmented_sort_workspace_bytes": (_sz, [_i]),
+    "spr_segmented_sort": (_i, [_vp, _vp, _i, _i, _i, _i, _vp, _vp, _vp, _sz, _vp]),
     "spr_voxel_downsample_workspace_bytes": (_sz, [_i]),
     "spr_voxel_downsample": (_i, [_vp, _i, ctypes.c_double, _vp, _vp, _vp, _sz, _vp]),
     "spr_radius_neighbors_workspace_bytes": (_sz, [_i, _i, _i]),
-    "spr_radius_neighbors": (_i, [_vp, _vp, _i, _vp, _vp, _i, _i, _f, _i, _i, _vp, _vp, _vp, _sz, _vp]),
+    "spr_radius_neighbors": (_i, [_vp, _vp, _i, _vp, _vp, _i, _i, _i, _f, _i, _i, _vp, _vp, _vp, _sz, _vp]),
     "spr_radius_table_bytes": (_sz, [_i, _i]),
     "spr_radius_table_build_workspace_bytes": (_sz, [_i, _i]),
     "spr_radius_table_query_workspace_bytes": (_sz, [_i]),
@@ -59,7 +61,7 @@
                             _vp, _i, _vp, _i, _vp, _i, _vp, _vp, _f, _vp, _sz, _vp]),
     "spr_instnorm_stats": (_i, [_vp, _vp, _i, _i, _i, _i, _f, _vp, _vp, _vp, _sz, _vp]),
     "spr_cell_order_workspace_bytes": (_sz, [_i]),
-    "spr_cell_order": (_i, [_vp, _vp, _i, _i, _f, _vp, _vp, _sz, _vp]),
+    "spr_cell_order": (_i, [_vp, _vp, _i, _i, _i, _f, _vp, _vp, _sz, _vp]),
     "spr_layernorm_range_count": (_i, [_i]),
     "spr_attn_inproj_prepare": (_i, [_vp, _i, _vp, _vp]),
     "spr_set_gemm_mode": (_i, [_i]),
diff --git a/superpoints_registration_amd/csrc/grid_subsample.hip b/superpoints_registration_amd/csrc/grid_subsample.hip
--- a/superpoints_registration_amd/csrc/grid_subsample.hip
+++ b/superpoints_registration_amd/csrc/grid_subsample.hip
@@ -9,6 +9,149 @@
 #include "spr_common.h"
 
 namespace spr {
+
+namespace {
+constexpr int kIdxBits = 14;
+constexpr int kSortThreads = 1024, kSortWaves = 16, kSortRounds = kCloudSortCap / kSortThreads;
+constexpr int kHistStride = 257;
+constexpr int kSortTailInts = kSortWaves * kHistStride + kSortWaves + 4 * kSortWaves;
+static_assert(kCloudSortCap == 1 << kIdxBits, "index bits");
+
+__global__ __launch_bounds__(kSortThreads) void k_cloud_sort(const unsigned long long* __restrict__ keys_in,
+                                                             const int* __restrict__ cu, int cap, int key_shift,
+                                                             unsigned long long* __restrict__ keys_out,
+                                                             int* __restrict__ vals_out) {
+  extern __shared__ __align__(16) unsigned long long s_word[];
+  int* hist = reinterpret_cast<int*>(s_word + cap);
+  int* wtot = hist + kSortWaves * kHistStride;
+  unsigned int* red = reinterpret_cast<unsigned int*>(wtot + kSortWaves);
+  const int c = blockIdx.x;
+  const int beg = cu[c], n = cu[c + 1] - beg;
+  if (n <= 0 || n > cap) return;
+  const int tid = threadIdx.x, w = tid >> 6, lane = tid & 63;
+  const unsigned long long kmask = (1ull << key_shift) - 1;
+  unsigned long long vor = 0, vand = ~0ull;
+  for (int i = tid; i < n; i += kSortThreads) {
+    const unsigned long long k = keys_in[beg + i] & kmask;
+    vor |= k;
+    vand &= k;
+    s_word[i] = (k << kIdxBits) | (unsigned long long)i;
+  }
+#pragma unroll
+  for (int o = 32; o > 0; o >>= 1) {
+    vor |= __shfl_xor(vor, o, 64);
+    vand &= __shfl_xor(vand, o, 64);
+  }
+  if (lane == 0) {
+    red[4 * w + 0] = (unsigned int)vor, red[4 * w + 1] = (unsigned int)(vor >> 32);
+    red[4 * w + 2] = (unsigned int)vand, red[4 * w + 3] = (unsigned int)(vand >> 32);
+  }
+  __syncthreads();
+  vor = 0, vand = ~0ull;
+  for (int v = 0; v < kSortWaves; ++v) {
+    vor |= ((unsigned long long)red[4 * v + 1] << 32) | red[4 * v + 0];
+    vand &= ((unsigned long long)red[4 * v + 3] << 32) | red[4 * v + 2];
+  }
+  const unsigned long long varying = vor ^ vand;
+  const int rounds = (n + kSortThreads - 1) / kSortThreads;
+  const int first = w * rounds * 64 + lane;
+  const unsigned long long below_me = (1ull << lane) - 1;
+
+  for (int kb = 0; kb < key_shift; kb += 8) {
+    if (((varying >> kb) & 0xff) == 0) continue;
+    const int shift = kIdxBits + kb;
+    unsigned long long word[kSortRounds];
+    int rank[kSortRounds];
+#pragma unroll
+    for (int r = 0; r < kSortRounds; ++r) {
+      word[r] = 0;
+      rank[r] = 0;
+      if (r < rounds) {
+        const int idx = first + 64 * r;
+        if (idx < n) word[r] = s_word[idx];
+      }
+    }
+    for (int i = tid; i < kSortWaves * kHistStride; i += kSortThreads) hist[i] = 0;
+    __syncthreads();
+#pragma unroll
+    for (int r = 0; r < kSortRounds; ++r) {
+      if (r < rounds) {
+        const bool valid = first + 64 * r < n;
+        const int d = (int)(word[r] >> shift) & 0xff;
+        unsigned long long peers = __builtin_amdgcn_ballot_w64(valid);
+#pragma unroll
+        for (int b = 0; b < 8; ++b) {
+          const bool bit = (d >> b) & 1;
+          const unsigned long long m = __builtin_amdgcn_ballot_w64(bit);
+          peers &= bit ? m : ~m;
+        }
+        const int leader = valid ? __builtin_ctzll(peers) : lane;
+        int base = 0;
+        if (valid && lane == leader) base = atomicAdd(&hist[w * kHistStride + d], (int)__popcll(peers));
+        base = __shfl(base, leader, 64);
+        rank[r] = base + (int)__popcll(peers & below_me);
+      }
+    }
+    __syncthreads();
+    {
+      const int d = tid >> 2, w0 = (tid & 3) * 4;
+      int h[4], mine = 0;
+#pragma unroll
+      for (int j = 0; j < 4; ++j) {
+        h[j] = hist[(w0 + j) * kHistStride + d];
+        mine += h[j];
+      }
+      int incl = mine;
+#pragma unroll
+      for (int o = 1; o < 64; o <<= 1) {
+        const int v = __shfl_up(incl, o, 64);
+        if (lane >= o) incl += v;
+      }
+      if (lane == 63) wtot[w] = incl;
+      __syncthreads();
+      int run = incl - mine;
+      for (int v = 0; v < w; ++v) run += wtot[v];
+#pragma unroll
+      for (int j = 0; j < 4; ++j) {
+        hist[(w0 + j) * kHistStride + d] = run;
+        run += h[j];
+      }
+    }
+    __syncthreads();
+#pragma unroll
+    for (int r = 0; r < kSortRounds; ++r) {
+      if (r < rounds && first + 64 * r < n) {
+        const int d = (int)(word[r] >> shift) & 0xff;
+        s_word[hist[w * kHistStride + d] + rank[r]] = word[r];
+      }
+    }
+    __syncthreads();
+  }
+  const unsigned long long hi = (unsigned long long)c << key_shift;
+  for (int i = tid; i < n; i += kSortThreads) {
+    const unsigned long long wd = s_word[i];
+    if (keys_out) keys_out[beg + i] = hi | (wd >> kIdxBits);
+    vals_out[beg + i] = beg + (int)(wd & (kCloudSortCap - 1));
+  }
+}
+}
+
+bool cloud_sort_fits(int max_len, int key_shift) {
+  return max_len >= 1 && max_len <= kCloudSortCap && key_shift >= 1 && key_shift + kIdxBits <= 64;
+}
+
+int cloud_sort(const unsigned long long* keys_in, const int* cu, int nb, int max_len, int key_shift,
+               unsigned long long* keys_out, int* vals_out, hipStream_t stream) {
+  SPR_REQUIRE(cloud_sort_fits(max_len, key_shift), "cloud_sort: clouds of up to %d points do not fit", max_len);
+  const int cap = (max_len + 63) / 64 * 64;
+  const int lds = cap * (int)sizeof(unsigned long long) + kSortTailInts * (int)sizeof(int);
+  if (int rc = ensure_dyn_lds((const void*)k_cloud_sort, lds)) return rc;
+  hipLaunchKernelGGL(k_cloud_sort, dim3(nb), dim3(kSortThreads), lds, stream, keys_in, cu, cap, key_shift, keys_out,
+                     vals_out);
+  SPR_LAUNCH_CHECK();
+  return 0;
+}
+
 namespace {
 
 constexpr int kKeyBits = 40;
@@ -48,8 +191,9 @@
 
 __global__ __launch_bounds__(256) void k_bbox(const float* __restrict__ xyz,
                                               const int* __restrict__ cu,
-                                              float dl, CloudInfo* info) {
+                                              float dl, CloudInfo* info, int* scalars) {
   const int c = blockIdx.x;
+  if (c == 0 && threadIdx.x < 2) scalars[threadIdx.x] = 0;
   const int beg = cu[c], end = cu[c + 1];
   __shared__ float smn[3][256], smx[3][256];
   float mn[3], mx[3];
@@ -168,8 +312,8 @@
   vcu[c] = lo;
 }
 
-__global__ void k_cloud_offsets(const int* __restrict__ vcu, int nb, int max_p, int* out_cu,
-                                int* out_lens, int* out_total) {
+__global__ void k_cloud_offsets(const int* __restrict__ vcu, int nb, int max_p, const int* __restrict__ err,
+                                int* out_cu, int* out_lens, int* out_total) {
   if (threadIdx.x != 0 || blockIdx.x != 0) return;
   int b = 0;
   for (int c = 0; c < nb; ++c) {
@@ -180,7 +324,7 @@
     b += keep;
   }
   out_cu[nb] = b;
-  *out_total = b;
+  *out_total = *err ? -1 : b;
 }
 
 __global__ void k_emit_canonical(const float* __restrict__ bary,
@@ -200,13 +344,13 @@
   out[3 * o + 2] = bary[3 * (size_t)v + 2];
 }
 
-__global__ void k_mark_first(const int* __restrict__ vfirst, const int* __restrict__ nvox_p, int* __restrict__ mark,
-                             int* __restrict__ who) {
-  const int v = blockIdx.x * blockDim.x + threadIdx.x;
-  if (v >= *nvox_p) return;
-  const int f = vfirst[v];
-  mark[f] = 1;
-  who[f] = v;
+__global__ void k_mark_first(const int* __restrict__ vals, const int* __restrict__ head, const int* __restrict__ vid,
+                             int n, int* __restrict__ mark, int* __restrict__ who) {
+  const int j = blockIdx.x * blockDim.x + threadIdx.x;
+  if (j >= n) return;
+  const int p = vals[j], h = head[j];
+  mark[p] = h;
+  if (h) who[p] = vid[j];
 }
 __global__ void k_compact_first(const int* __restrict__ mark, const int* __restrict__ pos, const int* __restrict__ who,
                                 int n, int* __restrict__ ins) {
@@ -328,10 +472,6 @@
   }
 }
 
-__global__ void k_check_err(const int* err, int* out_total) {
-  if (*err) *out_total = -1;
-}
-
 size_t sort_temp_bytes(int n) {
   size_t bytes = 0;
   rocprim::radix_sort_pairs(nullptr, bytes, (unsigned long long*)nullptr,
@@ -363,7 +503,7 @@
   return b;
 }
 
-extern "C" int spr_grid_subsample(const float* xyz, const int* cu, int n, int nb,
+extern "C" int spr_grid_subsample(const float* xyz, const int* cu, int n, int nb, int max_len,
                                   float dl, int max_p, int order_mode,
                                   float* out_xyz, int* out_lens, int* out_total,
                                   void* ws, size_t ws_bytes, void* stream_) {
@@ -397,7 +537,6 @@
   int* tfirst = w.take<int>(tsz);
   int* tcnt = w.take<int>(tsz);
   int* thead = w.take<int>(tsz);
-  int* cloud_cnt = w.take<int>(nb + 1);
   int* vcu = w.take<int>(nb + 1);
   int* out_cu = w.take<int>(nb + 1);
   int* scalars = w.take<int>(64);
@@ -407,19 +546,21 @@
   int* nvox = scalars;
   int* err = scalars + 1;
 
-  SPR_HIP_CHECK(hipMemsetAsync(scalars, 0, 64 * sizeof(int), stream));
-  SPR_HIP_CHECK(hipMemsetAsync(cloud_cnt, 0, (nb + 1) * sizeof(int), stream));
-
   const int TB = 256;
-  hipLaunchKernelGGL(k_bbox, dim3(nb), dim3(256), 0, stream, xyz, cu, dl, info);
+  hipLaunchKernelGGL(k_bbox, dim3(nb), dim3(256), 0, stream, xyz, cu, dl, info, scalars);
   hipLaunchKernelGGL(k_keys, dim3(cdiv(n, TB)), dim3(TB), 0, stream, xyz, cu, n, nb, dl,
                      info, keys, vals, err);
   SPR_LAUNCH_CHECK();
   size_t tb = temp_bytes;
-  int key_bits = kKeyBits + 1;
-  while (key_bits < 64 && (1ull << (key_bits - kKeyBits)) < (unsigned long long)nb) ++key_bits;
-  SPR_HIP_CHECK(rocprim::radix_sort_pairs(temp, tb, keys, keys2, vals, vals2,
-                                          (unsigned int)n, 0, key_bits, stream));
+  const int longest = max_len > 0 ? max_len : n;
+  if (max_len >= 0 && cloud_sort_fits(longest, kKeyBits)) {
+    if (int rc = cloud_sort(keys, cu, nb, longest, kKeyBits, keys2, vals2, stream)) return rc;
+  } else {
+    int key_bits = kKeyBits + 1;
+    while (key_bits < 64 && (1ull << (key_bits - kKeyBits)) < (unsigned long long)nb) ++key_bits;
+    SPR_HIP_CHECK(rocprim::radix_sort_pairs(temp, tb, keys, keys2, vals, vals2,
+                                            (unsigned int)n, 0, key_bits, stream));
+  }
   hipLaunchKernelGGL(k_flags, dim3(cdiv(n, TB)), dim3(TB), 0, stream, keys2, n, flags);
   tb = temp_bytes;
   SPR_HIP_CHECK(rocprim::exclusive_scan(temp, tb, flags, vid, 0, (size_t)n,
@@ -429,7 +570,7 @@
   hipLaunchKernelGGL(k_bary, dim3(cdiv(n, TB)), dim3(TB), 0, stream, xyz, keys2, vals2,
                      vstart, nvox, n, bary, vkey, vfirst);
   hipLaunchKernelGGL(k_cloud_lb, dim3(cdiv(nb + 1, 256)), dim3(256), 0, stream, vkey, nvox, nb, vcu);
-  hipLaunchKernelGGL(k_cloud_offsets, dim3(1), dim3(64), 0, stream, vcu, nb, max_p, out_cu,
+  hipLaunchKernelGGL(k_cloud_offsets, dim3(1), dim3(64), 0, stream, vcu, nb, max_p, err, out_cu,
                      out_lens, out_total);
   SPR_LAUNCH_CHECK();
   if (order_mode == SPR_ORDER_CANONICAL) {
@@ -441,18 +582,16 @@
     for (int i = 0; i < kMaxSched; ++i)
       sched.v[i] = i < (int)s.buckets.size() ? s.buckets[i] : 0xffffffffu;
     const int nsched = (int)(s.buckets.size() < (size_t)kMaxSched ? s.buckets.size() : kMaxSched);
-    SPR_HIP_CHECK(hipMemsetAsync(flags, 0, N * sizeof(int), stream));
-    hipLaunchKernelGGL(k_mark_first, dim3(cdiv(n, TB)), dim3(TB), 0, stream, vfirst, nvox, flags, vid);
+    hipLaunchKernelGGL(k_mark_first, dim3(cdiv(n, TB)), dim3(TB), 0, stream, vals2, flags, vid, n, nxt, scan);
     tb = temp_bytes;
-    SPR_HIP_CHECK(rocprim::exclusive_scan(temp, tb, flags, vstart, 0, (size_t)n, rocprim::plus<int>(), stream));
-    hipLaunchKernelGGL(k_compact_first, dim3(cdiv(n, TB)), dim3(TB), 0, stream, flags, vstart, vid, n, sval2);
+    SPR_HIP_CHECK(rocprim::exclusive_scan(temp, tb, nxt, vstart, 0, (size_t)n, rocprim::plus<int>(), stream));
+    hipLaunchKernelGGL(k_compact_first, dim3(cdiv(n, TB)), dim3(TB), 0, stream, nxt, vstart, scan, n, sval2);
     const int umap_lds = kUmapLdsInts * (int)sizeof(int);
     if (int rc = ensure_dyn_lds((const void*)k_umap_order, umap_lds)) return rc;
     hipLaunchKernelGGL(k_umap_order, dim3(nb), dim3(1024), umap_lds, stream, vkey, sval2, vcu, cu,
                        nsched, sched, listA, listB, tfirst, tcnt, thead, nxt, scan, sval, bary, out_cu,
                        out_lens, out_xyz);
   }
-  hipLaunchKernelGGL(k_check_err, dim3(1), dim3(1), 0, stream, err, out_total);
   SPR_LAUNCH_CHECK();
   return 0;
 }
@@ -496,7 +635,7 @@
   return 2 * align_up(8 * N, 256) + align_up(4 * N, 256) + sort_temp_bytes(n) + 256;
 }
 
-extern "C" int spr_cell_order(const float* xyz, const int* cu, int n, int nb, float cell, int* order, void* ws,
+extern "C" int spr_cell_order(const float* xyz, const int* cu, int n, int nb, int max_len, float cell, int* order, void* ws,
                               size_t ws_bytes, void* stream_) {
   hipStream_t stream = (hipStream_t)stream_;
   SPR_REQUIRE(n >= 1 && nb >= 1 && nb < (1 << 30) && cell > 0.f, "cell_order: bad arguments");
@@ -510,9 +649,48 @@
   SPR_REQUIRE(temp != nullptr, "cell_order: workspace carve failed");
   hipLaunchKernelGGL(k_order_keys, dim3(cdiv(n, 256)), dim3(256), 0, stream, xyz, cu, n, nb, 1.0f / cell, keys, vals);
   SPR_LAUNCH_CHECK();
+  const int longest = max_len > 0 ? max_len : n;
+  if (max_len >= 0 && cloud_sort_fits(longest, 30)) return cloud_sort(keys, cu, nb, longest, 30, nullptr, order, stream);
   int bits = 31;
   while (bits < 60 && (1ull << (bits - 30)) < (unsigned long long)nb) ++bits;
   SPR_HIP_CHECK(rocprim::radix_sort_pairs(temp, tb, keys, keys2, vals, order, (unsigned int)n, 0, bits, stream));
+  return 0;
+}
+
+namespace spr {
+namespace {
+__global__ void k_iota(int n, int* v) {
+  const int i = blockIdx.x * blockDim.x + threadIdx.x;
+  if (i < n) v[i] = i;
+}
+}
+}
+
+extern "C" size_t spr_segmented_sort_workspace_bytes(int n) {
+  return align_up(4 * (size_t)(n > 0 ? n : 1), 256) + sort_temp_bytes(n) + 256;
+}
+
+extern "C" int spr_segmented_sort(const unsigned long long* keys, const int* cu, int n, int nb, int max_len,
+                                  int key_shift, unsigned long long* keys_out, int* vals_out, void* ws,
+                                  size_t ws_bytes, void* stream_) {
+  hipStream_t stream = (hipStream_t)stream_;
+  SPR_REQUIRE(keys && cu && keys_out && vals_out && n >= 1 && nb >= 1, "segmented_sort: bad arguments");
+  SPR_REQUIRE(key_shift >= 1 && key_shift <= 48 && (unsigned long long)nb <= (1ull << (63 - key_shift)),
+"segmented_sort: key_shift out of range");
+  SPR_REQUIRE(ws_bytes >= spr_segmented_sort_workspace_bytes(n), "segmented_sort: workspace too small");
+  const int longest = max_len > 0 ? max_len : n;
+  if (max_len >= 0 && cloud_sort_fits(longest, key_shift))
+    return cloud_sort(keys, cu, nb, longest, key_shift, keys_out, vals_out, stream);
+  Workspace w(ws, ws_bytes);
+  int* vals = w.take<int>(n);
+  size_t tb = sort_temp_bytes(n);
+  void* temp = w.take<char>(tb);
+  SPR_REQUIRE(temp != nullptr, "segmented_sort: workspace carve failed");
+  hipLaunchKernelGGL(k_iota, dim3(cdiv(n, 256)), dim3(256), 0, stream, n, vals);
+  SPR_LAUNCH_CHECK();
+  int bits = key_shift + 1;
+  while (bits < 64 && (1ull << (bits - key_shift)) < (unsigned long long)nb) ++bits;
+  SPR_HIP_CHECK(rocprim::radix_sort_pairs(temp, tb, keys, keys_out, vals, vals_out, (unsigned int)n, 0, bits, stream));
   return 0;
 }
 
diff --git a/superpoints_registration_amd/csrc/radius_neighbors.hip b/superpoints_registration_amd/csrc/radius_neighbors.hip
--- a/superpoints_registration_amd/csrc/radius_neighbors.hip
+++ b/superpoints_registration_amd/csrc/radius_neighbors.hip
@@ -16,8 +16,12 @@
 constexpr int kMaxCell = 8191;
 
 __global__ __launch_bounds__(256) void k_min(const float* __restrict__ xyz,
-                                             const int* __restrict__ cu, NbrCloud* info) {
+                                             const int* __restrict__ cu, NbrCloud* info, int* err, int* max_count) {
   const int c = blockIdx.x;
+  if (c == 0 && threadIdx.x == 0) {
+    *err = 0;
+    *max_count = 0;
+  }
   const int beg = cu[c], end = cu[c + 1];
   __shared__ float smn[3][256];
   float mn[3] = {3.0e38f, 3.0e38f, 3.0e38f};
@@ -84,7 +88,7 @@
     const float* __restrict__ q_xyz, const int* __restrict__ q_cu, int nq,
     const int* __restrict__ s_cu, int ns, int nb, const NbrCloud* __restrict__ info,
     const unsigned long long* __restrict__ skeys, const float4* __restrict__ rec, float r2,
-    float inv_cell, int limit, int* __restrict__ out, int* max_count) {
+    float inv_cell, int limit, const int* __restrict__ err, int* __restrict__ out, int* max_count) {
   extern __shared__ __align__(16) unsigned char smem[];
   float* l_d2 = (float*)smem;
   int* l_id = (int*)(smem + sizeof(float) * (size_t)limit * BLOCK);
@@ -158,7 +162,9 @@
   int m = total;
 #pragma unroll
   for (int o = 32; o > 0; o >>= 1) m = max(m, __shfl_xor(m, o, 64));
-  if ((t & 63) == 0 && m > 0) atomicMax(max_count, m);
+  const int bad = *err;
+  if ((t & 63) == 0 && m > 0 && !bad) atomicMax(max_count, m);
+  if (bad && blockIdx.x == 0 && t == 0) *max_count = -1;
 }
 
 
@@ -215,11 +221,19 @@
 }
 
 constexpr int kTableSlots = 8;
-constexpr int kHdrErr = 0, kHdrCells = 1, kHdrSlot0 = 8;
+constexpr int kHdrErr = 0, kHdrCells = 1, kHdrSlot0 = 8, kHdrCtr0 = kHdrSlot0 + kTableSlots,
+              kHdrArrive0 = kHdrCtr0 + kTableSlots;
+static_assert(kHdrArrive0 + kTableSlots <= 64, "header is 64 ints");
+
+__device__ __forceinline__ int nbr_status(int err, int slot_max) {
+  if (err & 1) return -1;
+  if (err & 2) return -2;
+  return slot_max;
+}
 __global__ void k_grid_offsets(GridCloud* info, int nb, long long cap, int* hdr) {
   if (threadIdx.x != 0 || blockIdx.x != 0) return;
   int* err = hdr + kHdrErr;
-  for (int k = 0; k < kTableSlots; ++k) hdr[kHdrSlot0 + k] = 0;
+  for (int k = kHdrSlot0; k < kHdrArrive0 + kTableSlots; ++k) hdr[k] = 0;
   long long off = 0;
   for (int c = 0; c < nb; ++c) {
     info[c].off = off;
@@ -497,13 +511,16 @@
 __global__ __launch_bounds__(BLOCK) void k_sort_rows(const unsigned long long* __restrict__ tmp_key,
                                                      const int* __restrict__ kept_in,
                                                      const int* __restrict__ qid_in,
-                                                     const int* __restrict__ err, int nq, int ns,
-                                                     int limit, int lslots, int* __restrict__ out) {
+                                                     const int* __restrict__ hdr, int slot, int nq, int ns,
+                                                     int limit, int lslots, int* __restrict__ out,
+                                                     int* __restrict__ status) {
   extern __shared__ __align__(16) unsigned char smem[];
   unsigned long long* l_key = (unsigned long long*)smem;
   const int t = threadIdx.x;
   const int i = blockIdx.x * BLOCK + t;
-  if (*err || i >= nq) return;
+  const int err = hdr[kHdrErr];
+  if (blockIdx.x == 0 && t == 0) *status = nbr_status(err, hdr[kHdrSlot0 + slot]);
+  if (err || i >= nq) return;
   const int kept = kept_in[i];
   const unsigned long long* src = tmp_key + i;
   const size_t rs = (size_t)nq;
@@ -552,11 +569,18 @@
 __global__ __launch_bounds__(256) void k_knn_wave(
     const float* __restrict__ q_xyz, const int* __restrict__ q_cu, int nq, int nb,
     const GridCloud* __restrict__ info, const int* __restrict__ start, const float4* __restrict__ rec,
-    const int* __restrict__ err, float r2, float inv_cell, int limit, int self, int ns, int* __restrict__ out,
-    int* max_count, int* q_ctr) {
+    int* hdr, int slot, float r2, float inv_cell, int limit, int self, int ns, int* __restrict__ out,
+    int* __restrict__ status) {
   __shared__ unsigned long long s_key[4][128];
   const int lane = threadIdx.x & 63, wave = threadIdx.x >> 6;
-  if (*err) return;
+  int* const max_count = hdr + kHdrSlot0 + slot;
+  int* const q_ctr = hdr + kHdrCtr0 + slot;
+  int* const arrive = hdr + kHdrArrive0 + slot;
+  const int err = hdr[kHdrErr];
+  if (err) {
+    if (blockIdx.x == 0 && threadIdx.x == 0) *status = nbr_status(err, 0);
+    return;
+  }
   unsigned long long* sk = s_key[wave];
   constexpr unsigned long long kNone = ~0ull;
   int cl_lo = 0, cl_hi = 0;
@@ -671,6 +695,17 @@
     }
   }
   if (lane == 0 && wave_max > 0 && wave_max > *reinterpret_cast<volatile int*>(max_count)) atomicMax(max_count, wave_max);
+  __threadfence();
+  __syncthreads();
+  if (threadIdx.x == 0) {
+    const int ticket = atomicAdd(arrive, 1);
+    if (ticket == (int)gridDim.x - 1) {
+      __threadfence();
+      *status = atomicMax(max_count, 0);
+      atomicExch(q_ctr, 0);
+      atomicExch(arrive, 0);
+    }
+  }
 }
 
 template <int B, int E, class F>
@@ -684,11 +719,13 @@
 template <int N>
 __global__ __launch_bounds__(256) void k_sort_rows_reg(const unsigned long long* __restrict__ tmp_key,
                                                        const int* __restrict__ kept_in, const int* __restrict__ qid_in,
-                                                       const int* __restrict__ err, int nq, int ns, int limit,
-                                                       int* __restrict__ out) {
+                                                       const int* __restrict__ hdr, int slot, int nq, int ns, int limit,
+                                                       int* __restrict__ out, int* __restrict__ status) {
   static_assert(N % 8 == 0, "rows in chunks of eight");
   const int i = blockIdx.x * 256 + threadIdx.x;
-  if (*err) return;
+  const int err = hdr[kHdrErr];
+  if (i == 0) *status = nbr_status(err, hdr[kHdrSlot0 + slot]);
+  if (err) return;
   const bool act = i < nq;
   const int kept = act ? min(kept_in[i], N) : 0;
   int kmax = kept;
@@ -724,13 +761,6 @@
   });
   if (act)
     for (int k = kept; k < limit; ++k) row[k] = ns;
-}
-
-__global__ void k_nbr_err2(const int* hdr, int slot, int* max_count) {
-  const int err = hdr[kHdrErr];
-  if (err & 1) *max_count = -1;
-  else if (err & 2) *max_count = -2;
-  else *max_count = hdr[kHdrSlot0 + slot];
 }
 
 size_t table_cap_cells(int ns) { return (size_t)64 * (size_t)(ns > 0 ? ns : 1) + ((size_t)1 << 20); }
@@ -803,15 +833,13 @@
   const float r2 = radius * radius;
   const float inv_cell = 1.0f / (radius * (1.0f + 1.0f / 256.0f));
   if (algo == 1) {
-    SPR_HIP_CHECK(hipMemsetAsync(qid, 0, sizeof(int), stream));
     const int nblk = min(cdiv(nq, 4 * kKnnChunk), 8 * device_cu_count());
     if (limit <= 64)
       hipLaunchKernelGGL(k_knn_wave<false>, dim3(nblk), dim3(256), 0, stream, q_xyz, q_cu, nq, nb, t.ginfo, t.start, t.rec,
-                         t.hdr + kHdrErr, r2, inv_cell, limit, self, ns, out_idx, t.hdr + kHdrSlot0 + slot, qid);
+                         t.hdr, slot, r2, inv_cell, limit, self, ns, out_idx, max_count);
     else
       hipLaunchKernelGGL(k_knn_wave<true>, dim3(nblk), dim3(256), 0, stream, q_xyz, q_cu, nq, nb, t.ginfo, t.start, t.rec,
-                         t.hdr + kHdrErr, r2, inv_cell, limit, self, ns, out_idx, t.hdr + kHdrSlot0 + slot, qid);
-    hipLaunchKernelGGL(k_nbr_err2, dim3(1), dim3(1), 0, stream, t.hdr, slot, max_count);
+                         t.hdr, slot, r2, inv_cell, limit, self, ns, out_idx, max_count);
     SPR_LAUNCH_CHECK();
     return 0;
   }
@@ -819,21 +847,15 @@
                      t.rec, t.hdr + kHdrErr, r2, inv_cell, rcap, limit, self, tmp_key, kept, qid, t.hdr + kHdrSlot0 + slot);
   if (use_reg) {
     hipLaunchKernelGGL(k_sort_rows_reg<kRegRows>, dim3(cdiv(nq, 256)), dim3(256), 0, stream, tmp_key, kept, qid,
-                       t.hdr + kHdrErr, nq, ns, limit, out_idx);
-    hipLaunchKernelGGL(k_nbr_err2, dim3(1), dim3(1), 0, stream, t.hdr, slot, max_count);
+                       t.hdr, slot, nq, ns, limit, out_idx, max_count);
     SPR_LAUNCH_CHECK();
     return 0;
   }
   constexpr int BLOCK = 64;
   hipLaunchKernelGGL(k_sort_rows<BLOCK>, dim3(cdiv(nq, BLOCK)), dim3(BLOCK), (size_t)rcap * 8 * BLOCK, stream, tmp_key,
-                     kept, qid, t.hdr + kHdrErr, nq, ns, limit, rcap, out_idx);
-  hipLaunchKernelGGL(k_nbr_err2, dim3(1), dim3(1), 0, stream, t.hdr, slot, max_count);
+                     kept, qid, t.hdr, slot, nq, ns, limit, rcap, out_idx, max_count);
   SPR_LAUNCH_CHECK();
   return 0;
-}
-
-__global__ void k_nbr_err(const int* err, int* max_count) {
-  if (*err) *max_count = -1;
 }
 
 size_t nbr_sort_temp_bytes(int n) {
@@ -863,7 +885,7 @@
 }
 
 extern "C" int spr_radius_neighbors(const float* q_xyz, const int* q_cu, int nq,
-                                    const float* s_xyz, const int* s_cu, int ns, int nb,
+                                    const float* s_xyz, const int* s_cu, int ns, int nb, int s_max_len,
                                     float radius, int limit, int algo, int* out_idx,
                                     int* max_count, void* ws, size_t ws_bytes, void* stream_) {
   hipStream_t stream = (hipStream_t)stream_;
@@ -899,31 +921,33 @@
   }
   const float r2 = radius * radius;
   const float inv_cell = 1.0f / (radius * (1.0f + 1.0f / 256.0f));
-  SPR_HIP_CHECK(hipMemsetAsync(err, 0, 16 * sizeof(int), stream));
-  SPR_HIP_CHECK(hipMemsetAsync(max_count, 0, sizeof(int), stream));
-  hipLaunchKernelGGL(k_min, dim3(nb), dim3(256), 0, stream, s_xyz, s_cu, info);
+  hipLaunchKernelGGL(k_min, dim3(nb), dim3(256), 0, stream, s_xyz, s_cu, info, err, max_count);
   hipLaunchKernelGGL(k_cellkeys, dim3(cdiv(ns, TB)), dim3(TB), 0, stream, s_xyz, s_cu, ns, nb,
                      inv_cell, info, keys, vals, err);
   SPR_LAUNCH_CHECK();
-  size_t tb = temp_bytes;
-  SPR_HIP_CHECK(rocprim::radix_sort_pairs(temp, tb, keys, keys2, vals, vals2,
-                                          (unsigned int)ns, 0, 64, stream));
+  const int longest = s_max_len > 0 ? s_max_len : ns;
+  if (s_max_len >= 0 && cloud_sort_fits(longest, 48)) {
+    if (int rc = cloud_sort(keys, s_cu, nb, longest, 48, keys2, vals2, stream)) return rc;
+  } else {
+    size_t tb = temp_bytes;
+    SPR_HIP_CHECK(rocprim::radix_sort_pairs(temp, tb, keys, keys2, vals, vals2,
+                                            (unsigned int)ns, 0, 64, stream));
+  }
   hipLaunchKernelGGL(k_gather_sorted, dim3(cdiv(ns, TB)), dim3(TB), 0, stream, s_xyz, vals2, ns,
                      rec);
   if (limit <= 64) {
     constexpr int BLOCK = 128;
     const size_t lds = (size_t)limit * BLOCK * 8;
     hipLaunchKernelGGL(k_query<BLOCK>, dim3(cdiv(nq, BLOCK)), dim3(BLOCK), lds, stream, q_xyz,
-                       q_cu, nq, s_cu, ns, nb, info, keys2, rec, r2, inv_cell, limit, out_idx,
+                       q_cu, nq, s_cu, ns, nb, info, keys2, rec, r2, inv_cell, limit, err, out_idx,
                        max_count);
   } else {
     constexpr int BLOCK = 64;
     const size_t lds = (size_t)limit * BLOCK * 8;
     hipLaunchKernelGGL(k_query<BLOCK>, dim3(cdiv(nq, BLOCK)), dim3(BLOCK), lds, stream, q_xyz,
-                       q_cu, nq, s_cu, ns, nb, info, keys2, rec, r2, inv_cell, limit, out_idx,
+                       q_cu, nq, s_cu, ns, nb, info, keys2, rec, r2, inv_cell, limit, err, out_idx,
                        max_count);
   }
-  hipLaunchKernelGGL(k_nbr_err, dim3(1), dim3(1), 0, stream, err, max_count);
   SPR_LAUNCH_CHECK();
   return 0;
 }
diff --git a/superpoints_registration_amd/csrc/spr_common.h b/superpoints_registration_amd/csrc/spr_common.h
--- a/superpoints_registration_amd/csrc/spr_common.h
+++ b/superpoints_registration_amd/csrc/spr_common.h
@@ -85,6 +85,11 @@
 int ensure_dyn_lds(const void* kernel, int bytes);
 int device_cu_count();
 
+constexpr int kCloudSortCap = 16384;
+bool cloud_sort_fits(int max_len, int key_shift);
+int cloud_sort(const unsigned long long* keys_in, const int* cu, int nb, int max_len, int key_shift,
+               unsigned long long* keys_out, int* vals_out, hipStream_t stream);
+
 int launch_absmax(const float* x, long rows, int cols, long stride, float* parts, hipStream_t stream);
 int launch_absmax2(const float* x0, long rows0, int cols0, long stride0, float* parts0, const float* x1,
                    long rows1, int cols1, long stride1, float* parts1, hipStream_t stream);
diff --git a/superpoints_registration_amd/hip_shim.py b/superpoints_registration_amd/hip_shim.py
--- a/superpoints_registration_amd/hip_shim.py
+++ b/superpoints_registration_amd/hip_shim.py
@@ -53,7 +53,7 @@
         lens = torch.empty(nb, dtype=torch.int32, device=dev)
         tot = torch.empty(1, dtype=torch.int32, device=dev)
         cu = _cu(batches, dev)
-        rc = L.spr_grid_subsample(_p(x), _p(cu), n, nb, ctypes.c_float(sampleDl), int(max_p), 0,
+        rc = L.spr_grid_subsample(_p(x), _p(cu), n, nb, int(max(batches)), ctypes.c_float(sampleDl), int(max_p), 0,
                                   _p(out), _p(lens), _p(tot), _p(ws), ctypes.c_size_t(ws.numel()), _stream(dev))
         if rc:
             _raise(L)
@@ -80,7 +80,7 @@
         m = -2
         q_cu, s_cu = _cu(q_batches, dev), _cu(s_batches, dev)
         for algo in (0, 1):
-            rc = L.spr_radius_neighbors(_p(q), _p(q_cu), nq, _p(s), _p(s_cu), ns, nb,
+            rc = L.spr_radius_neighbors(_p(q), _p(q_cu), nq, _p(s), _p(s_cu), ns, nb, int(max(s_batches)),
                                         ctypes.c_float(radius), int(limit), algo, _p(out), _p(mc), _p(ws),
                                         ctypes.c_size_t(ws.numel()), _stream(dev))
             if rc:
diff --git a/superpoints_registration_amd/kpconv.py b/superpoints_registration_amd/kpconv.py
--- a/superpoints_registration_amd/kpconv.py
+++ b/superpoints_registration_amd/kpconv.py
@@ -209,11 +209,11 @@
             yield meta, 'conv', l
             if lv.down:
                 dl = 2 * lv.radius / cfg.conv_radius
-                sub_points, sub_lens = ops.grid_subsample(points, cu, dl, order=self.order)
+                sub_points, sub_lens = ops.grid_subsample(points, cu, dl, order=self.order, max_len=max(lens_host))
                 sub_lens_host = sub_lens.tolist()
                 sub_cu = ops.lengths_to_cu(sub_lens_host, device)
                 pool = search((l, 'pool'), sub_points, sub_cu, points, cu, lv.radius, lv.limit)
-                meta['pool_order'].append(ops.cell_order(sub_points, sub_cu, dl))
+                meta['pool_order'].append(ops.cell_order(sub_points, sub_cu, dl, max_len=max(sub_lens_host)))
                 if self.compute_upsamples:
                     up = search((l, 'up'), points, cu, sub_points, sub_cu, 2 * lv.radius, lv.limit)
             if not lv.down:
diff --git a/superpoints_registration_amd/ops.py b/superpoints_registration_amd/ops.py
--- a/superpoints_registration_amd/ops.py
+++ b/superpoints_registration_amd/ops.py
@@ -174,8 +174,12 @@
     _lib.check(_lib.lib().spr_selftest(ctypes.byref(st)), "spr_selftest")
 
 
+def _max_len_arg(max_len: Optional[int]) -> int:
+    return 0 if max_len is None else int(max_len)
+
+
 def grid_subsample(points: torch.Tensor, cu: torch.Tensor, dl: float, max_p: int = 0,
-                   order: int = ORDER_REFERENCE) -> Tuple[torch.Tensor, torch.Tensor]:
+                   order: int = ORDER_REFERENCE, max_len: Optional[int] = None) -> Tuple[torch.Tensor, torch.Tensor]:
     points = _dev(points, "points", torch.float32)
     cu = _dev(cu, "cu", torch.int32)
     n, nb = points.shape[0], cu.numel() - 1
@@ -184,13 +188,27 @@
     out = torch.empty((max(n, 1), 3), dtype=torch.float32, device=points.device)
     out_lens = torch.empty((nb,), dtype=torch.int32, device=points.device)
     total = torch.empty((1,), dtype=torch.int32, device=points.device)
-    _lib.check(L.spr_grid_subsample(_ptr(points), _ptr(cu), n, nb, float(dl), int(max_p), int(order),
+    _lib.check(L.spr_grid_subsample(_ptr(points), _ptr(cu), n, nb, _max_len_arg(max_len), float(dl), int(max_p), int(order),
                                     _ptr(out), _ptr(out_lens), _ptr(total), _ptr(ws), ws.numel(),
                                     _stream(points)), "spr_grid_subsample")
     m = int(total.item())
     if m < 0:
         raise RuntimeError("spr_grid_subsample: voxel grid too large for 40-bit keys")
     return out[:m], out_lens
+
+
+def segmented_sort(keys: torch.Tensor, cu: torch.Tensor, key_shift: int,
+                   max_len: Optional[int] = None) -> Tuple[torch.Tensor, torch.Tensor]:
+    keys = _dev(keys, "keys", torch.int64)
+    cu = _dev(cu, "cu", torch.int32)
+    n, nb = keys.shape[0], cu.numel() - 1
+    L = _lib.lib()
+    ws = _workspace(L.spr_segmented_sort_workspace_bytes(n), keys.device)
+    out_k = torch.empty_like(keys)
+    out_v = torch.empty((n,), dtype=torch.int32, device=keys.device)
+    _lib.check(L.spr_segmented_sort(_ptr(keys), _ptr(cu), n, nb, _max_len_arg(max_len), int(key_shift), _ptr(out_k),
+                                    _ptr(out_v), _ptr(ws), ws.numel(), _stream(keys)), "spr_segmented_sort")
+    return out_k, out_v
 
 
 def voxel_downsample(points: torch.Tensor, voxel_size: float) -> torch.Tensor:
@@ -210,7 +228,7 @@
 
 def radius_neighbors(queries: torch.Tensor, supports: torch.Tensor, q_cu: torch.Tensor,
                      s_cu: torch.Tensor, radius: float, limit: int,
-                     exact_width: bool = True, algo: int = 0) -> Tuple[torch.Tensor, int]:
+                     exact_width: bool = True, algo: int = 0, max_len: Optional[int] = None) -> Tuple[torch.Tensor, int]:
     queries = _dev(queries, "queries", torch.float32)
     supports = _dev(supports, "supports", torch.float32)
     q_cu = _dev(q_cu, "q_cu", torch.int32)
@@ -221,13 +239,13 @@
     out = torch.empty((nq, limit), dtype=torch.int32, device=queries.device)
     mc = torch.empty((1,), dtype=torch.int32, device=queries.device)
     _lib.check(L.spr_radius_neighbors(_ptr(queries), _ptr(q_cu), nq, _ptr(supports), _ptr(s_cu), ns,
-                                      nb, float(radius), int(limit), int(algo), _ptr(out), _ptr(mc),
+                                      nb, _max_len_arg(max_len), float(radius), int(limit), int(algo), _ptr(out), _ptr(mc),
                                       _ptr(ws), ws.numel(), _stream(queries)), "spr_radius_neighbors")
     if not exact_width:
         return out, -1
     m = int(mc.item())
     if m == -2 and algo == 0:
-        return radius_neighbors(queries, supports, q_cu, s_cu, radius, limit, exact_width, algo=1)
+        return radius_neighbors(queries, supports, q_cu, s_cu, radius, limit, exact_width, algo=1, max_len=max_len)
     if m < 0:
         raise RuntimeError("spr_radius_neighbors: cloud extent / radius exceeds 8191 cells per axis")
     if m < 1:
@@ -668,14 +686,14 @@
     return out
 
 
-def cell_order(points: torch.Tensor, cu: torch.Tensor, cell: float) -> torch.Tensor:
+def cell_order(points: torch.Tensor, cu: torch.Tensor, cell: float, max_len: Optional[int] = None) -> torch.Tensor:
     points = _dev(points, "points", torch.float32)
     cu = _dev(cu, "cu", torch.int32)
     n, nb = points.shape[0], cu.numel() - 1
     L = _lib.lib()
     out = torch.empty((n,), dtype=torch.int32, device=points.device)
     ws = _workspace(L.spr_cell_order_workspace_bytes(n), points.device)
-    _lib.check(L.spr_cell_order(_ptr(points), _ptr(cu), n, nb, float(cell), _ptr(out), _ptr(ws), ws.numel(),
+    _lib.check(L.spr_cell_order(_ptr(points), _ptr(cu), n, nb, _max_len_arg(max_len), float(cell), _ptr(out), _ptr(ws), ws.numel(),
                                 _stream(points)), "spr_cell_order")
     return out
 
```

Result: no change. 1224 pairs/s, median of 4 (+1.2%).
